# Bob-cheng/DepthModelHardening

Measured on AMD Instinct MI355X. Metric: adv-train images/sec @1024x320, 10-step PGD, bs32, higher is better.
Workload: dtype f32; 1 GPU; Monodepth2 ResNet18 1024x320, 10-step PGD-L_inf attack on 12 scenes, train batch 32/GPU, stereo photometric+SSIM+smoothness loss (md2), Adam; config_index=2, global_batch=32, per_gpu_batch=32, parallelism=dp1, attack_overlap=False, attack_scenes=12, graph_attack=False

## Files before the change

depthmodelhardening_amd/_native.py:

```python
import ctypes as C
import os

import torch

MAX_SCALES = 4
MAX_FRAMES = 4
VARIANT_MD2, VARIANT_DH = 0, 1
NOISE_NONE, NOISE_TENSOR, NOISE_PHILOX = 0, 1, 2
PASTE_COMPOSITE, PASTE_WARP_ONLY = 0, 1
FIN_LOSS, FIN_LOSS_S, FIN_REPROJ_S, FIN_COUNT_S, FIN_SMOOTH_S, FIN_HINT_S, FIN_HINTCOUNT_S, FIN_SIZE = 0, 1, 5, 9, 13, 20, 24, 28

LIB_PATH = os.environ.get("DMH_HIP_LIB") or os.path.join(os.path.dirname(os.path.abspath(__file__)), "lib",
                                                        "libdmh_hip.so")

_fp = C.c_void_p


class PhotoArgs(C.Structure):
    _fields_ = [("target", _fp), ("source", _fp * MAX_FRAMES), ("T", _fp * MAX_FRAMES), ("K", _fp), ("inv_K", _fp),
                ("disp", _fp * MAX_SCALES), ("Hs", C.c_int * MAX_SCALES), ("Ws", C.c_int * MAX_SCALES),
                ("B", C.c_int), ("H", C.c_int), ("W", C.c_int), ("num_frames", C.c_int), ("num_scales", C.c_int),
                ("min_depth", C.c_float), ("max_depth", C.c_float), ("variant", C.c_int), ("automask", C.c_int),
                ("no_ssim", C.c_int), ("noise_mode", C.c_int), ("noise", _fp * MAX_SCALES),
                ("seed", C.c_uint64), ("offset", C.c_uint64), ("depth_hint", _fp), ("depth_hint_mask", _fp)]


class SmoothArgs(C.Structure):
    _fields_ = [("disp", _fp * MAX_SCALES), ("color", _fp * MAX_SCALES), ("Hs", C.c_int * MAX_SCALES),
                ("Ws", C.c_int * MAX_SCALES), ("B", C.c_int), ("num_scales", C.c_int)]


class PasteArgs(C.Structure):
    _fields_ = [("scene", _fp), ("scene_bstride", C.c_int64), ("patch", _fp), ("pmask", _fp), ("coeffs", _fp),
                ("N", C.c_int), ("SH", C.c_int), ("SW", C.c_int), ("PH", C.c_int), ("PW", C.c_int),
                ("OH", C.c_int), ("OW", C.c_int), ("l_pad", C.c_int), ("t_pad", C.c_int), ("mode", C.c_int),
                ("flip", _fp), ("scene_index", _fp)]


class RoiGlueArgs(C.Structure):
    _fields_ = [("y", _fp), ("skip", _fp), ("y_org", _fp), ("skip_org", _fp), ("dst_org", _fp),
                ("B", C.c_int), ("C1", C.c_int), ("C2", C.c_int), ("sh", C.c_int), ("sw", C.c_int), ("kh", C.c_int),
                ("kw", C.c_int), ("hc", C.c_int), ("wc", C.c_int), ("H", C.c_int), ("W", C.c_int), ("up", C.c_int),
                ("elu", C.c_int)]


class WinoWtJob(C.Structure):
    _fields_ = [("w", _fp), ("scale", _fp), ("U", _fp), ("K", C.c_int), ("C", C.c_int), ("backward", C.c_int)]


_PtrArr = _fp * MAX_SCALES

_SIGNATURES = {
    "dmh_version": (C.c_char_p, []),
    "dmh_last_error": (C.c_char_p, []),
    "dmh_debug_channel_copy": (C.c_int, [_fp, _fp, C.c_int64, C.c_int, C.c_int, _fp]),
    "dmh_photo_partials_size": (C.c_int64, [C.c_int, C.c_int, C.c_int, C.c_int]),
    "dmh_photo_stage_size": (C.c_int64, [C.POINTER(PhotoArgs)]),
    "dmh_photo_loss_fwd": (C.c_int, [C.POINTER(PhotoArgs), _fp, _PtrArr, _fp, _fp]),
    "dmh_photo_loss_bwd": (C.c_int, [C.POINTER(PhotoArgs), _fp, _fp, _fp, _fp, _PtrArr, _fp]),
    "dmh_photo_pose_partials_size": (C.c_int64, [C.POINTER(PhotoArgs)]),
    "dmh_photo_loss_bwd_pose": (C.c_int, [C.POINTER(PhotoArgs), _fp, _fp, _fp, _fp, _PtrArr, _fp, _fp]),
    "dmh_unpack_selection": (C.c_int, [_fp, C.c_int64, C.c_int, _fp, _fp]),
    "dmh_upsample_bilinear_adjoint": (C.c_int, [_fp, _fp, C.c_int, C.c_int, C.c_int, C.c_int, C.c_int, C.c_int, _fp]),
    "dmh_warp_view_fwd": (C.c_int, [_fp] * 5 + [C.c_int] * 5 + [C.c_float, C.c_float] + [_fp] * 4),
    "dmh_warp_view_bwd": (C.c_int, [_fp] * 5 + [C.c_int] * 5 + [C.c_float, C.c_float] + [_fp] * 4),
    "dmh_smooth_partials_size": (C.c_int64, [C.POINTER(SmoothArgs)]),
    "dmh_smooth_loss_fwd": (C.c_int, [C.POINTER(SmoothArgs), _fp, _fp]),
    "dmh_smooth_loss_bwd": (C.c_int, [C.POINTER(SmoothArgs), _fp, _fp, C.c_float, _PtrArr, C.c_int, _fp]),
    "dmh_loss_finalize": (C.c_int, [_fp, _fp, C.c_int, C.c_int, C.c_int, C.POINTER(SmoothArgs), C.c_int, C.c_float,
                                    _fp, _fp, _fp]),
    "dmh_eot_paste_fwd": (C.c_int, [C.POINTER(PasteArgs), _fp, _fp, _fp]),
    "dmh_eot_paste_bwd": (C.c_int, [C.POINTER(PasteArgs), _fp, _fp, _fp]),
    "dmh_pgd_linf_step": (C.c_int, [_fp, _fp, _fp, C.c_float, C.c_float, _fp, C.c_int64, _fp]),
    "dmh_apgd_step": (C.c_int, [_fp] * 6 + [C.c_int, C.c_float, C.c_int64, _fp]),
    "dmh_apgd_commit": (C.c_int, [_fp] * 10 + [C.c_int] * 3 + [C.c_double, C.c_int64, _fp]),
    "dmh_l0_fused_step": (C.c_int, [_fp] * 15 + [C.c_int] * 3 + [C.c_float] * 3 + [_fp]),
    "dmh_tube_light_compose": (C.c_int, [_fp] * 4 + [C.c_int] * 3 + [_fp]),
    "dmh_tube_light_commit": (C.c_int, [_fp] * 4 + [C.c_int, _fp]),
    "dmh_gauss_blur_windows": (C.c_int, [_fp] * 5 + [C.c_int] * 9 + [_fp]),
    "dmh_gauss_blur_compose": (C.c_int, [_fp] * 4 + [C.c_int] * 8 + [_fp]),
    "dmh_square_propose": (C.c_int, [_fp] * 6 + [C.c_int] * 4 + [C.c_float, _fp]),
    "dmh_pgd_l2_workspace_size": (C.c_int64, [C.c_int64]),
    "dmh_pgd_l2_step": (C.c_int, [_fp, _fp, _fp, C.c_double, C.c_double, _fp, C.c_int64, _fp, C.c_int64, _fp]),
    "dmh_eigen_select_ws_size": (C.c_int64, [C.c_int]),
    "dmh_eigen_partials_size": (C.c_int64, [C.c_int]),
    "dmh_eigen_gt_stats": (C.c_int, [_fp, C.c_int64, _fp, _fp] + [C.c_int] * 7 + [_fp] * 4),
    "dmh_eigen_pred_depth": (C.c_int, [_fp, _fp, C.c_int, C.c_int, _fp, C.c_int64, _fp, _fp] + [C.c_int] * 7
                             + [C.c_float, C.c_int64, _fp, C.c_int64, _fp, _fp]),
    "dmh_eigen_pred_ratio": (C.c_int, [_fp, C.c_int64, C.c_int64, C.c_int64, _fp, _fp] + [C.c_int] * 6 + [_fp] * 5),
    "dmh_eigen_metrics": (C.c_int, [_fp, C.c_int64, _fp, C.c_int64, C.c_int64, _fp, _fp] + [C.c_int] * 6 + [_fp] * 4),
    "dmh_l0_compose_fwd": (C.c_int, [_fp, _fp, _fp, C.c_int, C.c_int, C.c_float, C.c_int, _fp, _fp, _fp]),
    "dmh_l0_compose_bwd": (C.c_int, [_fp, _fp, _fp, _fp, C.c_int, C.c_int, _fp, _fp, C.c_int, _fp]),
    "dmh_l0_mask_partials_size": (C.c_int64, [C.c_int]),
    "dmh_l0_mask_cost_fwd": (C.c_int, [_fp, _fp, C.c_int, C.c_int, _fp, _fp, _fp]),
    "dmh_l0_mask_cost_bwd": (C.c_int, [_fp, _fp, C.c_int, C.c_int, _fp, _fp, _fp, _fp, C.c_int, _fp]),
    "dmh_sq_mean_partials_size": (C.c_int64, [C.c_int64]),
    "dmh_masked_sq_mean_fwd": (C.c_int, [_fp, _fp, C.c_int64, _fp, _fp, _fp]),
    "dmh_masked_sq_mean_bwd": (C.c_int, [_fp, _fp, C.c_int64, _fp, _fp, _fp]),
    "dmh_gt_depth_mse_fwd": (C.c_int, [_fp, _fp, _fp, C.c_int64, _fp, C.c_int, C.c_int64, C.c_float, C.c_float, _fp, _fp, _fp]),
    "dmh_gt_depth_mse_bwd": (C.c_int, [_fp, _fp, _fp, C.c_int64, _fp, C.c_int, C.c_int64, C.c_float, C.c_float, _fp, _fp, _fp]),
    "dmh_ssim_map": (C.c_int, [_fp, _fp, C.c_int, C.c_int, C.c_int, _fp, _fp]),
    "dmh_ssim_map_bwd": (C.c_int, [_fp, _fp, _fp, C.c_int, C.c_int, C.c_int, _fp, _fp, _fp, _fp]),
    "dmh_avg_pyramid": (C.c_int, [_fp, C.c_int, C.c_int, C.c_int, _fp, _fp, _fp, _fp]),
    "dmh_edge_smooth_partials_size": (C.c_int64, [C.c_int, C.c_int, C.c_int]),
    "dmh_edge_smooth": (C.c_int, [_fp, _fp] + [C.c_int] * 4 + [_fp, _fp, _fp]),
    "dmh_edge_smooth_bwd": (C.c_int, [_fp, _fp] + [C.c_int] * 4 + [_fp, _fp, _fp]),
    "dmh_depth_errors_partials_size": (C.c_int64, [C.c_int64]),
    "dmh_masked_depth_errors": (C.c_int, [_fp, _fp, _fp, C.c_int64] + [C.c_float] * 5 + [_fp, _fp, _fp]),
    "dmh_dec_up_cat_pad_fwd": (C.c_int, [_fp, _fp] + [C.c_int] * 5 + [_fp, _fp]),
    "dmh_dec_up_cat_pad_bwd": (C.c_int, [_fp, _fp] + [C.c_int] * 5 + [_fp, _fp, _fp]),
    "dmh_elu_pad_fwd": (C.c_int, [_fp] + [C.c_int] * 5 + [_fp, _fp]),
    "dmh_elu_pad_bwd": (C.c_int, [_fp, _fp] + [C.c_int] * 5 + [_fp, _fp]),
    "dmh_roi_glue_fwd": (C.c_int, [C.POINTER(RoiGlueArgs), _fp, _fp]),
    "dmh_roi_glue_bwd": (C.c_int, [C.POINTER(RoiGlueArgs), _fp, _fp, _fp, _fp, C.c_int, C.c_int, _fp, C.c_int, C.c_int, _fp]),
    "dmh_roi_crop": (C.c_int, [_fp] * 4 + [C.c_int] * 7 + [_fp, _fp]),
    "dmh_roi_paste": (C.c_int, [_fp, _fp, C.c_int, C.c_int, _fp] + [C.c_int] * 6 + [_fp, _fp]),
    "dmh_stem_conv_norm_fwd_win": (C.c_int, [_fp, _fp, _fp] + [C.c_int] * 5 + [C.c_float, C.c_float, _fp, _fp]),
    "dmh_stem_bn_relu_pool_bwd_win": (C.c_int, [_fp] * 7 + [C.c_int] * 8 + [_fp, _fp]),
    "dmh_conv7x7s2_bwd_data_win": (C.c_int, [_fp] * 4 + [C.c_int] * 9 + [_fp, _fp]),
    "dmh_roi_cost_partials_size": (C.c_int64, [C.c_int, C.c_int, C.c_int]),
    "dmh_roi_cost_fwd": (C.c_int, [_fp, _fp, _fp] + [C.c_int] * 5 + [_fp] * 4),
    "dmh_roi_cost_bwd": (C.c_int, [_fp, _fp, _fp] + [C.c_int] * 5 + [_fp] * 3),
    "dmh_roi_cost_fwd_scaled": (C.c_int, [_fp, _fp, _fp] + [C.c_int] * 5 + [C.c_float] + [_fp] * 4),
    "dmh_roi_cost_bwd_scaled": (C.c_int, [_fp, _fp, _fp] + [C.c_int] * 5 + [C.c_float] + [_fp] * 3),
    "dmh_bn_act_fwd": (C.c_int, [_fp] * 4 + [C.c_int] * 4 + [_fp, _fp]),
    "dmh_bn_act_bwd": (C.c_int, [_fp] * 3 + [C.c_int] * 4 + [_fp, _fp, _fp]),
    "dmh_bn_stats_partials_size": (C.c_int64, [C.c_int, C.c_int, C.c_int]),
    "dmh_bn_train_stats": (C.c_int, [_fp, C.c_int, C.c_int, C.c_int, _fp, _fp, C.c_float, C.c_float] + [_fp] * 8),
    "dmh_bn_train_stats_tracked": (C.c_int, [_fp, C.c_int, C.c_int, C.c_int, _fp, _fp, C.c_float, C.c_float] + [_fp] * 9),
    "dmh_channel_sum_partials_size": (C.c_int64, [C.c_int, C.c_int, C.c_int]),
    "dmh_channel_sum": (C.c_int, [_fp, C.c_int, C.c_int, C.c_int, _fp, _fp, C.c_void_p]),
    "dmh_bn_train_bwd_workspace_size": (C.c_int64, [C.c_int, C.c_int, C.c_int]),
    "dmh_bn_train_bwd": (C.c_int, [_fp] * 6 + [C.c_int, C.c_int, C.c_int] + [_fp] * 5 + [C.c_void_p]),
    "dmh_stem_bn_relu_pool_fwd": (C.c_int, [_fp] * 3 + [C.c_int] * 4 + [_fp] * 4),
    "dmh_stem_bn_relu_pool_bwd": (C.c_int, [_fp] * 5 + [C.c_int] * 4 + [_fp, _fp]),
    "dmh_wino_weight_size": (C.c_int64, [C.c_int, C.c_int]),
    "dmh_wino_weight_transform": (C.c_int, [_fp, C.c_int, C.c_int, C.c_int, _fp, _fp]),
    "dmh_wino_conv3x3": (C.c_int, [_fp] * 3 + [C.c_int] * 6 + [_fp, _fp]),
    "dmh_wino_conv3x3_ws": (C.c_int, [_fp] * 3 + [C.c_int] * 6 + [_fp, _fp, C.c_int64, _fp]),
    "dmh_wino_conv3x3_plan": (C.c_int, [C.c_int] * 7 + [C.c_int64]),
    "dmh_wino_weight_transform_scaled": (C.c_int, [_fp, C.c_int, C.c_int, C.c_int, _fp, _fp, _fp]),
    "dmh_wino_conv3x3_act": (C.c_int, [_fp] * 4 + [C.c_int] * 7 + [_fp, _fp]),
    "dmh_wino_weight_transform_batch": (C.c_int, [C.POINTER(WinoWtJob), C.c_int, _fp]),
    "dmh_wino_conv3x3_act_ws": (C.c_int, [_fp] * 4 + [C.c_int] * 7 + [_fp, _fp, C.c_int64, _fp]),
    "dmh_wino32_weight_size": (C.c_int64, [C.c_int, C.c_int]),
    "dmh_wino32_weight_transform": (C.c_int, [_fp, C.c_int, C.c_int, C.c_int, _fp, _fp]),
    "dmh_wino32_conv3x3": (C.c_int, [_fp] * 3 + [C.c_int] * 6 + [_fp, _fp]),
    "dmh_wino32_conv3x3_ws": (C.c_int, [_fp] * 3 + [C.c_int] * 6 + [_fp, _fp, C.c_int64, _fp]),
    "dmh_wino_wrw_workspace_size": (C.c_int64, [C.c_int] * 6),
    "dmh_wino_wrw": (C.c_int, [_fp, _fp] + [C.c_int] * 6 + [_fp, _fp, _fp]),
    "dmh_conv3x3_small": (C.c_int, [_fp] * 3 + [C.c_int] * 7 + [_fp, _fp]),
    "dmh_conv3x3_head": (C.c_int, [_fp] * 3 + [C.c_int] * 5 + [_fp, _fp]),
    "dmh_conv3x3_head_bwd_data": (C.c_int, [_fp, _fp] + [C.c_int] * 4 + [_fp, _fp]),
    "dmh_down_wrw_workspace_size": (C.c_int64, [C.c_int] * 5),
    "dmh_down_wrw": (C.c_int, [_fp] * 3 + [C.c_int] * 5 + [_fp] * 4),
    "dmh_stem_wrw_workspace_size": (C.c_int64, [C.c_int] * 3),
    "dmh_stem_wrw": (C.c_int, [_fp, _fp] + [C.c_int] * 3 + [C.c_float, C.c_float, _fp, _fp, _fp]),
    "dmh_conv3x3_head_wrw_partials_size": (C.c_int64, [C.c_int] * 5),
    "dmh_conv3x3_head_wrw": (C.c_int, [_fp, _fp] + [C.c_int] * 5 + [_fp] * 4),
    "dmh_conv3x3_small_wrw_partials_size": (C.c_int64, [C.c_int]),
    "dmh_conv3x3_small_wrw": (C.c_int, [_fp, _fp] + [C.c_int] * 5 + [_fp] * 4),
    "dmh_conv7x7s2_bwd_data": (C.c_int, [_fp, _fp] + [C.c_int] * 5 + [_fp, _fp]),
    "dmh_stem_conv_norm_fwd": (C.c_int, [_fp, _fp, C.c_int, C.c_int, C.c_int, C.c_float, C.c_float, _fp, _fp]),
    "dmh_down_conv_fwd": (C.c_int, [_fp] * 3 + [C.c_int] * 5 + [_fp] * 3),
    "dmh_down_conv_fwd_act": (C.c_int, [_fp] * 5 + [C.c_int] * 6 + [_fp] * 3),
    "dmh_down_conv_bwd_data": (C.c_int, [_fp] * 4 + [C.c_int] * 5 + [_fp, _fp]),
    "dmh_down_conv_bwd_data_acc": (C.c_int, [_fp] * 5 + [C.c_int] * 5 + [_fp, _fp]),
    "dmh_down_conv_image_size": (C.c_int64, [C.c_int, C.c_int]),
    "dmh_down_conv_weight_image": (C.c_int, [_fp, _fp, C.c_int, C.c_int, _fp, _fp]),
    "dmh_down_conv_fwd_img": (C.c_int, [_fp, _fp, C.c_int, _fp, _fp] + [C.c_int] * 6 + [_fp] * 3),
    "dmh_down_conv_bwd_data_img": (C.c_int, [_fp] * 4 + [C.c_int] * 5 + [_fp, _fp]),
}

EXPORTS = tuple(sorted(_SIGNATURES))

_lib = None


def lib():
    global _lib
    if _lib is None:
        if not os.path.exists(LIB_PATH) and "DMH_HIP_LIB" not in os.environ:
            try:
                from .build import build
                build(verbose=False)
            except Exception as e:
                raise RuntimeError("libdmh_hip.so is not built (%s) and building it failed (%s): run `python -m "
                                   "depthmodelhardening_amd.build`; there is no CPU/eager fallback for the hot path"
                                   % (LIB_PATH, e))
        if not os.path.exists(LIB_PATH):
            raise RuntimeError("libdmh_hip.so is not built (%s): run `python -m depthmodelhardening_amd.build`; "
                               "there is no CPU/eager fallback for the hot path" % LIB_PATH)
        handle = C.CDLL(LIB_PATH)
        for name, (res, args) in _SIGNATURES.items():
            fn = getattr(handle, name)
            fn.restype = res
            fn.argtypes = args
        _lib = handle
    return _lib


def check(rc):
    if rc != 0:
        raise RuntimeError("libdmh_hip: " + lib().dmh_last_error().decode())


def ptr(t):
    if t is None:
        return None
    if not t.is_cuda:
        raise RuntimeError("libdmh_hip ops need CUDA (ROCm) tensors; got device %s -- there is no CPU path" % t.device)
    if not t.is_contiguous():
        raise RuntimeError("libdmh_hip ops need contiguous tensors")
    if t.dtype not in (torch.float32, torch.int32, torch.uint8):
        raise RuntimeError("libdmh_hip ops compute in fp32; got %s" % t.dtype)
    return C.c_void_p(t.data_ptr())


def ptr_f64(t):
    if not t.is_cuda:
        raise RuntimeError("libdmh_hip ops need CUDA (ROCm) tensors; got device %s -- there is no CPU path" % t.device)
    if not t.is_contiguous() or t.dtype != torch.float64:
        raise RuntimeError("libdmh_hip: expected a contiguous float64 tensor; got %s" % t.dtype)
    return C.c_void_p(t.data_ptr())


def stream():
    return C.c_void_p(torch.cuda.current_stream().cuda_stream)


def ptr_array(tensors, n=MAX_SCALES):
    arr = (_fp * n)()
    for i, t in enumerate(tensors):
        arr[i] = None if t is None else ptr(t)
    return arr
```

depthmodelhardening_amd/csrc/common.hpp:

```cpp
#pragma once
#include <hip/hip_runtime.h>

#include <atomic>
#include <stdint.h>
#include <stdio.h>
#include <string.h>

#include "dmh_hip.h"

namespace dmh {

constexpr int WAVE = 64;

extern thread_local char g_err[512];

inline int fail(int code, const char* fmt, const char* a = "", long long b = 0, long long c = 0) {
    snprintf(g_err, sizeof(g_err), fmt, a, b, c);
    return code;
}

#define DMH_REQUIRE(cond, msg)                                                     \
    do {                                                                            \
        if (!(cond)) return dmh::fail(DMH_EINVAL, "%s: requirement failed: " msg, __func__); \
    } while (0)

inline int check_launch(const char* fn) {
    hipError_t e = hipGetLastError();
    if (e != hipSuccess) {
        snprintf(g_err, sizeof(g_err), "%s: launch failed: %s", fn, hipGetErrorString(e));
        return DMH_ELAUNCH;
    }
    return DMH_OK;
}

__device__ __forceinline__ float wave_sum(float v) {
#pragma unroll
    for (int o = WAVE / 2; o > 0; o >>= 1) v += __shfl_down(v, o, WAVE);
    return v;
}

template <int NT>
__device__ __forceinline__ float block_sum(float v, float* red) {
    v = wave_sum(v);
    const int lane = threadIdx.x & (WAVE - 1), w = threadIdx.x / WAVE;
    __syncthreads();
    if (lane == 0) red[w] = v;
    __syncthreads();
    float t = 0.f;
    if (threadIdx.x == 0) {
#pragma unroll
        for (int i = 0; i < NT / WAVE; ++i) t += red[i];
    }
    return t;
}

__device__ __forceinline__ int reflect_idx(int p, int n) {
    p = p < 0 ? -p : p;
    p = p >= n ? 2 * (n - 1) - p : p;
    return min(max(p, 0), n - 1);
}

__device__ __forceinline__ float fast_rcp(float x) {
    float r = __builtin_amdgcn_rcpf(x);
    return r * (2.0f - x * r);
}

typedef __amdgpu_buffer_rsrc_t rsrc_t;

__device__ __forceinline__ rsrc_t make_rsrc(const void* p, unsigned bytes) {
    const unsigned long long v = (unsigned long long)p;
    const unsigned lo = __builtin_amdgcn_readfirstlane((unsigned)v), hi = __builtin_amdgcn_readfirstlane((unsigned)(v >> 32));
    return __builtin_amdgcn_make_buffer_rsrc((void*)(((unsigned long long)hi << 32) | lo), 0, bytes, 0x00020000);
}
typedef float f32x2 __attribute__((ext_vector_type(2)));
#define DMH_PK_FORM(NAME, MODS)                                                  \
    __device__ __forceinline__ f32x2 NAME(const f32x2 a, const f32x2 b) {        \
        f32x2 r;                                                                 \
        asm("v_pk_add_f32 %0, %1, %2 " MODS : "=v"(r) : "v"(a), "v"(b));         \
        return r;                                                                \
    }
DMH_PK_FORM(pk_add, "")
DMH_PK_FORM(pk_sub, "neg_lo:[0,1] neg_hi:[0,1]")
DMH_PK_FORM(pk_bfly, "op_sel:[0,1] op_sel_hi:[0,1] neg_hi:[0,1]")
DMH_PK_FORM(pk_bfly_neg, "op_sel:[0,1] op_sel_hi:[0,1] neg_lo:[1,1] neg_hi:[1,0]")
DMH_PK_FORM(pk_col01, "op_sel:[0,0] op_sel_hi:[1,0] neg_lo:[0,1]")
DMH_PK_FORM(pk_col23, "op_sel:[1,0] op_sel_hi:[1,1] neg_lo:[1,0] neg_hi:[0,1]")
#define DMH_PK_MOV(NAME, MODS)                                                   \
    __device__ __forceinline__ f32x2 NAME(const f32x2 a, const f32x2 b) {        \
        f32x2 r;                                                                 \
        asm("v_pk_mov_b32 %0, %1, %2 " MODS : "=v"(r) : "v"(a), "v"(b));         \
        return r;                                                                \
    }
DMH_PK_MOV(pk_lo_lo, "op_sel:[0,0]")
DMH_PK_MOV(pk_hi_hi, "op_sel:[1,1]")

__device__ __forceinline__ float ldb(rsrc_t rs, unsigned byte_off, unsigned s_off) {
    return __builtin_bit_cast(float, __builtin_amdgcn_raw_buffer_load_b32(rs, byte_off, s_off, 0));
}
__device__ __forceinline__ float lane_prev(float v) {
    return __builtin_bit_cast(float, __builtin_amdgcn_update_dpp(0, __builtin_bit_cast(int, v), 0x138, 0xf, 0xf, false));
}
__device__ __forceinline__ float lane_next(float v) {
    return __builtin_bit_cast(float, __builtin_amdgcn_update_dpp(0, __builtin_bit_cast(int, v), 0x130, 0xf, 0xf, false));
}

template <int ROUNDS = 7>
struct Philox {
    uint32_t k0, k1;
    __device__ __forceinline__ Philox(uint64_t seed) : k0((uint32_t)seed), k1((uint32_t)(seed >> 32)) {}
    __device__ __forceinline__ uint4 operator()(uint64_t ctr_lo, uint64_t ctr_hi) const {
        uint32_t c0 = (uint32_t)ctr_lo, c1 = (uint32_t)(ctr_lo >> 32), c2 = (uint32_t)ctr_hi,
                 c3 = (uint32_t)(ctr_hi >> 32);
        uint32_t a = k0, b = k1;
#pragma unroll
        for (int r = 0; r < ROUNDS; ++r) {
            const uint32_t hi0 = __umulhi(0xD2511F53u, c0), lo0 = 0xD2511F53u * c0;
            const uint32_t hi1 = __umulhi(0xCD9E8D57u, c2), lo1 = 0xCD9E8D57u * c2;
            const uint32_t n0 = hi1 ^ c1 ^ a, n1 = lo1, n2 = hi0 ^ c3 ^ b, n3 = lo0;
            c0 = n0; c1 = n1; c2 = n2; c3 = n3;
            a += 0x9E3779B9u;
            b += 0xBB67AE85u;
        }
        return make_uint4(c0, c1, c2, c3);
    }
};

__device__ __forceinline__ float normal_from_bits(uint32_t u0, uint32_t u1) {
    const float a = ((float)u0 + 1.0f) * 2.3283064365386963e-10f;
    const float b = (float)u1 * 2.3283064365386963e-10f;
    return sqrtf(-2.0f * __logf(a)) * __cosf(6.283185307179586f * b);
}

__device__ __forceinline__ float2 normal_pair_from_bits(uint32_t u0, uint32_t u1) {
    const float a = ((float)u0 + 1.0f) * 2.3283064365386963e-10f;
    const float b = (float)u1 * 2.3283064365386963e-10f;
    const float rad = sqrtf(-2.0f * __logf(a));
    float sn, cs;
    __sincosf(6.283185307179586f * b, &sn, &cs);
    return make_float2(rad * cs, rad * sn);
}

__host__ __device__ inline int sk_boundary(int per, int rem, int nch, int w) {
    const int b = w * per + (w < rem ? w : rem);
    const int item = b / nch;
    int c = b - item * nch;
    if (c != 0) {
        if (nch >= 6) c = c < 3 ? 3 : (c > nch - 3 ? nch - 3 : c);
        else c = (2 * c < nch) ? 0 : nch;
    }
    return item * nch + c;
}

template <typename Kernel>
inline hipError_t configure_dynamic_lds(Kernel kernel, size_t bytes, std::atomic<uint64_t>& done) {
    int dev = 0;
    hipError_t e = hipGetDevice(&dev);
    if (e != hipSuccess) return e;
    const uint64_t bit = (dev >= 0 && dev < 64) ? (1ull << dev) : 0;
    if (bit && (done.load(std::memory_order_acquire) & bit)) return hipSuccess;
    e = hipFuncSetAttribute(reinterpret_cast<const void*>(kernel), hipFuncAttributeMaxDynamicSharedMemorySize, (int)bytes);
    if (e == hipSuccess && bit) done.fetch_or(bit, std::memory_order_release);
    return e;
}

}
```

depthmodelhardening_amd/csrc/encoder_glue.hip:

```cpp
#include "common.hpp"

#include <cmath>

using namespace dmh;

namespace {

constexpr int NT = 256;

__device__ __forceinline__ float relu_f(float v) { return v > 0.f ? v : 0.f; }

template <bool RELU, bool RES>
__global__ __launch_bounds__(NT) void bn_act_fwd_vec(const float4* __restrict__ x, const float* __restrict__ scale,
                                                     const float* __restrict__ shift, const float4* __restrict__ res,
                                                     unsigned C, unsigned hw4, unsigned total4, float4* __restrict__ out) {
    const unsigned i = blockIdx.x * NT + threadIdx.x;
    if (i >= total4) return;
    const unsigned c = (i / hw4) % C;
    const float s = scale[c], b = shift[c];
    const float4 v = x[i];
    float4 r = make_float4(fmaf(v.x, s, b), fmaf(v.y, s, b), fmaf(v.z, s, b), fmaf(v.w, s, b));
    if (RES) {
        const float4 q = res[i];
        r.x += q.x; r.y += q.y; r.z += q.z; r.w += q.w;
// ... 41 lines not shown
    if (RES) g_res[i] = gv;
    g_x[i] = gv * scale[(i / hw) % C];
}

__global__ __launch_bounds__(NT) void stem_fwd_kernel(const float* __restrict__ x, const float* __restrict__ scale,
                                                      const float* __restrict__ shift, int C, int H, int W,
                                                      float* __restrict__ feat, float* __restrict__ pooled,
                                                      unsigned char* __restrict__ argmax) {
    const int PH = H >> 1, PW = W >> 1;
    const int t = blockIdx.x * NT + threadIdx.x;
    if (t >= PH * PW) return;
    const int plane = blockIdx.y, c = plane % C;
    const int i = t / PW, j = t - i * PW;
    const float s = scale[c], b = shift[c];
    const float* xp = x + (size_t)plane * H * W;
    float* fp = feat + (size_t)plane * H * W;
    float m = -INFINITY;
    int arg = 4;
#pragma unroll
    for (int ky = 0; ky < 3; ++ky) {
        const int yy = 2 * i - 1 + ky;
        if (yy < 0) continue;
        const float* row = xp + (size_t)yy * W + 2 * j;
        const float2 vc = *reinterpret_cast<const float2*>(row);
        const float a1 = relu_f(fmaf(vc.x, s, b)), a2 = relu_f(fmaf(vc.y, s, b));
        if (j > 0) {
            const float a0 = relu_f(fmaf(row[-1], s, b));
            if (a0 > m) { m = a0; arg = ky * 3; }
        }
        if (a1 > m) { m = a1; arg = ky * 3 + 1; }
        if (a2 > m) { m = a2; arg = ky * 3 + 2; }
        if (ky >= 1) *reinterpret_cast<float2*>(fp + (size_t)yy * W + 2 * j) = make_float2(a1, a2);
    }
    const size_t o = (size_t)plane * PH * PW + t;
    pooled[o] = m;
    argmax[o] = (unsigned char)arg;
}

__global__ __launch_bounds__(NT) void stem_bwd_kernel(const float* __restrict__ feat, const unsigned char* __restrict__ argmax,
                                                      const float* __restrict__ g_feat, const float* __restrict__ g_pool,
                                                      const float* __restrict__ scale, int C, int H, int W,
                                                      float* __restrict__ g_x) {
    const int PH = H >> 1, PW = W >> 1;
    const int t = blockIdx.x * NT + threadIdx.x;
    if (t >= PH * PW) return;
    const int plane = blockIdx.y, c = plane % C;
    const int i = t / PW, j = t - i * PW;
    const size_t base = (size_t)plane * H * W, pbase = (size_t)plane * PH * PW;
    float acc[2][2] = {{0.f, 0.f}, {0.f, 0.f}};
    if (g_pool) {
#pragma unroll
        for (int di = 0; di < 2; ++di) {
            const int oi = i + di;
            if (oi >= PH) continue;
#pragma unroll
            for (int dj = 0; dj < 2; ++dj) {
                const int oj = j + dj;
                if (oj >= PW) continue;
                const int a = argmax[pbase + (size_t)oi * PW + oj];
                const int ky = a / 3, kx = a - ky * 3;
                const int ry = 2 * di - 1 + ky, rx = 2 * dj - 1 + kx;
                if (ry >= 0 && ry < 2 && rx >= 0 && rx < 2) {
                    const float gp = g_pool[pbase + (size_t)oi * PW + oj];
                    if (ry == 0 && rx == 0) acc[0][0] += gp;
                    if (ry == 0 && rx == 1) acc[0][1] += gp;
                    if (ry == 1 && rx == 0) acc[1][0] += gp;
                    if (ry == 1 && rx == 1) acc[1][1] += gp;
                }
            }
        }
    }
    const float s = scale[c];
#pragma unroll
    for (int r = 0; r < 2; ++r) {
        const size_t o = base + (size_t)(2 * i + r) * W + 2 * j;
        const float2 f = *reinterpret_cast<const float2*>(feat + o);
        float g0 = acc[r][0], g1 = acc[r][1];
        if (g_feat) {
            const float2 gf = *reinterpret_cast<const float2*>(g_feat + o);
            g0 += gf.x;
            g1 += gf.y;
        }
        *reinterpret_cast<float2*>(g_x + o) = make_float2(f.x > 0.f ? g0 * s : 0.f, f.y > 0.f ? g1 * s : 0.f);
    }
}

__global__ __launch_bounds__(NT) void stem_bwd4_kernel(const float* __restrict__ feat, const unsigned char* __restrict__ argmax,
                                                       const float* __restrict__ g_feat, const float* __restrict__ g_pool,
                                                       const float* __restrict__ scale, int C, int H, int W,
                                                       float* __restrict__ g_x) {
    const int PH = H >> 1, PW = W >> 1, PW2 = PW >> 1;
    const int t = blockIdx.x * NT + threadIdx.x;
    if (t >= PH * PW2) return;
    const int plane = blockIdx.y, c = plane % C;
    const int i = t / PW2, j = (t - i * PW2) * 2;
    const size_t base = (size_t)plane * H * W, pbase = (size_t)plane * PH * PW;
    float acc[2][4] = {{0.f, 0.f, 0.f, 0.f}, {0.f, 0.f, 0.f, 0.f}};
    if (g_pool) {
#pragma unroll
        for (int di = 0; di < 2; ++di) {
            const int oi = i + di;
            if (oi >= PH) continue;
#pragma unroll
            for (int dj = 0; dj < 3; ++dj) {
                const int oj = j + dj;
                if (oj >= PW) continue;
                const int a = argmax[pbase + (size_t)oi * PW + oj];
                const int ky = a / 3, kx = a - ky * 3;
                const int ry = 2 * di - 1 + ky, rx = 2 * dj - 1 + kx;
                if (ry >= 0 && ry < 2 && rx >= 0 && rx < 4) {
                    const float gp = g_pool[pbase + (size_t)oi * PW + oj];
#pragma unroll
                    for (int r = 0; r < 2; ++r)
#pragma unroll
                        for (int q = 0; q < 4; ++q)
                            if (ry == r && rx == q) acc[r][q] += gp;
                }
            }
        }
    }
    const float s = scale[c];
#pragma unroll
    for (int r = 0; r < 2; ++r) {
        const size_t o = base + (size_t)(2 * i + r) * W + 2 * j;
        const float4 f = *reinterpret_cast<const float4*>(feat + o);
        float g0 = acc[r][0], g1 = acc[r][1], g2 = acc[r][2], g3 = acc[r][3];
        if (g_feat) {
            const float4 gf = *reinterpret_cast<const float4*>(g_feat + o);
            g0 += gf.x;
            g1 += gf.y;
            g2 += gf.z;
            g3 += gf.w;
        }
        *reinterpret_cast<float4*>(g_x + o) = make_float4(f.x > 0.f ? g0 * s : 0.f, f.y > 0.f ? g1 * s : 0.f,
                                                          f.z > 0.f ? g2 * s : 0.f, f.w > 0.f ? g3 * s : 0.f);
    }
}

__device__ __forceinline__ int slabs_of(int HW, int s, int S) {
    const int nslab = (HW + 4 * NT - 1) / (4 * NT);
    return s < nslab ? (nslab - 1 - s) / S + 1 : 0;
}

struct Wf {
    float n, mean, m2;
};
__device__ __forceinline__ Wf wf_merge(Wf a, Wf b) {
    if (b.n == 0.f) return a;
    if (a.n == 0.f) return b;
    const float n = a.n + b.n, d = b.mean - a.mean, f = b.n / n;
    return Wf{n, a.mean + d * f, a.m2 + b.m2 + d * d * a.n * f};
}

__global__ __launch_bounds__(NT) void bn_stats_partial_kernel(const float* __restrict__ x, int B, int C, int HW, int S,
                                                              float* __restrict__ part) {
    const int c = blockIdx.y, s = blockIdx.x;
    const float k = x[(size_t)c * HW];
    float nq[4] = {0.f, 0.f, 0.f, 0.f}, s1q[4] = {0.f, 0.f, 0.f, 0.f}, s2q[4] = {0.f, 0.f, 0.f, 0.f};
    for (int b = 0; b < B; ++b) {
        const float* xp = x + ((size_t)b * C + c) * HW;
        if ((HW & 3) == 0) continue;
        for (int r0 = s * 4 * NT; r0 < HW; r0 += S * 4 * NT) {
            float v[4];
#pragma unroll
            for (int q = 0; q < 4; ++q) {
                const int r = r0 + q * NT + threadIdx.x;
                v[q] = r < HW ? xp[r] : k;
                nq[q] += r < HW ? 1.f : 0.f;
            }
#pragma unroll
            for (int q = 0; q < 4; ++q) {
                const float d = v[q] - k;
                s1q[q] += d;
                s2q[q] = fmaf(d, d, s2q[q]);
            }
        }
    }
    if ((HW & 3) == 0) {
        const int nk = slabs_of(HW, s, S), total = B * nk;
        for (int i0 = 0; i0 < total; i0 += 4) {
            float4 v4[4];
            bool ok[4];
#pragma unroll
            for (int u = 0; u < 4; ++u) {
                const int i = min(i0 + u, total - 1), b = i / nk, r = (s + (i - b * nk) * S) * 4 * NT + 4 * (int)threadIdx.x;
                ok[u] = i0 + u < total && r < HW;
                v4[u] = ok[u] ? *reinterpret_cast<const float4*>(x + ((size_t)b * C + c) * HW + r) : make_float4(k, k, k, k);
            }
#pragma unroll
            for (int u = 0; u < 4; ++u) {
                const float v[4] = {v4[u].x, v4[u].y, v4[u].z, v4[u].w};
#pragma unroll
                for (int q = 0; q < 4; ++q) {
                    const float d = v[q] - k;
                    nq[q] += ok[u] ? 1.f : 0.f;
                    s1q[q] += d;
                    s2q[q] = fmaf(d, d, s2q[q]);
                }
            }
        }
    }
    const float n = (nq[0] + nq[1]) + (nq[2] + nq[3]), s1 = (s1q[0] + s1q[1]) + (s1q[2] + s1q[3]),
                s2 = (s2q[0] + s2q[1]) + (s2q[2] + s2q[3]);
    Wf w{n, n > 0.f ? k + s1 / n : 0.f, n > 0.f ? s2 - s1 * s1 / n : 0.f};
#pragma unroll
    for (int o = WAVE / 2; o > 0; o >>= 1) {
        Wf other{__shfl_down(w.n, o, WAVE), __shfl_down(w.mean, o, WAVE), __shfl_down(w.m2, o, WAVE)};
        w = wf_merge(w, other);
    }
    __shared__ Wf red[NT / WAVE];
    if ((threadIdx.x & (WAVE - 1)) == 0) red[threadIdx.x / WAVE] = w;
    __syncthreads();
    if (threadIdx.x == 0) {
        Wf t = red[0];
#pragma unroll
        for (int i = 1; i < NT / WAVE; ++i) t = wf_merge(t, red[i]);
        float* p = part + ((size_t)c * S + s) * 3;
        p[0] = t.n; p[1] = t.mean; p[2] = t.m2;
    }
}

__global__ __launch_bounds__(NT) void bn_stats_finalize_kernel(const float* __restrict__ part, int C, int S,
                                                               const float* __restrict__ weight,
                                                               const float* __restrict__ bias, float momentum, float eps,
                                                               float* __restrict__ running_mean,
                                                               float* __restrict__ running_var, float* __restrict__ scale,
                                                               float* __restrict__ shift, float* __restrict__ save_mean,
                                                               float* __restrict__ save_invstd,
                                                               long long* __restrict__ num_batches_tracked) {
    const int c = blockIdx.x * NT + threadIdx.x;
    if (c >= C) return;
    if (c == 0 && num_batches_tracked) num_batches_tracked[0] += 1;
    Wf t{0.f, 0.f, 0.f};
    for (int s = 0; s < S; ++s) {
        const float* p = part + ((size_t)c * S + s) * 3;
        t = wf_merge(t, Wf{p[0], p[1], p[2]});
    }
    const float var = t.m2 / t.n, invstd = rsqrtf(var + eps);
    const float sc = (weight ? weight[c] : 1.f) * invstd;
    scale[c] = sc;
    shift[c] = (bias ? bias[c] : 0.f) - t.mean * sc;
    save_mean[c] = t.mean;
    save_invstd[c] = invstd;
    if (running_mean) running_mean[c] = (1.f - momentum) * running_mean[c] + momentum * t.mean;
    if (running_var) running_var[c] = (1.f - momentum) * running_var[c] + momentum * (t.m2 / fmaxf(t.n - 1.f, 1.f));
}

inline unsigned blocks_for(int64_t n) { return (unsigned)((n + NT - 1) / NT); }

template <bool RELU, bool VEC>
__global__ __launch_bounds__(NT) void bn_bwd_partial_kernel(const float* __restrict__ x, const float* __restrict__ g,
                                                            const float* __restrict__ out, const float* __restrict__ mean,
                                                            int B, int C, int HW, int S, float* __restrict__ part) {
    const int c = blockIdx.y, s = blockIdx.x;
    const float m = mean[c];
    float a1[4] = {0.f, 0.f, 0.f, 0.f}, a2[4] = {0.f, 0.f, 0.f, 0.f};
    for (int b = 0; b < B; ++b) {
        const size_t base = ((size_t)b * C + c) * HW;
        if (VEC) {
            break;
        } else {
            for (int r0 = s * 4 * NT; r0 < HW; r0 += S * 4 * NT) {
#pragma unroll
                for (int q = 0; q < 4; ++q) {
                    const int r = r0 + q * NT + (int)threadIdx.x;
                    if (r < HW) {
                        float gv = g[base + r];
                        if (RELU) gv = out[base + r] > 0.f ? gv : 0.f;
                        a1[q] += gv;
                        a2[q] = fmaf(gv, x[base + r] - m, a2[q]);
                    }
                }
            }
        }
    }
    if (VEC) {
        const int nk = slabs_of(HW, s, S), total = B * nk;
        for (int i0 = 0; i0 < total; i0 += 2) {
            float4 xv[2], gv[2], ov[2];
#pragma unroll
            for (int u = 0; u < 2; ++u) {
                const int i = min(i0 + u, total - 1), b = i / nk, r = (s + (i - b * nk) * S) * 4 * NT + 4 * (int)threadIdx.x;
                const bool ok = i0 + u < total && r < HW;
                const size_t o = ((size_t)b * C + c) * HW + r;
                xv[u] = ok ? *reinterpret_cast<const float4*>(x + o) : make_float4(m, m, m, m);
                gv[u] = ok ? *reinterpret_cast<const float4*>(g + o) : make_float4(0.f, 0.f, 0.f, 0.f);
                if (RELU) ov[u] = ok ? *reinterpret_cast<const float4*>(out + o) : make_float4(0.f, 0.f, 0.f, 0.f);
            }
#pragma unroll
            for (int u = 0; u < 2; ++u) {
                float4 gq = gv[u];
                if (RELU)
                    gq = make_float4(ov[u].x > 0.f ? gq.x : 0.f, ov[u].y > 0.f ? gq.y : 0.f, ov[u].z > 0.f ? gq.z : 0.f,
                                     ov[u].w > 0.f ? gq.w : 0.f);
                a1[0] += gq.x; a1[1] += gq.y; a1[2] += gq.z; a1[3] += gq.w;
                a2[0] = fmaf(gq.x, xv[u].x - m, a2[0]); a2[1] = fmaf(gq.y, xv[u].y - m, a2[1]);
                a2[2] = fmaf(gq.z, xv[u].z - m, a2[2]); a2[3] = fmaf(gq.w, xv[u].w - m, a2[3]);
            }
        }
    }
    float s1 = (a1[0] + a1[1]) + (a1[2] + a1[3]), s2 = (a2[0] + a2[1]) + (a2[2] + a2[3]);
#pragma unroll
    for (int o = WAVE / 2; o > 0; o >>= 1) {
        s1 += __shfl_down(s1, o, WAVE);
        s2 += __shfl_down(s2, o, WAVE);
    }
    __shared__ float red[NT / WAVE][2];
    if ((threadIdx.x & (WAVE - 1)) == 0) {
        red[threadIdx.x / WAVE][0] = s1;
        red[threadIdx.x / WAVE][1] = s2;
    }
    __syncthreads();
    if (threadIdx.x == 0) {
        float t1 = red[0][0], t2 = red[0][1];
#pragma unroll
        for (int i = 1; i < NT / WAVE; ++i) {
            t1 += red[i][0];
            t2 += red[i][1];
        }
        part[((size_t)c * S + s) * 2 + 0] = t1;
        part[((size_t)c * S + s) * 2 + 1] = t2;
    }
}

__global__ __launch_bounds__(NT) void bn_bwd_finalize_kernel(const float* __restrict__ part, int C, int S, double inv_n,
                                                             const float* __restrict__ weight, const float* __restrict__ mean,
                                                             const float* __restrict__ invstd, float* __restrict__ coef,
                                                             float* __restrict__ g_weight, float* __restrict__ g_bias) {
    const int c = blockIdx.x * NT + threadIdx.x;
    if (c >= C) return;
    double s1 = 0.0, s2 = 0.0;
    for (int s = 0; s < S; ++s) {
        s1 += (double)part[((size_t)c * S + s) * 2 + 0];
        s2 += (double)part[((size_t)c * S + s) * 2 + 1];
    }
    const double is = (double)invstd[c], w = weight ? (double)weight[c] : 1.0;
    if (g_bias) g_bias[c] = (float)s1;
    if (g_weight) g_weight[c] = (float)(s2 * is);
    float4 k;
    k.x = (float)(w * is);
    k.y = (float)(s1 * inv_n);
    k.z = (float)(s2 * is * is * inv_n);
    k.w = mean[c];
    reinterpret_cast<float4*>(coef)[c] = k;
}

template <bool RELU, bool RES>
__global__ __launch_bounds__(NT) void bn_bwd_apply_vec(const float4* __restrict__ x, const float4* __restrict__ g,
                                                       const float4* __restrict__ out, const float4* __restrict__ coef,
                                                       unsigned C, unsigned hw4, unsigned total4, float4* __restrict__ g_x,
                                                       float4* __restrict__ g_res) {
    const unsigned i = blockIdx.x * NT + threadIdx.x;
    if (i >= total4) return;
    const float4 k = coef[(i / hw4) % C];
    const float4 xv = x[i];
    float4 gv = g[i];
    if (RELU) {
        const float4 o = out[i];
        gv = make_float4(o.x > 0.f ? gv.x : 0.f, o.y > 0.f ? gv.y : 0.f, o.z > 0.f ? gv.z : 0.f, o.w > 0.f ? gv.w : 0.f);
    }
    if (RES) g_res[i] = gv;
    g_x[i] = make_float4(k.x * ((gv.x - k.y) - (xv.x - k.w) * k.z), k.x * ((gv.y - k.y) - (xv.y - k.w) * k.z),
                         k.x * ((gv.z - k.y) - (xv.z - k.w) * k.z), k.x * ((gv.w - k.y) - (xv.w - k.w) * k.z));
}

template <bool RELU, bool RES>
__global__ __launch_bounds__(NT) void bn_bwd_apply_scalar(const float* __restrict__ x, const float* __restrict__ g,
                                                          const float* __restrict__ out, const float4* __restrict__ coef,
                                                          unsigned C, unsigned hw, unsigned total, float* __restrict__ g_x,
                                                          float* __restrict__ g_res) {
    const unsigned i = blockIdx.x * NT + threadIdx.x;
    if (i >= total) return;
    const float4 k = coef[(i / hw) % C];
    float gv = g[i];
    if (RELU) gv = out[i] > 0.f ? gv : 0.f;
    if (RES) g_res[i] = gv;
    g_x[i] = k.x * ((gv - k.y) - (x[i] - k.w) * k.z);
}

template <bool RELU, bool RES>
void launch_bn_bwd_apply(const float* x, const float* g, const float* out, const float* coef, int C, int HW, int64_t total,
                         float* g_x, float* g_res, hipStream_t st) {
    if ((HW & 3) == 0)
        hipLaunchKernelGGL((bn_bwd_apply_vec<RELU, RES>), dim3(blocks_for(total / 4)), dim3(NT), 0, st,
                           reinterpret_cast<const float4*>(x), reinterpret_cast<const float4*>(g),
                           reinterpret_cast<const float4*>(out), reinterpret_cast<const float4*>(coef), (unsigned)C,
                           (unsigned)(HW / 4), (unsigned)(total / 4), reinterpret_cast<float4*>(g_x),
                           reinterpret_cast<float4*>(g_res));
    else
        hipLaunchKernelGGL((bn_bwd_apply_scalar<RELU, RES>), dim3(blocks_for(total)), dim3(NT), 0, st, x, g, out,
                           reinterpret_cast<const float4*>(coef), (unsigned)C, (unsigned)HW, (unsigned)total, g_x, g_res);
}

__global__ __launch_bounds__(NT) void channel_sum_partial_kernel(const float* __restrict__ g, int B, int C, int HW, int S,
                                                                 float* __restrict__ part) {
    const int c = blockIdx.y, s = blockIdx.x;
    float a[4] = {0.f, 0.f, 0.f, 0.f};
    if ((HW & 3) == 0) {
        const int nk = slabs_of(HW, s, S), total = B * nk;
        for (int i0 = 0; i0 < total; i0 += 4) {
            float4 v[4];
#pragma unroll
            for (int u = 0; u < 4; ++u) {
                const int i = min(i0 + u, total - 1), b = i / nk, r = (s + (i - b * nk) * S) * 4 * NT + 4 * (int)threadIdx.x;
                v[u] = (i0 + u < total && r < HW) ? *reinterpret_cast<const float4*>(g + ((size_t)b * C + c) * HW + r)
                                                  : make_float4(0.f, 0.f, 0.f, 0.f);
            }
#pragma unroll
            for (int u = 0; u < 4; ++u) { a[0] += v[u].x; a[1] += v[u].y; a[2] += v[u].z; a[3] += v[u].w; }
        }
    } else {
        for (int b = 0; b < B; ++b) {
            const float* gp = g + ((size_t)b * C + c) * HW;
            for (int r = s * NT + (int)threadIdx.x; r < HW; r += S * NT) a[0] += gp[r];
        }
    }
    float t = (a[0] + a[1]) + (a[2] + a[3]);
#pragma unroll
    for (int o = WAVE / 2; o > 0; o >>= 1) t += __shfl_down(t, o, WAVE);
    __shared__ float red[NT / WAVE];
    if ((threadIdx.x & (WAVE - 1)) == 0) red[threadIdx.x / WAVE] = t;
    __syncthreads();
    if (threadIdx.x == 0) {
        float u = red[0];
#pragma unroll
        for (int i = 1; i < NT / WAVE; ++i) u += red[i];
        part[(size_t)c * S + s] = u;
    }
}

__global__ __launch_bounds__(NT) void channel_sum_finalize_kernel(const float* __restrict__ part, int C, int S,
                                                                  float* __restrict__ out) {
    const int c = blockIdx.x * NT + threadIdx.x;
    if (c >= C) return;
    double t = 0.0;
    for (int s = 0; s < S; ++s) t += (double)part[(size_t)c * S + s];
    out[c] = (float)t;
}

template <bool RELU, bool RES>
void launch_fwd(const float* x, const float* scale, const float* shift, const float* res, int C, int HW, int64_t total,
                float* out, hipStream_t st) {
    if ((HW & 3) == 0)
        hipLaunchKernelGGL((bn_act_fwd_vec<RELU, RES>), dim3(blocks_for(total / 4)), dim3(NT), 0, st,
                           reinterpret_cast<const float4*>(x), scale, shift, reinterpret_cast<const float4*>(res),
                           (unsigned)C, (unsigned)(HW / 4), (unsigned)(total / 4), reinterpret_cast<float4*>(out));
    else
        hipLaunchKernelGGL((bn_act_fwd_scalar<RELU, RES>), dim3(blocks_for(total)), dim3(NT), 0, st, x, scale, shift, res,
                           (unsigned)C, (unsigned)HW, (unsigned)total, out);
}

template <bool RELU, bool RES>
void launch_bwd(const float* out, const float* g, const float* scale, int C, int HW, int64_t total, float* g_x,
                float* g_res, hipStream_t st) {
    if ((HW & 3) == 0)
        hipLaunchKernelGGL((bn_act_bwd_vec<RELU, RES>), dim3(blocks_for(total / 4)), dim3(NT), 0, st,
                           reinterpret_cast<const float4*>(out), reinterpret_cast<const float4*>(g), scale, (unsigned)C,
                           (unsigned)(HW / 4), (unsigned)(total / 4), reinterpret_cast<float4*>(g_x),
                           reinterpret_cast<float4*>(g_res));
    else
        hipLaunchKernelGGL((bn_act_bwd_scalar<RELU, RES>), dim3(blocks_for(total)), dim3(NT), 0, st, out, g, scale,
                           (unsigned)C, (unsigned)HW, (unsigned)total, g_x, g_res);
}

}

extern "C" {

int dmh_bn_act_fwd(const float* x, const float* scale, const float* shift, const float* residual, int B, int C, int HW,
                   int relu, float* out, void* stream) {
    DMH_REQUIRE(x && scale && shift && out, "null pointer");
    DMH_REQUIRE(B > 0 && C > 0 && HW > 0, "bad sizes");
    const int64_t total = (int64_t)B * C * HW;
    DMH_REQUIRE(total < ((int64_t)1 << 31), "tensor too large");
    hipStream_t st = (hipStream_t)stream;
    if (relu) {
        if (residual) launch_fwd<true, true>(x, scale, shift, residual, C, HW, total, out, st);
        else launch_fwd<true, false>(x, scale, shift, nullptr, C, HW, total, out, st);
    } else {
        if (residual) launch_fwd<false, true>(x, scale, shift, residual, C, HW, total, out, st);
        else launch_fwd<false, false>(x, scale, shift, nullptr, C, HW, total, out, st);
    }
    return check_launch("dmh_bn_act_fwd");
}

int dmh_bn_act_bwd(const float* out, const float* g_out, const float* scale, int B, int C, int HW, int relu, float* g_x,
                   float* g_residual, void* stream) {
    DMH_REQUIRE(g_out && scale && g_x && (out || !relu), "null pointer");
    DMH_REQUIRE(B > 0 && C > 0 && HW > 0, "bad sizes");
    const int64_t total = (int64_t)B * C * HW;
    DMH_REQUIRE(total < ((int64_t)1 << 31), "tensor too large");
    hipStream_t st = (hipStream_t)stream;
    if (relu) {
        if (g_residual) launch_bwd<true, true>(out, g_out, scale, C, HW, total, g_x, g_residual, st);
        else launch_bwd<true, false>(out, g_out, scale, C, HW, total, g_x, nullptr, st);
    } else {
        if (g_residual) launch_bwd<false, true>(out, g_out, scale, C, HW, total, g_x, g_residual, st);
        else launch_bwd<false, false>(out, g_out, scale, C, HW, total, g_x, nullptr, st);
    }
    return check_launch("dmh_bn_act_bwd");
}

int64_t dmh_bn_stats_partials_size(int B, int C, int HW) {
    if (B <= 0 || C <= 0 || HW <= 0) return -1;
    int64_t S = ((int64_t)HW + 4 * NT - 1) / (4 * NT);
    if (S > 64) S = 64;
    return (int64_t)C * S * 3;
}

int dmh_bn_train_stats(const float* x, int B, int C, int HW, const float* weight, const float* bias, float momentum,
                       float eps, float* running_mean, float* running_var, float* partials, float* scale, float* shift,
                       float* save_mean, float* save_invstd, void* stream) {
    return dmh_bn_train_stats_tracked(x, B, C, HW, weight, bias, momentum, eps, running_mean, running_var, nullptr, partials,
                                      scale, shift, save_mean, save_invstd, stream);
}

int dmh_bn_train_stats_tracked(const float* x, int B, int C, int HW, const float* weight, const float* bias, float momentum,
                               float eps, float* running_mean, float* running_var, long long* num_batches_tracked,
                               float* partials, float* scale, float* shift, float* save_mean, float* save_invstd,
                               void* stream) {
    DMH_REQUIRE(x && partials && scale && shift && save_mean && save_invstd, "null pointer");
    DMH_REQUIRE((reinterpret_cast<uintptr_t>(num_batches_tracked) & 7) == 0, "num_batches_tracked must be an aligned int64");
    DMH_REQUIRE(B > 0 && C > 0 && HW > 0 && C <= 65535, "bad sizes");
    int64_t S = ((int64_t)HW + 4 * NT - 1) / (4 * NT);
    if (S > 64) S = 64;
    hipStream_t st = (hipStream_t)stream;
    hipLaunchKernelGGL(bn_stats_partial_kernel, dim3((unsigned)S, C), dim3(NT), 0, st, x, B, C, HW, (int)S, partials);
    hipLaunchKernelGGL(bn_stats_finalize_kernel, dim3(blocks_for(C)), dim3(NT), 0, st, partials, C, (int)S, weight, bias,
                       momentum, eps, running_mean, running_var, scale, shift, save_mean, save_invstd, num_batches_tracked);
    return check_launch("dmh_bn_train_stats");
}

int64_t dmh_channel_sum_partials_size(int B, int C, int HW) {
    const int64_t S = dmh_bn_stats_partials_size(B, C, HW);
    return S < 0 ? -1 : S / 3;
}

int dmh_channel_sum(const float* g, int B, int C, int HW, float* partials, float* out, void* stream) {
    DMH_REQUIRE(g && partials && out, "null pointer");
    DMH_REQUIRE(B > 0 && C > 0 && HW > 0 && C <= 65535, "bad sizes");
    int64_t S = ((int64_t)HW + 4 * NT - 1) / (4 * NT);
    if (S > 64) S = 64;
    hipStream_t st = (hipStream_t)stream;
    hipLaunchKernelGGL(channel_sum_partial_kernel, dim3((unsigned)S, C), dim3(NT), 0, st, g, B, C, HW, (int)S, partials);
    hipLaunchKernelGGL(channel_sum_finalize_kernel, dim3(blocks_for(C)), dim3(NT), 0, st, partials, C, (int)S, out);
    return check_launch("dmh_channel_sum");
}

int64_t dmh_bn_train_bwd_workspace_size(int B, int C, int HW) {
    const int64_t S = dmh_bn_stats_partials_size(B, C, HW);
    if (S < 0) return -1;
    return S / 3 * 2 + (int64_t)C * 4;
}

int dmh_bn_train_bwd(const float* x, const float* g_out, const float* out, const float* weight, const float* save_mean,
                     const float* save_invstd, int B, int C, int HW, float* workspace, float* g_x, float* g_weight,
                     float* g_bias, float* g_pre, void* stream) {
    DMH_REQUIRE(x && g_out && save_mean && save_invstd && workspace && g_x, "null pointer");
    DMH_REQUIRE(B > 0 && C > 0 && HW > 0 && C <= 65535, "bad sizes");
    const int64_t total = (int64_t)B * C * HW;
    DMH_REQUIRE(total < ((int64_t)1 << 31), "tensor too large");
    DMH_REQUIRE((reinterpret_cast<uintptr_t>(workspace) & 15) == 0, "workspace must be 16-byte aligned");
    int64_t S = ((int64_t)HW + 4 * NT - 1) / (4 * NT);
    if (S > 64) S = 64;
    hipStream_t st = (hipStream_t)stream;
    float* coef = workspace;
    float* part = workspace + (size_t)C * 4;
    const dim3 pg((unsigned)S, C);
    const bool vec = (HW & 3) == 0;
    if (out) {
        if (vec) hipLaunchKernelGGL((bn_bwd_partial_kernel<true, true>), pg, dim3(NT), 0, st, x, g_out, out, save_mean, B, C, HW, (int)S, part);
        else hipLaunchKernelGGL((bn_bwd_partial_kernel<true, false>), pg, dim3(NT), 0, st, x, g_out, out, save_mean, B, C, HW, (int)S, part);
    } else {
        if (vec) hipLaunchKernelGGL((bn_bwd_partial_kernel<false, true>), pg, dim3(NT), 0, st, x, g_out, out, save_mean, B, C, HW, (int)S, part);
        else hipLaunchKernelGGL((bn_bwd_partial_kernel<false, false>), pg, dim3(NT), 0, st, x, g_out, out, save_mean, B, C, HW, (int)S, part);
    }
    hipLaunchKernelGGL(bn_bwd_finalize_kernel, dim3(blocks_for(C)), dim3(NT), 0, st, part, C, (int)S,
                       1.0 / ((double)B * (double)HW), weight, save_mean, save_invstd, coef, g_weight, g_bias);
    if (out) {
        if (g_pre) launch_bn_bwd_apply<true, true>(x, g_out, out, coef, C, HW, total, g_x, g_pre, st);
        else launch_bn_bwd_apply<true, false>(x, g_out, out, coef, C, HW, total, g_x, nullptr, st);
    } else {
        if (g_pre) launch_bn_bwd_apply<false, true>(x, g_out, out, coef, C, HW, total, g_x, g_pre, st);
        else launch_bn_bwd_apply<false, false>(x, g_out, out, coef, C, HW, total, g_x, nullptr, st);
    }
    return check_launch("dmh_bn_train_bwd");
}

int dmh_stem_bn_relu_pool_fwd(const float* x, const float* scale, const float* shift, int B, int C, int H, int W,
                              float* feat, float* pooled, unsigned char* argmax, void* stream) {
    DMH_REQUIRE(x && scale && shift && feat && pooled && argmax, "null pointer");
    DMH_REQUIRE(B > 0 && C > 0 && H >= 2 && W >= 2 && (H & 1) == 0 && (W & 1) == 0, "H and W must be even and >= 2");
    DMH_REQUIRE((int64_t)B * C <= 65535 && (int64_t)H * W < (1 << 30), "tensor too large");
    hipLaunchKernelGGL(stem_fwd_kernel, dim3(blocks_for((int64_t)(H / 2) * (W / 2)), B * C), dim3(NT), 0,
                       (hipStream_t)stream, x, scale, shift, C, H, W, feat, pooled, argmax);
    return check_launch("dmh_stem_bn_relu_pool_fwd");
}

int dmh_stem_bn_relu_pool_bwd(const float* feat, const unsigned char* argmax, const float* g_feat, const float* g_pooled,
                              const float* scale, int B, int C, int H, int W, float* g_x, void* stream) {
    DMH_REQUIRE(feat && argmax && scale && g_x, "null pointer");
    DMH_REQUIRE(B > 0 && C > 0 && H >= 2 && W >= 2 && (H & 1) == 0 && (W & 1) == 0, "H and W must be even and >= 2");
    DMH_REQUIRE((int64_t)B * C <= 65535 && (int64_t)H * W < (1 << 30), "tensor too large");
    if ((W & 3) == 0)
        hipLaunchKernelGGL(stem_bwd4_kernel, dim3(blocks_for((int64_t)(H / 2) * (W / 4)), B * C), dim3(NT), 0,
                           (hipStream_t)stream, feat, argmax, g_feat, g_pooled, scale, C, H, W, g_x);
    else
        hipLaunchKernelGGL(stem_bwd_kernel, dim3(blocks_for((int64_t)(H / 2) * (W / 2)), B * C), dim3(NT), 0,
                           (hipStream_t)stream, feat, argmax, g_feat, g_pooled, scale, C, H, W, g_x);
    return check_launch("dmh_stem_bn_relu_pool_bwd");
}

}
```

depthmodelhardening_amd/csrc/roi_glue.hip:

```cpp
#include <stdlib.h>

#include "common.hpp"

using namespace dmh;

namespace {

constexpr int NT = 256;

__device__ __forceinline__ float elu_f(float x) { return x > 0.f ? x : expf(x) - 1.f; }
__device__ __forceinline__ float elu_grad(float x) { return x > 0.f ? 1.f : expf(x); }

__device__ __forceinline__ void split_rc(int t, int w2, unsigned magic, int& row, int& col2) {
    if (w2 == 1) {
        row = t;
        col2 = 0;
        return;
    }
    int r = (int)__umulhi((unsigned)t, magic);
    if (r * w2 > t) --r;
    row = r;
    col2 = t - r * w2;
}

// ... 124 lines not shown
        }
        const float* gp = g_out + (size_t)(b * C + a.C1 + c) * PH * PW;
        const int Ys = ky0 + yy, Xs = kx0 + xx;
        g_skip[((size_t)q * a.kh + yy) * a.kw + xx] = (Ys > 1 && Ys < a.H - 2 && Xs > 1 && Xs < a.W - 2)
                                                          ? gather_interior(gp, Ys, Xs, oy, ox, PH, PW)
                                                          : gather_pad(gp, Ys, Xs, a.H, a.W, oy, ox, PH, PW);
    }
}

__device__ __forceinline__ float glue_bwd_y_elem(const dmh_roi_glue_args& a, const float* __restrict__ gp, int Ys, int Xs, int oy,
                                                 int ox, int PH, int PW) {
    if (a.up) {
        const int Y0 = 2 * Ys, X0 = 2 * Xs;
        if (Y0 > 1 && Y0 + 1 < a.H - 2 && X0 > 1 && X0 + 1 < a.W - 2) {
            const int r = Y0 + 1 - oy, q = X0 + 1 - ox;
            if (r >= 0 && r + 1 < PH && q >= 0 && q + 1 < PW) {
                const float* p0 = gp + r * PW + q;
                return p0[0] + p0[1] + p0[PW] + p0[PW + 1];
            }
            if (r + 1 < 0 || r >= PH || q + 1 < 0 || q >= PW) return 0.f;
            return gather_interior(gp, Y0, X0, oy, ox, PH, PW) + gather_interior(gp, Y0, X0 + 1, oy, ox, PH, PW) +
                   gather_interior(gp, Y0 + 1, X0, oy, ox, PH, PW) + gather_interior(gp, Y0 + 1, X0 + 1, oy, ox, PH, PW);
        }
        return gather_pad(gp, Y0, X0, a.H, a.W, oy, ox, PH, PW) + gather_pad(gp, Y0, X0 + 1, a.H, a.W, oy, ox, PH, PW) +
               gather_pad(gp, Y0 + 1, X0, a.H, a.W, oy, ox, PH, PW) + gather_pad(gp, Y0 + 1, X0 + 1, a.H, a.W, oy, ox, PH, PW);
    }
    if (Ys > 1 && Ys < a.H - 2 && Xs > 1 && Xs < a.W - 2) return gather_interior(gp, Ys, Xs, oy, ox, PH, PW);
    return gather_pad(gp, Ys, Xs, a.H, a.W, oy, ox, PH, PW);
}

struct Region2 {
    Region rg;
    unsigned ymagic, kmagic;
    int yblocks, kblocks;
};
template <int CPT>
__global__ __launch_bounds__(NT) void roi_glue_bwd2_kernel(const dmh_roi_glue_args a, const Region2 r2,
                                                           const float* __restrict__ g_out, float* __restrict__ g_y,
                                                           float* __restrict__ g_skip) {
    const Region& rg = r2.rg;
    const int PH = a.hc + 2, PW = a.wc + 2, C = a.C1 + a.C2;
    const int ytotal = r2.yblocks * a.B * (a.C1 / CPT);
    const bool ypart = (int)blockIdx.x < ytotal;
    const int bid = ypart ? (int)blockIdx.x : (int)blockIdx.x - ytotal;
    const int per = ypart ? r2.yblocks : r2.kblocks;
    const int pl = bid / per;
    const int t = (bid - pl * per) * NT + (int)threadIdx.x;
    const size_t gplane = (size_t)PH * PW;
    if (ypart) {
        const int groups = a.C1 / CPT;
        const int b = pl / groups, c0 = (pl - b * groups) * CPT;
        const int w2 = rg.yw >> 1;
        if (t >= rg.yh * w2) return;
        const int oy = a.dst_org[2 * b], ox = a.dst_org[2 * b + 1];
        const int sy0 = a.y_org ? a.y_org[2 * b] : 0, sx0 = a.y_org ? a.y_org[2 * b + 1] : 0;
        int yy, xx;
        split_rc(t, w2, r2.ymagic, yy, xx);
        xx *= 2;
        if (rg.y_org) {
            yy += rg.y_org[2 * b];
            xx += rg.y_org[2 * b + 1];
        }
        const int Ys = sy0 + yy, Xs = sx0 + xx;
        const float* gp = g_out + (size_t)(b * C + c0) * gplane;
        const size_t splane = (size_t)a.sh * a.sw;
        size_t o = ((size_t)(b * a.C1 + c0) * a.sh + yy) * a.sw + xx;
        int fast = 0, off = 0;
        if (a.up) {
            const int Y0 = 2 * Ys, X0 = 2 * Xs, r = Y0 + 1 - oy, q = X0 + 1 - ox;
            if (Y0 > 1 && Y0 + 1 < a.H - 2 && X0 > 1 && X0 + 3 < a.W - 2 && r >= 0 && r + 1 < PH && q >= 0 && q + 3 < PW) {
                fast = 1;
                off = r * PW + q;
            }
        } else {
            const int r = Ys + 1 - oy, q = Xs + 1 - ox;
            if (Ys > 1 && Ys < a.H - 2 && Xs > 1 && Xs + 1 < a.W - 2 && r >= 0 && r < PH && q >= 0 && q + 1 < PW) {
                fast = 2;
                off = r * PW + q;
            }
        }
        if (fast == 1) {
#pragma unroll
            for (int j = 0; j < CPT; ++j, gp += gplane, o += splane) {
                const float* p0 = gp + off;
                float v0 = p0[0] + p0[1] + p0[PW] + p0[PW + 1];
                float v1 = p0[2] + p0[3] + p0[PW + 2] + p0[PW + 3];
                if (a.elu) {
                    const float2 yv = *reinterpret_cast<const float2*>(a.y + o);
                    v0 = v0 != 0.f ? v0 * elu_grad(yv.x) : v0;
                    v1 = v1 != 0.f ? v1 * elu_grad(yv.y) : v1;
                }
                *reinterpret_cast<float2*>(g_y + o) = make_float2(v0, v1);
            }
        } else if (fast == 2) {
#pragma unroll
            for (int j = 0; j < CPT; ++j, gp += gplane, o += splane) {
                float v0 = gp[off], v1 = gp[off + 1];
                if (a.elu) {
                    const float2 yv = *reinterpret_cast<const float2*>(a.y + o);
                    v0 = v0 != 0.f ? v0 * elu_grad(yv.x) : v0;
                    v1 = v1 != 0.f ? v1 * elu_grad(yv.y) : v1;
                }
                *reinterpret_cast<float2*>(g_y + o) = make_float2(v0, v1);
            }
        } else {
#pragma unroll 1
            for (int j = 0; j < CPT; ++j, gp += gplane, o += splane) {
                float v0 = glue_bwd_y_elem(a, gp, Ys, Xs, oy, ox, PH, PW);
                float v1 = glue_bwd_y_elem(a, gp, Ys, Xs + 1, oy, ox, PH, PW);
                if (a.elu) {
                    const float2 yv = *reinterpret_cast<const float2*>(a.y + o);
                    v0 = v0 != 0.f ? v0 * elu_grad(yv.x) : v0;
                    v1 = v1 != 0.f ? v1 * elu_grad(yv.y) : v1;
                }
                *reinterpret_cast<float2*>(g_y + o) = make_float2(v0, v1);
            }
        }
    } else {
        const int groups = a.C2 / CPT;
        const int b = pl / groups, c0 = (pl - b * groups) * CPT;
        const int w2 = rg.kw >> 1;
        if (t >= rg.kh * w2) return;
        const int oy = a.dst_org[2 * b], ox = a.dst_org[2 * b + 1];
        const int ky0 = a.skip_org ? a.skip_org[2 * b] : 0, kx0 = a.skip_org ? a.skip_org[2 * b + 1] : 0;
        int yy, xx;
        split_rc(t, w2, r2.kmagic, yy, xx);
        xx *= 2;
        if (rg.skip_org) {
            yy += rg.skip_org[2 * b];
            xx += rg.skip_org[2 * b + 1];
        }
        const float* gp = g_out + (size_t)(b * C + a.C1 + c0) * gplane;
        const int Ys = ky0 + yy, Xs = kx0 + xx;
        const int r = Ys + 1 - oy, qq = Xs + 1 - ox;
        const bool fast = Ys > 1 && Ys < a.H - 2 && Xs > 1 && Xs + 1 < a.W - 2 && r >= 0 && r < PH && qq >= 0 && qq + 1 < PW;
        const bool in0 = Ys > 1 && Ys < a.H - 2 && Xs > 1 && Xs < a.W - 2, in1 = Ys > 1 && Ys < a.H - 2 && Xs + 1 > 1 && Xs + 1 < a.W - 2;
        const size_t kplane = (size_t)a.kh * a.kw;
        float* gs = g_skip + ((size_t)(b * a.C2 + c0) * a.kh + yy) * a.kw + xx;
        if (fast) {
#pragma unroll
            for (int j = 0; j < CPT; ++j, gp += gplane, gs += kplane)
                *reinterpret_cast<float2*>(gs) = make_float2(gp[r * PW + qq], gp[r * PW + qq + 1]);
        } else {
#pragma unroll 1
            for (int j = 0; j < CPT; ++j, gp += gplane, gs += kplane) {
                const float v0 = in0 ? gather_interior(gp, Ys, Xs, oy, ox, PH, PW) : gather_pad(gp, Ys, Xs, a.H, a.W, oy, ox, PH, PW);
                const float v1 = in1 ? gather_interior(gp, Ys, Xs + 1, oy, ox, PH, PW) : gather_pad(gp, Ys, Xs + 1, a.H, a.W, oy, ox, PH, PW);
                *reinterpret_cast<float2*>(gs) = make_float2(v0, v1);
            }
        }
    }
}

__global__ __launch_bounds__(NT) void roi_cost_fwd_kernel(const float* __restrict__ d_pre, const float* __restrict__ mask,
                                                          const int* __restrict__ org, int hd, int wd, int H, int W,
                                                          float* __restrict__ sig, float* __restrict__ partials) {
    __shared__ float s_red[NT / WAVE];
    const int b = blockIdx.y, n = hd * wd;
    const int oy = org[2 * b], ox = org[2 * b + 1];
    float acc = 0.f;
    for (int t = blockIdx.x * NT + threadIdx.x; t < n; t += gridDim.x * NT) {
        const int i = t / wd, j = t - i * wd;
        const float s = 1.f / (1.f + expf(-d_pre[(size_t)b * n + t]));
        sig[(size_t)b * n + t] = s;
        const float v = s * mask[((size_t)b * H + oy + i) * W + ox + j];
        acc += v * v;
    }
    const float r = block_sum<NT>(acc, s_red);
    if (threadIdx.x == 0) partials[blockIdx.y * gridDim.x + blockIdx.x] = r;
}

__global__ __launch_bounds__(NT) void roi_cost_finalize_kernel(const float* __restrict__ partials, int nblk, double n,
                                                               float* __restrict__ cost) {
    __shared__ double s_red[NT];
    double acc = 0.0;
    for (int i = threadIdx.x; i < nblk; i += NT) acc += (double)partials[i];
    s_red[threadIdx.x] = acc;
    __syncthreads();
    for (int o = NT / 2; o > 0; o >>= 1) {
        if ((int)threadIdx.x < o) s_red[threadIdx.x] += s_red[threadIdx.x + o];
        __syncthreads();
    }
    if (threadIdx.x == 0) cost[0] = (float)(s_red[0] / n);
}

__global__ __launch_bounds__(NT) void roi_cost_bwd_kernel(const float* __restrict__ sig, const float* __restrict__ mask,
                                                          const int* __restrict__ org, int hd, int wd, int H, int W,
                                                          const float* __restrict__ gscale, float inv_n,
                                                          float* __restrict__ g_pre) {
    const int b = blockIdx.y, n = hd * wd;
    const int t = blockIdx.x * NT + threadIdx.x;
    if (t >= n) return;
    const int oy = org[2 * b], ox = org[2 * b + 1];
    const int i = t / wd, j = t - i * wd;
    const float s = sig[(size_t)b * n + t], m = mask[((size_t)b * H + oy + i) * W + ox + j];
    g_pre[(size_t)b * n + t] = gscale[0] * 2.f * inv_n * s * m * m * s * (1.f - s);
}

inline unsigned blocks_for(int64_t n) { return (unsigned)((n + NT - 1) / NT); }
inline int cost_blocks(int n) {
    const int b = (n + NT * 4 - 1) / (NT * 4);
    return b < 1 ? 1 : (b > 64 ? 64 : b);
}

int check_glue(const dmh_roi_glue_args* a) {
    DMH_REQUIRE(a && a->y && a->dst_org && (a->skip || a->C2 == 0), "null pointer");
    DMH_REQUIRE(a->B > 0 && a->C1 > 0 && a->C2 >= 0 && a->sh >= 1 && a->sw >= 1 && (a->C2 == 0 || (a->kh >= 1 && a->kw >= 1)),
                "bad sizes");
    DMH_REQUIRE(a->hc >= 2 && a->wc >= 2 && (a->wc & 1) == 0 && a->hc <= a->H && a->wc <= a->W && a->H >= 4 && a->W >= 4,
                "window must be at least 2 x 2, of even width, inside a frame of at least 4 x 4");
    DMH_REQUIRE((int64_t)a->B * (a->C1 + a->C2) <= 65535, "too many planes");
    DMH_REQUIRE((int64_t)a->sh * a->sw < (1 << 30) && (int64_t)a->kh * a->kw < (1 << 30), "source plane too large");
    return DMH_OK;
}

}

extern "C" {

int dmh_roi_glue_fwd(const dmh_roi_glue_args* a, float* out, void* stream) {
    if (int rc = check_glue(a)) return rc;
    DMH_REQUIRE(out, "null pointer");
    const unsigned magic = (unsigned)(((uint64_t)1 << 32) / (unsigned)((a->wc + 2) >> 1)) + 1u;
    const int cpt = (a->C1 % 8 == 0 && a->C2 % 8 == 0) ? 8 : ((a->C1 % 4 == 0 && a->C2 % 4 == 0) ? 4 : 1);
    const dim3 grid(blocks_for((int64_t)(a->hc + 2) * (a->wc + 2) / 2), (unsigned)(a->B * ((a->C1 + a->C2) / cpt)));
    if (cpt == 8) hipLaunchKernelGGL(roi_glue_fwd_kernel<8>, grid, dim3(NT), 0, (hipStream_t)stream, *a, magic, out);
    else if (cpt == 4) hipLaunchKernelGGL(roi_glue_fwd_kernel<4>, grid, dim3(NT), 0, (hipStream_t)stream, *a, magic, out);
    else hipLaunchKernelGGL(roi_glue_fwd_kernel<1>, grid, dim3(NT), 0, (hipStream_t)stream, *a, magic, out);
    return check_launch("dmh_roi_glue_fwd");
}

int dmh_roi_glue_bwd(const dmh_roi_glue_args* a, const float* g_out, float* g_y, float* g_skip, const int* y_reg_org,
                     int y_reg_h, int y_reg_w, const int* skip_reg_org, int skip_reg_h, int skip_reg_w, void* stream) {
    if (int rc = check_glue(a)) return rc;
    DMH_REQUIRE(g_out && g_y, "null pointer");
    DMH_REQUIRE(!y_reg_org || (!a->y_org && y_reg_h >= 1 && y_reg_w >= 1 && y_reg_h <= a->sh && y_reg_w <= a->sw),
                "a y region needs a whole-frame y and must fit its plane");
    DMH_REQUIRE(!skip_reg_org || (!a->skip_org && skip_reg_h >= 1 && skip_reg_w >= 1 && skip_reg_h <= a->kh && skip_reg_w <= a->kw),
                "a skip region needs a whole-frame skip and must fit its plane");
    Region rg;
    rg.y_org = y_reg_org;
    rg.skip_org = skip_reg_org;
    rg.yh = y_reg_org ? y_reg_h : a->sh;
    rg.yw = y_reg_org ? y_reg_w : a->sw;
    rg.kh = skip_reg_org ? skip_reg_h : a->kh;
    rg.kw = skip_reg_org ? skip_reg_w : a->kw;
    const bool skip = g_skip && a->C2 > 0;
    const int planes = a->B * a->C1 + (skip ? a->B * a->C2 : 0);
    const int64_t ny = (int64_t)rg.yh * rg.yw, nk = skip ? (int64_t)rg.kh * rg.kw : 0;
    static const bool wide_ok = !(getenv("DMH_ROI_GLUE2") && atoi(getenv("DMH_ROI_GLUE2")) == 0);
    bool wide = wide_ok && !(rg.yw & 1) && !(a->sw & 1) && !(((uintptr_t)g_y | (uintptr_t)a->y) & 7) &&
                (!skip || (!(rg.kw & 1) && !(a->kw & 1) && !((uintptr_t)g_skip & 7)));
    if (wide) {
        Region2 r2;
        r2.rg = rg;
        const unsigned yw2 = (unsigned)(rg.yw >> 1), kw2 = skip ? (unsigned)(rg.kw >> 1) : 1u;
        r2.ymagic = (unsigned)(((uint64_t)1 << 32) / yw2) + 1u;
        r2.kmagic = (unsigned)(((uint64_t)1 << 32) / kw2) + 1u;
        r2.yblocks = (int)blocks_for(ny / 2);
        r2.kblocks = skip ? (int)blocks_for(nk / 2) : 1;
        const int c2 = skip ? a->C2 : 0;
        static const int cpt_env = getenv("DMH_ROI_GLUE_CPT") ? atoi(getenv("DMH_ROI_GLUE_CPT")) : 1;
        const int cpt = (cpt_env == 8 && a->C1 % 8 == 0 && c2 % 8 == 0) ? 8 : ((cpt_env >= 4 && a->C1 % 4 == 0 && c2 % 4 == 0) ? 4 : 1);
        const int64_t total = (int64_t)r2.yblocks * a->B * (a->C1 / cpt) + (skip ? (int64_t)r2.kblocks * a->B * (c2 / cpt) : 0);
        DMH_REQUIRE(total < ((int64_t)1 << 31), "too many blocks");
        const dim3 grid((unsigned)total);
        if (cpt == 8) hipLaunchKernelGGL(roi_glue_bwd2_kernel<8>, grid, dim3(NT), 0, (hipStream_t)stream, *a, r2, g_out, g_y, g_skip);
        else if (cpt == 4) hipLaunchKernelGGL(roi_glue_bwd2_kernel<4>, grid, dim3(NT), 0, (hipStream_t)stream, *a, r2, g_out, g_y, g_skip);
        else hipLaunchKernelGGL(roi_glue_bwd2_kernel<1>, grid, dim3(NT), 0, (hipStream_t)stream, *a, r2, g_out, g_y, g_skip);
        return check_launch("dmh_roi_glue_bwd");
    }
    hipLaunchKernelGGL(roi_glue_bwd_kernel, dim3(blocks_for(ny > nk ? ny : nk), planes), dim3(NT), 0, (hipStream_t)stream, *a,
                       rg, g_out, g_y, g_skip);
    return check_launch("dmh_roi_glue_bwd");
}

int64_t dmh_roi_cost_partials_size(int B, int hd, int wd) { return (int64_t)B * cost_blocks(hd * wd); }

int dmh_roi_cost_fwd(const float* d_pre, const float* mask, const int* org, int B, int hd, int wd, int H, int W, float* sig,
                     float* partials, float* cost, void* stream) {
    return dmh_roi_cost_fwd_scaled(d_pre, mask, org, B, hd, wd, H, W, 1.f, sig, partials, cost, stream);
}

int dmh_roi_cost_fwd_scaled(const float* d_pre, const float* mask, const int* org, int B, int hd, int wd, int H, int W,
                            float scale, float* sig, float* partials, float* cost, void* stream) {
    DMH_REQUIRE(d_pre && mask && org && sig && partials && cost, "null pointer");
    DMH_REQUIRE(scale == 1.f || scale == -1.f, "scale must be +1 or -1 (a sign: the result stays bit-identical to -cost)");
    DMH_REQUIRE(B > 0 && B <= 65535 && hd >= 1 && wd >= 1 && hd <= H && wd <= W && (int64_t)hd * wd < (1 << 30), "bad sizes");
    const int nb = cost_blocks(hd * wd);
    hipLaunchKernelGGL(roi_cost_fwd_kernel, dim3(nb, B), dim3(NT), 0, (hipStream_t)stream, d_pre, mask, org, hd, wd, H, W, sig,
                       partials);
    hipLaunchKernelGGL(roi_cost_finalize_kernel, dim3(1), dim3(NT), 0, (hipStream_t)stream, partials, nb * B,
                       (double)scale * (double)B * (double)H * (double)W, cost);
    return check_launch("dmh_roi_cost_fwd");
}

int dmh_roi_cost_bwd(const float* sig, const float* mask, const int* org, int B, int hd, int wd, int H, int W,
                     const float* gscale, float* g_pre, void* stream) {
    return dmh_roi_cost_bwd_scaled(sig, mask, org, B, hd, wd, H, W, 1.f, gscale, g_pre, stream);
}

int dmh_roi_cost_bwd_scaled(const float* sig, const float* mask, const int* org, int B, int hd, int wd, int H, int W,
                            float scale, const float* gscale, float* g_pre, void* stream) {
    DMH_REQUIRE(sig && mask && org && gscale && g_pre, "null pointer");
    DMH_REQUIRE(scale == 1.f || scale == -1.f, "scale must be +1 or -1");
    DMH_REQUIRE(B > 0 && B <= 65535 && hd >= 1 && wd >= 1 && hd <= H && wd <= W && (int64_t)hd * wd < (1 << 30), "bad sizes");
    hipLaunchKernelGGL(roi_cost_bwd_kernel, dim3(blocks_for((int64_t)hd * wd), B), dim3(NT), 0, (hipStream_t)stream, sig, mask,
                       org, hd, wd, H, W, gscale, (float)((double)scale / ((double)B * (double)H * (double)W)), g_pre);
    return check_launch("dmh_roi_cost_bwd");
}

}
```

depthmodelhardening_amd/ops.py:

```python
import contextlib
import ctypes as C
import os
from collections import namedtuple

import numpy as np
import torch

from . import _native as N

LossOut = namedtuple("LossOut", ["fin", "sel", "to_opt"])

_profile = None
_profile_only = None


def enable_profile(on=True, only=None):
    global _profile, _profile_only
    _profile = {} if on else None
    _profile_only = tuple(only) if (on and only) else None


def profile_ms():
    if not _profile:
        return {}
# ... 851 lines not shown

def l0_fused_step(obj, pos, neg, m_pos, v_pos, m_neg, v_neg, g_adv, adv, count, rec, cursor, tab, adv_cost, mask_cost, steps,
                  mask_wt, thresh, l0_clip=1.0 / 255.0):
    steps = int(steps)
    if obj.dim() != 4 or obj.shape[0] != 1:
        raise RuntimeError("l0_fused_step: obj must be [1,C,H,W]")
    n = obj.numel()
    for t in (obj, pos, neg, m_pos, v_pos, m_neg, v_neg, g_adv, adv):
        if t.numel() != n or t.dtype != torch.float32:
            raise RuntimeError("l0_fused_step: the patch-sized tensors must be fp32 and of one size")
    if steps < 1 or steps >= 1 << 24:
        raise RuntimeError("l0_fused_step: steps must lie in [1, 2^24)")
    if count.dtype != torch.int32 or count.numel() < 2 * steps + 1:
        raise RuntimeError("l0_fused_step: count must be int32[2 * steps + 1]")
    if rec.dtype != torch.float32 or rec.numel() < 2 * steps * L0_REC:
        raise RuntimeError("l0_fused_step: rec must hold 2 * steps records of %d floats" % L0_REC)
    if tab.dtype != torch.float32 or tab.numel() < 4 * steps:
        raise RuntimeError("l0_fused_step: tab must hold 2 * steps pairs of floats")
    if cursor.dtype != torch.int32 or cursor.numel() < 2:
        raise RuntimeError("l0_fused_step: cursor must be int32[2]")
    for name, t in (("adv_cost", adv_cost), ("mask_cost", mask_cost)):
        if t is not None and (t.numel() != 1 or t.dtype != torch.float32):
            raise RuntimeError("l0_fused_step: %s must be one fp32 value" % name)
    N.check(N.lib().dmh_l0_fused_step(N.ptr(obj), N.ptr(pos), N.ptr(neg), N.ptr(m_pos), N.ptr(v_pos), N.ptr(m_neg), N.ptr(v_neg),
                                      N.ptr(g_adv), N.ptr(adv), N.ptr(count), N.ptr(rec), N.ptr(cursor), N.ptr(tab),
                                      N.ptr(adv_cost), N.ptr(mask_cost), steps, obj.shape[1], obj.shape[2] * obj.shape[3],
                                      float(mask_wt), float(thresh), float(l0_clip), N.stream()))
    return adv


class _UpCatPad(torch.autograd.Function):
    @staticmethod
    def forward(ctx, y, skip):
        lib = N.lib()
        B, C1, h, w = y.shape
        C2 = 0 if skip is None else skip.shape[1]
        if skip is not None and tuple(skip.shape) != (B, C2, 2 * h, 2 * w):
            raise RuntimeError("up_cat_pad: skip must be [B,C2,2h,2w], got %s for y %s" % (tuple(skip.shape), tuple(y.shape)))
        out = torch.empty((B, C1 + C2, 2 * h + 2, 2 * w + 2), device=y.device, dtype=torch.float32)
        nb = 4 * (y.numel() + (0 if skip is None else skip.numel()) + out.numel())
        N.check(_timed("up_cat_pad_fwd", lambda: lib.dmh_dec_up_cat_pad_fwd(N.ptr(y), N.ptr(skip), B, C1, C2, h, w,
                                                                           N.ptr(out), N.stream()), nb))
        ctx.save_for_backward(y)
        ctx.c2 = C2
        ctx.skip_grad = skip is not None and skip.requires_grad
        return out

    @staticmethod
    def backward(ctx, g_out):
        (y,) = ctx.saved_tensors
        lib = N.lib()
        B, C1, h, w = y.shape
        g_y = torch.empty_like(y)
        g_skip = torch.empty((B, ctx.c2, 2 * h, 2 * w), device=y.device, dtype=torch.float32) if ctx.skip_grad else None
        g_out = _c(g_out)
        nb = 4 * (2 * y.numel() + g_out.numel() + (0 if g_skip is None else g_skip.numel()))
        N.check(_timed("up_cat_pad_bwd", lambda: lib.dmh_dec_up_cat_pad_bwd(N.ptr(y), N.ptr(g_out), B, C1, ctx.c2, h, w,
                                                                           N.ptr(g_y), N.ptr(g_skip), N.stream()), nb))
        return g_y, g_skip


def up_cat_pad(y, skip=None):
    return _UpCatPad.apply(_c(y), None if skip is None else _c(skip))


class _EluPad(torch.autograd.Function):
    @staticmethod
    def forward(ctx, z, apply_elu):
        lib = N.lib()
        B, Cc, H, W = z.shape
        out = torch.empty((B, Cc, H + 2, W + 2), device=z.device, dtype=torch.float32)
        N.check(_timed("elu_pad_fwd", lambda: lib.dmh_elu_pad_fwd(N.ptr(z), B, Cc, H, W, int(apply_elu), N.ptr(out),
                                                                 N.stream()), 4 * (z.numel() + out.numel())))
        ctx.save_for_backward(z)
        ctx.apply_elu = int(apply_elu)
        return out

    @staticmethod
    def backward(ctx, g_out):
        (z,) = ctx.saved_tensors
        lib = N.lib()
        B, Cc, H, W = z.shape
        g_z = torch.empty_like(z)
        g_out = _c(g_out)
        N.check(_timed("elu_pad_bwd", lambda: lib.dmh_elu_pad_bwd(N.ptr(z), N.ptr(g_out), B, Cc, H, W, ctx.apply_elu,
                                                                 N.ptr(g_z), N.stream()), 4 * (2 * z.numel() + g_out.numel())))
        return g_z, None


def elu_pad(z, apply_elu=True):
    return _EluPad.apply(_c(z), bool(apply_elu))


class _BnAct(torch.autograd.Function):
    @staticmethod
    def forward(ctx, x, scale, shift, residual, relu):
        lib = N.lib()
        B, Cc = x.shape[0], x.shape[1]
        HW = x.numel() // (B * Cc)
        if scale.numel() != Cc or shift.numel() != Cc:
            raise RuntimeError("bn_act: scale/shift must have %d entries" % Cc)
        if residual is not None and residual.shape != x.shape:
            raise RuntimeError("bn_act: residual %s does not match x %s" % (tuple(residual.shape), tuple(x.shape)))
        out = torch.empty_like(x)
        nb = 4 * (x.numel() * (2 if residual is None else 3))
        N.check(_timed("bn_act_fwd", lambda: lib.dmh_bn_act_fwd(N.ptr(x), N.ptr(scale), N.ptr(shift), N.ptr(residual), B,
                                                               Cc, HW, int(relu), N.ptr(out), N.stream()), nb))
        ctx.save_for_backward(out if relu else None, scale)
        ctx.relu = int(relu)
        ctx.res_grad = residual is not None and residual.requires_grad
        ctx.x_grad = x.requires_grad
        return out

    @staticmethod
    def backward(ctx, g_out):
        out, scale = ctx.saved_tensors
        lib = N.lib()
        g_out = _c(g_out)
        B, Cc = g_out.shape[0], g_out.shape[1]
        HW = g_out.numel() // (B * Cc)
        g_x = torch.empty_like(g_out)
        g_res = torch.empty_like(g_out) if ctx.res_grad else None
        nb = 4 * g_out.numel() * (2 + (1 if ctx.relu else 0) + (1 if ctx.res_grad else 0))
        N.check(_timed("bn_act_bwd", lambda: lib.dmh_bn_act_bwd(N.ptr(out), N.ptr(g_out), N.ptr(scale), B, Cc, HW, ctx.relu,
                                                               N.ptr(g_x), N.ptr(g_res), N.stream()), nb))
        return g_x, None, None, g_res, None


def _reject_affine_grad(name, scale, shift):
    if torch.is_grad_enabled() and not _wino_frozen and (scale.requires_grad or shift.requires_grad):
        raise RuntimeError("%s: scale/shift require grad, but this op treats them as constants (eval-mode BatchNorm "
                           "inside an attack); use the nn.BatchNorm2d module path, ops.frozen_weights() or detach()" % name)


def bn_act(x, scale, shift, residual=None, relu=True):
    _reject_affine_grad("bn_act", scale, shift)
    return _BnAct.apply(_c(x), _c(scale.detach()), _c(shift.detach()), None if residual is None else _c(residual),
                        bool(relu))


def _bn_train_stats(x, bn):
    lib = N.lib()
    B, Cc = x.shape[0], x.shape[1]
    HW = x.numel() // (B * Cc)
    dev = x.device
    part = torch.empty(lib.dmh_bn_stats_partials_size(B, Cc, HW), device=dev, dtype=torch.float32)
    scale, shift, mean, invstd = (torch.empty(Cc, device=dev, dtype=torch.float32) for _ in range(4))
    if bn.momentum is None:
        raise RuntimeError("bn_act_train: cumulative-average BatchNorm (momentum=None) is not supported")
    track = bn.track_running_stats and bn.running_mean is not None
    nbt = bn.num_batches_tracked if (track and bn.num_batches_tracked is not None) else None
    if nbt is not None and not (nbt.is_cuda and nbt.dtype == torch.int64 and nbt.numel() == 1):
        raise RuntimeError("bn_act_train: num_batches_tracked must be a CUDA int64 scalar")
    N.check(_timed("bn_train_stats", lambda: lib.dmh_bn_train_stats_tracked(
        N.ptr(x), B, Cc, HW, N.ptr(None if bn.weight is None else _c(bn.weight.detach())),
        N.ptr(None if bn.bias is None else _c(bn.bias.detach())), float(bn.momentum), float(bn.eps),
        N.ptr(bn.running_mean if track else None), N.ptr(bn.running_var if track else None),
        None if nbt is None else C.c_void_p(nbt.data_ptr()), N.ptr(part), N.ptr(scale),
        N.ptr(shift), N.ptr(mean), N.ptr(invstd), N.stream()), 4 * x.numel()))
    return scale, shift, mean, invstd


def _bn_backward(g_pre, x, weight, bn, mean, invstd, eps, mask):
    if all(mask) and weight is not None and hasattr(torch.ops.aten, "miopen_batch_norm_backward"):
        return torch.ops.aten.miopen_batch_norm_backward(x, g_pre, weight, bn.running_mean, bn.running_var, mean, invstd, eps)
    return torch.ops.aten.native_batch_norm_backward(g_pre, x, weight, bn.running_mean, bn.running_var, mean, invstd, True,
                                                     eps, mask)


def channel_sum(g):
    lib = N.lib()
    B, Cc = g.shape[0], g.shape[1]
    HW = g.numel() // (B * Cc)
    part = torch.empty(lib.dmh_channel_sum_partials_size(B, Cc, HW), device=g.device, dtype=torch.float32)
    out = torch.empty(Cc, device=g.device, dtype=torch.float32)
    N.check(_timed("channel_sum", lambda: lib.dmh_channel_sum(N.ptr(g), B, Cc, HW, N.ptr(part), N.ptr(out), N.stream()),
                   4 * g.numel()))
    return out


BN_BWD_ENABLED = os.environ.get("DMH_BN_BWD", "1") != "0"


def _bn_backward_fused(g, x, out, weight, mean, invstd, want_pre):
    lib = N.lib()
    B, Cc = g.shape[0], g.shape[1]
    HW = g.numel() // (B * Cc)
    ws = torch.empty(lib.dmh_bn_train_bwd_workspace_size(B, Cc, HW), device=g.device, dtype=torch.float32)
    gx = torch.empty_like(g)
    gw = torch.empty(Cc, device=g.device, dtype=torch.float32)
    gb = torch.empty(Cc, device=g.device, dtype=torch.float32)
    g_pre = torch.empty_like(g) if want_pre else None
    nb = 4 * g.numel() * ((6 if out is not None else 4) + 1 + (1 if want_pre else 0))
    N.check(_timed("bn_train_bwd", lambda: lib.dmh_bn_train_bwd(
        N.ptr(x), N.ptr(g), N.ptr(out), N.ptr(weight), N.ptr(mean), N.ptr(invstd), B, Cc, HW, N.ptr(ws), N.ptr(gx), N.ptr(gw),
        N.ptr(gb), N.ptr(g_pre), N.stream()), nb))
    return gx, gw, gb, g_pre


class _BnActTrain(torch.autograd.Function):

    @staticmethod
    def forward(ctx, x, weight, bias, residual, relu, bn):
        lib = N.lib()
        scale, shift, mean, invstd = _bn_train_stats(x, bn)
        B, Cc = x.shape[0], x.shape[1]
        HW = x.numel() // (B * Cc)
        out = torch.empty_like(x)
        nb = 4 * (x.numel() * (2 if residual is None else 3))
        N.check(_timed("bn_act_fwd", lambda: lib.dmh_bn_act_fwd(N.ptr(x), N.ptr(scale), N.ptr(shift), N.ptr(residual), B, Cc,
                                                               HW, int(relu), N.ptr(out), N.stream()), nb))
        ctx.save_for_backward(x, weight, mean, invstd, out if relu else None)
        ctx.relu, ctx.eps, ctx.bn = bool(relu), float(bn.eps), bn
        ctx.res_grad = residual is not None and residual.requires_grad
        return out

    @staticmethod
    def backward(ctx, g):
        x, weight, mean, invstd, out = ctx.saved_tensors
        lib = N.lib()
        g = _c(g)
        B, Cc = g.shape[0], g.shape[1]
        if BN_BWD_ENABLED and weight is not None and g.numel() < (1 << 31) and Cc <= 65535:
            gx, gw, gb, g_pre = _bn_backward_fused(g, x, out if ctx.relu else None, weight, mean, invstd,
                                                   ctx.res_grad and ctx.relu)
            if ctx.res_grad and not ctx.relu:
                g_pre = g
            return gx, gw, gb, (g_pre if ctx.res_grad else None), None, None
        if ctx.relu:
            ones = frozen_memo(("ones", Cc, g.device), lambda: torch.ones(Cc, device=g.device, dtype=torch.float32))
            g_pre = torch.empty_like(g)
            N.check(_timed("bn_act_bwd", lambda: lib.dmh_bn_act_bwd(N.ptr(out), N.ptr(g), N.ptr(ones), B, Cc,
                                                                   g.numel() // (B * Cc), 1, N.ptr(g_pre), None, N.stream()),
                           12 * g.numel()))
        else:
            g_pre = g
        gx, gw, gb = _bn_backward(g_pre, x, weight, ctx.bn, mean, invstd, ctx.eps,
                                  [ctx.needs_input_grad[0], weight is not None and ctx.needs_input_grad[1],
                                   weight is not None and ctx.needs_input_grad[2]])
        return gx, gw, gb, (g_pre if ctx.res_grad else None), None, None


def bn_act_train(bn, x, residual=None, relu=True):
    return _BnActTrain.apply(_c(x), bn.weight, bn.bias, None if residual is None else _c(residual), bool(relu), bn)


class _StemBnReluPool(torch.autograd.Function):
    @staticmethod
    def forward(ctx, x, scale, shift):
        lib = N.lib()
        B, Cc, H, W = x.shape
        feat = torch.empty_like(x)
        pooled = torch.empty((B, Cc, H // 2, W // 2), device=x.device, dtype=torch.float32)
        arg = torch.empty((B, Cc, H // 2, W // 2), device=x.device, dtype=torch.uint8)
        nb = 4 * (2 * x.numel() + pooled.numel()) + arg.numel()
        N.check(_timed("stem_fwd", lambda: lib.dmh_stem_bn_relu_pool_fwd(N.ptr(x), N.ptr(scale), N.ptr(shift), B, Cc, H, W,
                                                                        N.ptr(feat), N.ptr(pooled), N.ptr(arg),
                                                                        N.stream()), nb))
        ctx.save_for_backward(feat, arg, scale)
        ctx.mark_non_differentiable(arg)
        ctx.set_materialize_grads(False)
        return feat, pooled, arg

    @staticmethod
    def backward(ctx, g_feat, g_pooled, _g_arg):
        feat, arg, scale = ctx.saved_tensors
        if g_feat is None and g_pooled is None:
            return None, None, None
        lib = N.lib()
        B, Cc, H, W = feat.shape
        g_feat = None if g_feat is None else _c(g_feat)
        g_pooled = None if g_pooled is None else _c(g_pooled)
        g_x = torch.empty_like(feat)
        nb = 4 * (2 * feat.numel() + (0 if g_feat is None else feat.numel()) +
                  (0 if g_pooled is None else g_pooled.numel())) + arg.numel()
        N.check(_timed("stem_bwd", lambda: lib.dmh_stem_bn_relu_pool_bwd(N.ptr(feat), N.ptr(arg), N.ptr(g_feat),
                                                                        N.ptr(g_pooled), N.ptr(scale), B, Cc, H, W,
                                                                        N.ptr(g_x), N.stream()), nb))
        return g_x, None, None


class _StemTrain(torch.autograd.Function):

    @staticmethod
    def forward(ctx, x, weight, bias, bn):
        lib = N.lib()
        scale, shift, mean, invstd = _bn_train_stats(x, bn)
        B, Cc, H, W = x.shape
        feat = torch.empty_like(x)
        pooled = torch.empty((B, Cc, H // 2, W // 2), device=x.device, dtype=torch.float32)
        arg = torch.empty((B, Cc, H // 2, W // 2), device=x.device, dtype=torch.uint8)
        nb = 4 * (2 * x.numel() + pooled.numel()) + arg.numel()
        N.check(_timed("stem_fwd", lambda: lib.dmh_stem_bn_relu_pool_fwd(N.ptr(x), N.ptr(scale), N.ptr(shift), B, Cc, H, W,
                                                                        N.ptr(feat), N.ptr(pooled), N.ptr(arg),
                                                                        N.stream()), nb))
        ctx.save_for_backward(x, weight, mean, invstd, feat, arg)
        ctx.eps, ctx.bn = float(bn.eps), bn
        ctx.mark_non_differentiable(arg)
        ctx.set_materialize_grads(False)
        return feat, pooled, arg

    @staticmethod
    def backward(ctx, g_feat, g_pooled, _g_arg):
        x, weight, mean, invstd, feat, arg = ctx.saved_tensors
        if g_feat is None and g_pooled is None:
            return None, None, None, None
        lib = N.lib()
        B, Cc, H, W = feat.shape
        g_feat = None if g_feat is None else _c(g_feat)
        g_pooled = None if g_pooled is None else _c(g_pooled)
        ones = frozen_memo(("ones", Cc, feat.device), lambda: torch.ones(Cc, device=feat.device, dtype=torch.float32))
        g_pre = torch.empty_like(feat)
        N.check(_timed("stem_bwd", lambda: lib.dmh_stem_bn_relu_pool_bwd(N.ptr(feat), N.ptr(arg), N.ptr(g_feat),
                                                                        N.ptr(g_pooled), N.ptr(ones), B, Cc, H, W,
                                                                        N.ptr(g_pre), N.stream()), 12 * feat.numel()))
        if BN_BWD_ENABLED and weight is not None and g_pre.numel() < (1 << 31) and Cc <= 65535:
            gx, gw, gb, _ = _bn_backward_fused(g_pre, x, None, weight, mean, invstd, False)
            return gx, gw, gb, None
        gx, gw, gb = _bn_backward(g_pre, x, weight, ctx.bn, mean, invstd, ctx.eps,
                                  [ctx.needs_input_grad[0], weight is not None and ctx.needs_input_grad[1],
                                   weight is not None and ctx.needs_input_grad[2]])
        return gx, gw, gb, None


def stem_bn_relu_pool_train(bn, x):
    feat, pooled, _ = _StemTrain.apply(_c(x), bn.weight, bn.bias, bn)
    return feat, pooled


def stem_bn_relu_pool(x, scale, shift):
    _reject_affine_grad("stem_bn_relu_pool", scale, shift)
    feat, pooled, _ = _StemBnReluPool.apply(_c(x), _c(scale.detach()), _c(shift.detach()))
    return feat, pooled


WINO_ENABLED = os.environ.get("DMH_WINO", "1") != "0"
WRW_ENABLED = os.environ.get("DMH_WRW", "1") != "0"
_wino_frozen = 0
_wino_cache = {}


@contextlib.contextmanager
def frozen_weights():
    global _wino_frozen
    _wino_frozen += 1
    try:
        yield
    finally:
        _wino_frozen -= 1
# ... 17 lines not shown
    lib = N.lib()
    K, Cc = weight.shape[0], weight.shape[1]
    key = (weight.data_ptr(), weight._version, bool(backward), None if scale is None else scale.data_ptr())
    if _wino_frozen and key in _wino_cache:
        return _wino_cache[key]
    if scale is None and not _wino_frozen:
        ready = _wino_ready.get((key[0], key[2]))
        if ready is not None and ready[0] == key[1] and ready[1].device == weight.device:
            return ready[1]
    n_out, n_in = (Cc, K) if backward else (K, Cc)
    U = torch.empty(lib.dmh_wino_weight_size(n_out, n_in), device=weight.device, dtype=torch.float32)
    N.check(lib.dmh_wino_weight_transform_scaled(N.ptr(_c(weight.detach())), K, Cc, int(backward), N.ptr(scale), N.ptr(U),
                                                 N.stream()))
    if _wino_frozen:
        _wino_cache[key] = U
    return U


WINO_PREFETCH = os.environ.get("DMH_WINO_PREFETCH", "1") != "0"
_wino_ready = {}


def wino_prefetch(jobs, fresh=False):
    if not (WINO_ENABLED and WINO_PREFETCH):
        return 0
    lib = N.lib()
    todo, keep = [], []
    if fresh and not _wino_frozen:
        _wino_ready.clear()
    for weight, backward, scale in jobs:
        if not (weight.is_cuda and weight.dtype == torch.float32 and weight.dim() == 4 and tuple(weight.shape[2:]) == (3, 3)):
            continue
        K, Cc = weight.shape[0], weight.shape[1]
        n_out, n_in = (Cc, K) if backward else (K, Cc)
        if n_in % 8 or n_in < 24 or n_out < 64:
            continue
        if scale is not None and not _wino_frozen:
            continue
        sc = None if scale is None else _c(scale.detach())
        key = (weight.data_ptr(), weight._version, bool(backward), None if sc is None else sc.data_ptr())
        if _wino_frozen and key in _wino_cache:
            continue
        U = torch.empty(lib.dmh_wino_weight_size(n_out, n_in), device=weight.device, dtype=torch.float32)
        w = _c(weight.detach())
        keep.append((w, sc))
        todo.append((N.ptr(w), N.ptr(sc), N.ptr(U), K, Cc, int(bool(backward))))
        if _wino_frozen:
            _wino_cache[key] = U
        else:
            _wino_ready[(key[0], key[2])] = (key[1], U, weight)
    if todo:
        arr = (N.WinoWtJob * len(todo))()
        for j, (w, sc, U, K, Cc, bw) in enumerate(todo):
            arr[j].w, arr[j].scale, arr[j].U, arr[j].K, arr[j].C, arr[j].backward = w, sc, U, K, Cc, bw
        N.check(lib.dmh_wino_weight_transform_batch(arr, len(todo), N.stream()))
    return len(todo)


WINO_SK = os.environ.get("DMH_WINO_SK", "1") != "0"
_WINO_MIN_ITEMS = int(os.environ.get("DMH_WINO_MIN_ITEMS", "64"))
_WINO_MIN_FILL = float(os.environ.get("DMH_WINO_MIN_FILL", "0.5"))


def _wino_ok(B, n_in, n_out, Ho, Wo, allow_split=True, allow_sk=False):
    if not WINO_ENABLED or n_in % 8 or n_in < 24 or n_out < 64 or Ho % 2 or Wo % 2 or Ho < 2 or Wo < 2:
        return False
    if B * n_in * (Ho + 2) * (Wo + 2) >= (1 << 30):
        return False
    if n_in < 64 and n_out % 64:
        return False
    ht, wt = Ho // 2, Wo // 2
    narrow = wt % 32 != 0 and (wt <= 16 or (-wt) % 16 < (-wt) % 32)
    if narrow:
        flat = 5 * ht <= 4 * (-(-ht // 4) * 4)
        rows = -(-(B * ht) // 4) * 4 if flat else B * -(-ht // 4) * 4
        cols = -(-wt // 16) * 16
    else:
        rows, cols = B * -(-ht // 2) * 2, -(-wt // 32) * 32
    if B * ht * wt < _WINO_MIN_FILL * rows * cols:
        return False
    regions = (rows // (4 if narrow else 2)) * (cols // (16 if narrow else 32))
    regions *= -(-n_out // 64)
    nch = n_in // 8
    split = 2 if (allow_split and regions < 192 and nch % 2 == 0 and nch >= 6) else 1
    if WINO_SK and (allow_split or allow_sk) and regions * nch >= 8 * _WINO_MIN_ITEMS:
        try:
            ws_floats = _sk_ws_floats(torch.cuda.current_device()) if torch.cuda.is_available() else 2 * 256 * _SK_SLOT_FLOATS
        except Exception:
            ws_floats = 2 * 256 * _SK_SLOT_FLOATS
        plan = N.lib().dmh_wino_conv3x3_plan(B, n_in, n_out, Ho, Wo, 1, 0 if allow_split else 1, ws_floats)
        if plan >= 0 and (plan & 1):
            return True
    return regions * split >= (_WINO_MIN_ITEMS if WINO_SK else max(_WINO_MIN_ITEMS, 200))


def _wrw_ok(x, g, K, Cc):
    if not WINO_ENABLED or not WRW_ENABLED or g.shape[2] % 2 or g.shape[3] % 2:
        return False
    if K % 64 == 0 and Cc % 64 == 0:
        kch, cch = 64, 64
    elif K % 32 == 0 and Cc % 96 == 0:
        kch, cch = 32, 96
    elif K % 32 == 0 and Cc % 64 == 0:
        kch, cch = 32, 64
    else:
        return False
    pad = (g.shape[2] + 2 - x.shape[2]) // 2
    if pad not in (0, 1) or (pad == 1 and x.shape[3] % 16):
        return False
    if x.numel() * 4 > 0xFFFFFF00 or g.numel() >= (1 << 30):
        return False
    chunks = g.shape[0] * (g.shape[2] // 2) * -(-(g.shape[3] // 2) // 8)
    return chunks * (K // kch) * (Cc // cch) >= 1024


def _wino32_ok(B, n_in, n_out, Ho, Wo):
    if (not WINO_ENABLED or n_in % 8 or n_in < 32 or n_out % 32 or n_out % 64 == 0 or n_out > 96 or Ho % 2 or Wo % 2
            or B * n_in * (Ho + 2) * (Wo + 2) >= (1 << 30)):
        return False
    ht, wt = Ho // 2, Wo // 2
    rows, cols = -(-ht // 4) * 4, -(-wt // 32) * 32
    if ht * wt < 0.8 * rows * cols:
        return False
    return B * (rows // 4) * (cols // 32) * (n_out // 32) >= 400


def _wino32_filter(weight, backward):
    lib = N.lib()
    K, Cc = weight.shape[0], weight.shape[1]
    key = (weight.data_ptr(), weight._version, bool(backward), "k17")
    if _wino_frozen and key in _wino_cache:
        return _wino_cache[key]
    n_out, n_in = (Cc, K) if backward else (K, Cc)
    U = torch.empty(lib.dmh_wino32_weight_size(n_out, n_in), device=weight.device, dtype=torch.float32)
    N.check(lib.dmh_wino32_weight_transform(N.ptr(_c(weight.detach())), K, Cc, int(backward), N.ptr(U), N.stream()))
    if _wino_frozen:
        _wino_cache[key] = U
    return U


def _wino32_conv(x, U, bias, K, pad):
    lib = N.lib()
    B, Cc, H, W = x.shape
    y = torch.empty((B, K, H + 2 * pad - 2, W + 2 * pad - 2), device=x.device, dtype=torch.float32)
    nb = 4 * (x.numel() + y.numel()) + 4 * U.numel()
    ws = _sk_workspace(x.device) if WINO_SK else None
    N.check(_timed("wino32_conv3x3", lambda: lib.dmh_wino32_conv3x3_ws(
        N.ptr(x), N.ptr(U), N.ptr(bias), B, Cc, K, H, W, pad, N.ptr(y), N.ptr(ws), 0 if ws is None else ws.numel(), N.stream()),
        nb, 18 * Cc * y.numel()))
    return y


_sk_ws = {}
_SK_SLOT_FLOATS = 16384


def _sk_ws_floats(device):
    return 2 * torch.cuda.get_device_properties(device).multi_processor_count * _SK_SLOT_FLOATS


def _sk_workspace(device):
    key = (device.index if device.index is not None else torch.cuda.current_device(), torch.cuda.current_stream(device).cuda_stream)
    ws = _sk_ws.get(key)
    if ws is None:
        ws = _sk_ws[key] = torch.empty(_sk_ws_floats(device), device=device, dtype=torch.float32)
    return ws


def _k10_act(lib, x, U, bias, res, relu, B, Cc, K, H, W, pad, y, stream):
    if not WINO_SK:
        return lib.dmh_wino_conv3x3_act(x, U, bias, res, relu, B, Cc, K, H, W, pad, y, stream)
    ws = _sk_workspace(torch.device("cuda", torch.cuda.current_device()))
    return lib.dmh_wino_conv3x3_act_ws(x, U, bias, res, relu, B, Cc, K, H, W, pad, y, N.ptr(ws), ws.numel(), stream)


def _wino_conv(x, U, bias, K, pad):
    lib = N.lib()
    B, Cc, H, W = x.shape
    y = torch.empty((B, K, H + 2 * pad - 2, W + 2 * pad - 2), device=x.device, dtype=torch.float32)
    nb = 4 * (x.numel() + y.numel()) + 4 * U.numel()
    ws = _sk_workspace(x.device) if WINO_SK else None
    N.check(_timed("wino_conv3x3", lambda: lib.dmh_wino_conv3x3_ws(
        N.ptr(x), N.ptr(U), N.ptr(bias), B, Cc, K, H, W, pad, N.ptr(y), N.ptr(ws), 0 if ws is None else ws.numel(), N.stream()),
        nb, 18 * Cc * y.numel()))
    return y


def _small_ok(n_in, n_out):
    return WINO_ENABLED and ((n_in in (1, 2, 3, 4, 16) and n_out <= 32) or (n_in == 32 and n_out <= 16))


def _small_conv(x, weight, bias, pad, backward):
    lib = N.lib()
    if x.numel() >= (1 << 30):
        if backward:
            return torch.nn.functional.conv_transpose2d(x, weight, None, 1, 2 - pad)
        return torch.conv2d(x, weight, bias, 1, pad)
    B, _, H, W = x.shape
    Kw, Cw = weight.shape[0], weight.shape[1]
    n_out = Cw if backward else Kw
    y = torch.empty((B, n_out, H + 2 * pad - 2, W + 2 * pad - 2), device=x.device, dtype=torch.float32)
    nb = 4 * (x.numel() + y.numel())
    N.check(_timed("conv3x3_small", lambda: lib.dmh_conv3x3_small(N.ptr(x), N.ptr(_c(weight.detach())), N.ptr(bias), B, Kw,
                                                                 Cw, H, W, pad, int(backward), N.ptr(y), N.stream()), nb,
                   18 * x.shape[1] * y.numel()))
    return y


class _Conv3x3(torch.autograd.Function):
    @staticmethod
    def forward(ctx, x, weight, bias, pad):
        B, Cc, H, W = x.shape
        K = weight.shape[0]
        ctx.pad = pad
        ctx.has_bias = bias is not None
        ctx.params_const = _wino_frozen > 0
        ctx.save_for_backward(x, weight)
        if _wino_ok(B, Cc, K, H + 2 * pad - 2, W + 2 * pad - 2):
            return _wino_conv(x, _wino_filter(weight, False), None if bias is None else _c(bias.detach()), K, pad)
        if _wino32_ok(B, Cc, K, H + 2 * pad - 2, W + 2 * pad - 2):
            return _wino32_conv(x, _wino32_filter(weight, False), None if bias is None else _c(bias.detach()), K, pad)
        if WINO_ENABLED and K == 1 and ((pad == 0 and Cc % 4 == 0) or (
                Cc % 16 == 0 and Cc >= 32 and B * -(-(H + 2 * pad - 2) // 8) * -(-(W + 2 * pad - 2) // 64) >= 512)):
            lib = N.lib()
            y = torch.empty((B, 1, H + 2 * pad - 2, W + 2 * pad - 2), device=x.device, dtype=torch.float32)
            N.check(_timed("conv3x3_head", lambda: lib.dmh_conv3x3_head(
                N.ptr(x), N.ptr(_c(weight.detach())), N.ptr(None if bias is None else _c(bias.detach())), B, Cc, H, W, pad,
                N.ptr(y), N.stream()), 4 * (x.numel() + y.numel())))
            return y
        if _small_ok(Cc, K):
            return _small_conv(x, weight, None if bias is None else _c(bias.detach()), pad, False)
        return torch.conv2d(x, weight, bias, 1, pad)

    @staticmethod
    def backward(ctx, g):
        x, weight = ctx.saved_tensors
        B, Cc, H, W = x.shape
        K = weight.shape[0]
        pad = ctx.pad
        g = _c(g)
        need_x = ctx.needs_input_grad[0]
        need_w = ctx.needs_input_grad[1] and not ctx.params_const
        need_b = ctx.has_bias and ctx.needs_input_grad[2] and not ctx.params_const
        g_x = g_w = g_b = None
        if need_x and _wino_ok(B, K, Cc, H, W):
            g_x = _wino_conv(g, _wino_filter(weight, True), None, Cc, 2 - pad)
            need_x = False
        elif need_x and _wino32_ok(B, K, Cc, H, W):
            g_x = _wino32_conv(g, _wino32_filter(weight, True), None, Cc, 2 - pad)
            need_x = False
        elif need_x and K == 1 and pad == 0 and Cc % 4 == 0 and Cc <= 64 and H >= 3 and W >= 3 and WINO_ENABLED:
            lib = N.lib()
            g_x = torch.empty_like(x)
            N.check(_timed("conv3x3_head_bwd", lambda: lib.dmh_conv3x3_head_bwd_data(
                N.ptr(g), N.ptr(_c(weight.detach())), B, Cc, H, W, N.ptr(g_x), N.stream()), 4 * (g_x.numel() + g.numel())))
            need_x = False
        elif need_x and _small_ok(K, Cc):
            g_x = _small_conv(g, weight, None, 2 - pad, True)
            need_x = False
        if need_w and K == 1 and WINO_ENABLED and Cc * H * W < (1 << 29):
            lib = N.lib()
            part = torch.empty(lib.dmh_conv3x3_head_wrw_partials_size(B, Cc, H, W, pad), device=g.device, dtype=torch.float32)
            g_w = torch.empty_like(weight)
            g_b = torch.empty(1, device=g.device, dtype=torch.float32) if need_b else None
            N.check(_timed("conv3x3_head_wrw", lambda: lib.dmh_conv3x3_head_wrw(
                N.ptr(x), N.ptr(g), B, Cc, H, W, pad, N.ptr(part), N.ptr(g_w), N.ptr(g_b), N.stream()),
                4 * (x.numel() + g.numel())))
            need_w = need_b = False
        if need_w and K == 16 and Cc in (16, 32) and WINO_ENABLED and Cc * H * W < (1 << 28):
            lib = N.lib()
            part = torch.empty(lib.dmh_conv3x3_small_wrw_partials_size(Cc), device=g.device, dtype=torch.float32)
            g_w = torch.empty_like(weight)
            g_b = torch.empty(16, device=g.device, dtype=torch.float32) if need_b else None
            N.check(_timed("conv3x3_small_wrw", lambda: lib.dmh_conv3x3_small_wrw(
                N.ptr(x), N.ptr(g), B, Cc, H, W, pad, N.ptr(part), N.ptr(g_w), N.ptr(g_b), N.stream()),
                4 * (x.numel() + g.numel()), 2 * 9 * 16 * Cc * g.numel() // 16))
            need_w = need_b = False
        if need_w and _wrw_ok(x, g, K, Cc):
            lib = N.lib()
            ws = torch.empty(lib.dmh_wino_wrw_workspace_size(B, Cc, K, H, W, pad), device=g.device, dtype=torch.float32)
            g_w = torch.empty_like(weight)
            N.check(_timed("wino_wrw", lambda: lib.dmh_wino_wrw(N.ptr(x), N.ptr(g), B, Cc, K, H, W, pad, N.ptr(ws), N.ptr(g_w),
                                                                N.stream()), 4 * (x.numel() + g.numel()), 18 * Cc * g.numel()))
            if need_b:
                g_b = channel_sum(g) if K <= 65535 else g.sum((0, 2, 3))
            need_w = need_b = False
        if need_x or need_w or need_b:
            r = torch.ops.aten.convolution_backward(g, x, weight, [K] if ctx.has_bias else None, [1, 1], [pad, pad], [1, 1],
                                                    False, [0, 0], 1, [need_x, need_w, need_b])
            g_x = r[0] if need_x else g_x
            g_w = r[1] if need_w else g_w
            g_b = r[2] if need_b else g_b
        return g_x, g_w, g_b, None


class _ConvBnAct(torch.autograd.Function):

    @staticmethod
    def forward(ctx, x, weight, scale, shift, residual, relu, pad):
        K = weight.shape[0]
        lib = N.lib()
        B, Cc, H, W = x.shape
        y = torch.empty((B, K, H + 2 * pad - 2, W + 2 * pad - 2), device=x.device, dtype=torch.float32)
        U = _wino_filter(weight, False, scale)
        nb = 4 * (x.numel() + y.numel() * (1 if residual is None else 2)) + 4 * U.numel()
        N.check(_timed("wino_conv3x3", lambda: _k10_act(lib, N.ptr(x), N.ptr(U), N.ptr(shift), N.ptr(residual),
                                                                       int(relu), B, Cc, K, H, W, pad, N.ptr(y),
                                                                       N.stream()), nb, 18 * Cc * y.numel()))
        ctx.save_for_backward(x, weight, scale, y if relu else None)
        ctx.pad, ctx.relu = pad, bool(relu)
        ctx.res_grad = residual is not None and residual.requires_grad
        ctx.params_const = _wino_frozen > 0
        return y

    @staticmethod
    def backward(ctx, g):
        x, weight, scale, y = ctx.saved_tensors
        lib = N.lib()
        B, Cc, H, W = x.shape
# ... 342 lines not shown
                           lambda: _c((wd * sd.view(-1, 1, 1, 1)).reshape(Co, Cin).t()))
        g_x = torch.empty((B, Cin, H, W), device=g.device, dtype=torch.float32)
        N.check(_timed("down_conv_bwd", lambda: _k15_bwd(lib, g1, g2, w3ts, wdts, g_skip, B, Cin, Co, H, W, g_x, N.stream()),
                       4 * (g_x.numel() * (1 if g_skip is None else 2) + 2 * g.numel()), 20 * Cin * g.numel()))
        return (g_x,) + (None,) * 10


DOWN_NODE_ENABLED = os.environ.get("DMH_DOWN_NODE", "1") != "0"


def down_block_eval_ok(x, w3, wd, w2):
    if not (_wino_frozen > 0 and DOWN_NODE_ENABLED and down_convs_ok(x, w3, wd)):
        return False
    Co = w3.shape[0]
    return tuple(w2.shape) == (Co, Co, 3, 3) and _wino_ok(x.shape[0], Co, Co, x.shape[2] // 2, x.shape[3] // 2, allow_split=False,
                                                         allow_sk=True)


def down_block_eval(x, w3, scale1, shift1, wd, scale_d, shift_d, w2, scale2, shift2, return_skip=False):
    if not down_block_eval_ok(x, w3, wd, w2):
        raise RuntimeError("down_block_eval: needs ops.frozen_weights() and shapes K15 / K10 take (ops.down_block_eval_ok)")
    for sc, sh in ((scale1, shift1), (scale_d, shift_d), (scale2, shift2)):
        _reject_affine_grad("down_block_eval", sc, sh)
    d = lambda t: _c(t.detach())
    x = _c(x)
    args = (x, w3.detach(), d(scale1), d(shift1), wd.detach(), d(scale_d), d(shift_d), w2.detach(), d(scale2), d(shift2))
    if not x.requires_grad:
        with torch.no_grad():
            y, _ = _DownBlockEval.apply(*args, False)
        return (y, x) if return_skip else y
    y, skip = _DownBlockEval.apply(*args, bool(return_skip))
    return (y, skip) if return_skip else y


ROI_ENABLED = os.environ.get("DMH_ROI", "1") != "0"


def _conv_any(x, weight, bias, pad, backward=False):
    B, n_in, H, W = x.shape
    n_out = weight.shape[1] if backward else weight.shape[0]
    Ho, Wo = H + 2 * pad - 2, W + 2 * pad - 2
    if WINO_ENABLED and x.numel() < (1 << 30):
        if not backward and n_out == 1 and pad == 0 and n_in % 4 == 0:
            y = torch.empty((B, 1, Ho, Wo), device=x.device, dtype=torch.float32)
            N.check(_timed("conv3x3_head", lambda: N.lib().dmh_conv3x3_head(
                N.ptr(x), N.ptr(_c(weight.detach())), N.ptr(bias), B, n_in, H, W, 0, N.ptr(y), N.stream()),
                4 * (x.numel() + y.numel())))
            return y
        if backward and n_in == 1 and pad == 2 and n_out % 4 == 0 and n_out <= 64 and Ho >= 3 and Wo >= 3:
            y = torch.empty((B, n_out, Ho, Wo), device=x.device, dtype=torch.float32)
            N.check(_timed("conv3x3_head_bwd", lambda: N.lib().dmh_conv3x3_head_bwd_data(
                N.ptr(x), N.ptr(_c(weight.detach())), B, n_out, Ho, Wo, N.ptr(y), N.stream()), 4 * (x.numel() + y.numel())))
            return y
        if _small_ok(n_in, n_out):
            return _small_conv(x, weight, bias, pad, backward)
        if n_in % 8 == 0 and n_in >= 24 and Ho % 2 == 0 and Wo % 2 == 0 and Ho >= 2 and Wo >= 2:
            if n_out % 32 == 0 and n_out % 64 and n_out <= 96:
                return _wino32_conv(x, _wino32_filter(weight, backward), bias, n_out, pad)
            if n_out >= 64:
                return _wino_conv(x, _wino_filter(weight, backward), bias, n_out, pad)
    if backward:
        return torch.nn.functional.conv_transpose2d(x, weight, None, 1, 2 - pad)
    return torch.conv2d(x, weight, bias, 1, pad)


def _roi_glue_args(y, y_org, skip, skip_org, dst_org, size, frame, up, elu):
    a = N.RoiGlueArgs()
    a.y, a.skip = N.ptr(y), N.ptr(skip)
    a.y_org, a.skip_org, a.dst_org = N.ptr(y_org), N.ptr(skip_org), N.ptr(dst_org)
    a.B, a.C1, a.C2 = y.shape[0], y.shape[1], (0 if skip is None else skip.shape[1])
    a.sh, a.sw = y.shape[2], y.shape[3]
    a.kh, a.kw = (0, 0) if skip is None else (skip.shape[2], skip.shape[3])
    a.hc, a.wc = size
    a.H, a.W = frame
    a.up, a.elu = int(up), int(elu)
    return a


def _roi_glue_fwd(a, device):
    out = torch.empty((a.B, a.C1 + a.C2, a.hc + 2, a.wc + 2), device=device, dtype=torch.float32)
    N.check(_timed("roi_glue_fwd", lambda: N.lib().dmh_roi_glue_fwd(C.byref(a), N.ptr(out), N.stream()), 8 * out.numel()))
    return out


def _roi_glue_bwd(a, g_out, device, want_skip, y_region=None, skip_region=None, skip_prezero=True):
    if y_region is not None and a.sh * a.sw < 3 * y_region[1][0] * y_region[1][1]:
        y_region = None
    if skip_region is not None and skip_prezero and a.kh * a.kw < 3 * skip_region[1][0] * skip_region[1][1]:
        skip_region = None
    new = torch.zeros if y_region is not None else torch.empty
    g_y = new((a.B, a.C1, a.sh, a.sw), device=device, dtype=torch.float32)
    g_skip = None
    if want_skip:
        new = torch.zeros if (skip_region is not None and skip_prezero) else torch.empty
        g_skip = new((a.B, a.C2, a.kh, a.kw), device=device, dtype=torch.float32)
    yo, (yh, yw) = y_region if y_region is not None else (None, (0, 0))
    ko, (kh, kw) = skip_region if (skip_region is not None and want_skip) else (None, (0, 0))
    nb = 4 * (g_out.numel() + 2 * a.B * a.C1 * (yh * yw if yo is not None else a.sh * a.sw) +
              (0 if g_skip is None else a.B * a.C2 * (kh * kw if ko is not None else a.kh * a.kw)))
    N.check(_timed("roi_glue_bwd", lambda: N.lib().dmh_roi_glue_bwd(C.byref(a), N.ptr(g_out), N.ptr(g_y), N.ptr(g_skip),
                                                                   N.ptr(yo), yh, yw, N.ptr(ko), kh, kw, N.stream()), nb))
    return g_y, g_skip


from .roi import STAGES as _ROI_STAGES, TABLE as _ROI_NAMES

ROI_DEPTH = int(os.environ.get("DMH_ROI_DEPTH", "4"))
_ROI_CHANNELS = {"d": (1, 16), "z01": (16, 16), "y00": (16, 32), "z11": (32, 96), "y10": (32, 64), "z21": (64, 128),
                 "y20": (64, 128), "z31": (128, 256), "y30": (128, 256), "z41": (256, 512)}


def _roi_chain(depth):
    names = [st[0] for st in _ROI_STAGES]
    return list(reversed(_ROI_STAGES[:names.index("z%d1" % depth) + 1]))


class _RoiTail(torch.autograd.Function):

    @staticmethod
    def _glue(chain, k, src, feats, org, sz, H0, W0, f0_compact):
        name, lvl, up, skip = chain[k]
        src_org = None if k == 0 else org[chain[k - 1][0]]
        skip_org = org["hz"] if (skip == 0 and f0_compact) else None
        return _roi_glue_args(src, src_org, None if skip is None else feats[skip], skip_org, org[name], sz[name],
                              (H0 >> lvl, W0 >> lvl), up, 1)

    @staticmethod
    def forward(ctx, plan, depth, x_top, *rest):
        lib = N.lib()
        dev = x_top.device
        depth, sign = (depth if isinstance(depth, tuple) else (depth, 1.0))
        feats, mask, tab = rest[:depth], rest[depth], rest[depth + 1]
        wb = rest[depth + 2:]
        chain = _roi_chain(depth)
        B = x_top.shape[0]
        H0, W0 = x_top.shape[2] << (depth + 1), x_top.shape[3] << (depth + 1)
        f0c = bool(plan.f0_compact)
        if (any(tuple(f.shape[2:]) != ((H0 >> (k + 1), W0 >> (k + 1)) if (k or not f0c) else plan.size["hz"])
                for k, f in enumerate(feats))
                or tuple(mask.shape) != (B, 1, H0, W0) or plan.B != B or (plan.H, plan.W) != (H0, W0)):
            raise RuntimeError("roi tail: feature / mask / plan shapes do not match")
        org = {n: tab[k] for k, n in enumerate(_ROI_NAMES)}
        sz = plan.size
        outs, src = [], x_top
        for k in range(len(chain)):
            a = _RoiTail._glue(chain, k, src, feats, org, sz, H0, W0, f0c)
            src = _conv_any(_roi_glue_fwd(a, dev), wb[2 * k], wb[2 * k + 1], 0)
            outs.append(src)
        d_pre = outs.pop()
        hd, wd_ = sz["d"]
        sig = torch.empty_like(d_pre)
        part = torch.empty(lib.dmh_roi_cost_partials_size(B, hd, wd_), device=dev, dtype=torch.float32)
        cost = torch.empty((), device=dev, dtype=torch.float32)
        N.check(lib.dmh_roi_cost_fwd_scaled(N.ptr(d_pre), N.ptr(mask), N.ptr(org["d"]), B, hd, wd_, H0, W0, sign, N.ptr(sig),
                                            N.ptr(part), N.ptr(cost), N.stream()))
        ctx.save_for_backward(x_top, mask, tab, sig, *feats, *outs, *wb[0::2])
        ctx.plan, ctx.depth, ctx.f0c, ctx.sign = plan, depth, f0c, sign
        return cost

    @staticmethod
    def backward(ctx, g):
        plan, depth = ctx.plan, ctx.depth
        sv = ctx.saved_tensors
        x_top, mask, tab, sig = sv[:4]
        chain = _roi_chain(depth)
        n = len(chain)
        feats, outs, ws = sv[4:4 + depth], sv[4 + depth:4 + depth + n - 1], sv[4 + depth + n - 1:]
        lib = N.lib()
        dev = x_top.device
        B = x_top.shape[0]
        H0, W0 = plan.H, plan.W
        org = {nm: tab[k] for k, nm in enumerate(_ROI_NAMES)}
        sz = plan.size
        hd, wd_ = sz["d"]
        g_cur = torch.empty_like(sig)
        N.check(lib.dmh_roi_cost_bwd_scaled(N.ptr(sig), N.ptr(mask), N.ptr(org["d"]), B, hd, wd_, H0, W0, ctx.sign,
                                            N.ptr(_c(g.to(torch.float32))), N.ptr(g_cur), N.stream()))
        g_feats = [None] * depth
        for k in range(n - 1, -1, -1):
            name, lvl, up, skip = chain[k]
            src = x_top if k == 0 else outs[k - 1]
            a = _RoiTail._glue(chain, k, src, feats, org, sz, H0, W0, ctx.f0c)
            want_skip = skip is not None and ctx.needs_input_grad[3 + skip]
            y_reg = ("r_y%d0" % lvl) if k == 0 else None
            s_reg = None if (skip is None or (skip == 0 and ctx.f0c)) else "r_f%d" % skip
            g_cur, g_skip = _roi_glue_bwd(a, _conv_any(g_cur, ws[k], None, 2, True), dev, want_skip,
                                          y_region=None if y_reg is None else (org[y_reg], sz[y_reg]),
                                          skip_region=None if s_reg is None else (org[s_reg], sz[s_reg]),
                                          skip_prezero=not (skip == 0 and plan.head_windowed))
            if skip is not None:
                g_feats[skip] = g_skip
        return (None, None, g_cur) + tuple(g_feats) + (None,) * (2 + 2 * n)


def roi_tail_ok(x_top, feats, convs, depth):
    if depth not in (2, 3, 4) or len(feats) != depth:
        return False
    chain = _roi_chain(depth)
    shapes = [tuple(c.weight.shape) for c in convs]
    return (ROI_ENABLED and _wino_frozen > 0 and x_top.is_cuda and all(t.dtype == torch.float32 for t in (x_top,) + tuple(feats))
            and shapes == [_ROI_CHANNELS[st[0]] + (3, 3) for st in chain]
            and x_top.shape[1] == _ROI_CHANNELS["z%d1" % depth][0]
            and all(f.shape[1] == _ROI_CHANNELS["z%d1" % (k + 1)][1] - _ROI_CHANNELS["z%d1" % (k + 1)][0] for k, f in enumerate(feats))
            and x_top.shape[2] >= 2 and x_top.shape[3] >= 2)


def roi_tail_cost(x_top, feats, mask, plan, tab, convs, negate=False):
    depth = plan.depth
    feats = tuple(feats)
    if not roi_tail_ok(x_top, feats, convs, depth):
        raise RuntimeError("roi_tail_cost: needs ops.frozen_weights(), fp32 CUDA tensors and the Monodepth2 decoder tail")
    if tab.dtype != torch.int32 or tuple(tab.shape) != (len(_ROI_NAMES), x_top.shape[0], 2):
        raise RuntimeError("roi_tail_cost: origin table must be int32 [%d, B, 2] (roi.TABLE)" % len(_ROI_NAMES))
    wb = []
    for c in convs:
        wb += [c.weight.detach(), None if c.bias is None else _c(c.bias.detach())]
    return _RoiTail.apply(plan, (depth, -1.0) if negate else depth, _c(x_top), *[_c(f) for f in feats], _c(mask), _c(tab), *wb)


def _roi_crop(src, gate, g, org, size):
    ref = src if src is not None else gate
    B, Cc, H, W = ref.shape
    out = torch.empty((B, Cc) + tuple(size), device=ref.device, dtype=torch.float32)
    N.check(_timed("roi_crop", lambda: N.lib().dmh_roi_crop(N.ptr(src), N.ptr(gate), N.ptr(g), N.ptr(org), B, Cc, H, W, size[0],
                                                           size[1], 0, N.ptr(out), N.stream()),
                   4 * out.numel() * (2 + (gate is not None))))
    return out


class _EncHeadEval(torch.autograd.Function):

    @staticmethod
    def forward(ctx, x, plan, tab, w_stem, s0, b0, w1a, s1a, b1a, w2a, s2a, b2a, w1b, s1b, b1b, w2b, s2b, b2b):
        lib = N.lib()
        B, _, H, W = x.shape
        dev = x.device
        st = N.stream()
        z = torch.empty((B, 64, H // 2, W // 2), device=dev, dtype=torch.float32)
        N.check(_timed("stem_conv_fwd", lambda: lib.dmh_stem_conv_norm_fwd(N.ptr(x), N.ptr(_c(w_stem)), B, H, W, 0.45, 0.225,
                                                                          N.ptr(z), st), 4 * (x.numel() + z.numel()),
                       2 * 147 * z.numel()))
        f0 = torch.empty_like(z)
        pooled = torch.empty((B, 64, H // 4, W // 4), device=dev, dtype=torch.float32)
        arg = torch.empty((B, 64, H // 4, W // 4), device=dev, dtype=torch.uint8)
        N.check(_timed("stem_fwd", lambda: lib.dmh_stem_bn_relu_pool_fwd(N.ptr(z), N.ptr(s0), N.ptr(b0), B, 64, H // 2, W // 2,
                                                                        N.ptr(f0), N.ptr(pooled), N.ptr(arg), st),
                       4 * (2 * z.numel() + pooled.numel()) + arg.numel()))
        del z

        def conv_act(inp, w, s, b, res):
            y = torch.empty_like(inp)
            N.check(_timed("wino_conv3x3", lambda: lib.dmh_wino_conv3x3_act(
                N.ptr(inp), N.ptr(_wino_filter(w, False, s)), N.ptr(b), N.ptr(res), 1, B, 64, 64, H // 4, W // 4, 1, N.ptr(y), st),
                4 * (2 + (res is not None)) * inp.numel(), 18 * 64 * inp.numel()))
            return y

        o1a = conv_act(pooled, w1a, s1a, b1a, None)
        ya = conv_act(o1a, w2a, s2a, b2a, pooled)
        o1b = conv_act(ya, w1b, s1b, b1b, None)
        f1 = conv_act(o1b, w2b, s2b, b2b, ya)
        ctx.save_for_backward(f0, arg, s0, o1a, ya, o1b, f1, tab, w_stem, w1a, s1a, w2a, s2a, w1b, s1b, w2b, s2b)
        ctx.plan, ctx.img = plan, (H, W)
        ctx.set_materialize_grads(False)
        return f0, f1

    @staticmethod
    def backward(ctx, g_f0, g_f1):
        f0, arg, s0, o1a, ya, o1b, f1, tab, w_stem, w1a, s1a, w2a, s2a, w1b, s1b, w2b, s2b = ctx.saved_tensors
        plan, (H, W) = ctx.plan, ctx.img
        lib = N.lib()
        dev = f0.device
        B = f0.shape[0]
        st = N.stream()
        org = {n: tab[k] for k, n in enumerate(_ROI_NAMES)}
        sz = plan.size
        hq, wq = sz["l1"]
        if g_f1 is None:
            g_pool = torch.zeros((B, 64, hq, wq), device=dev, dtype=torch.float32)
        else:
            def conv_bwd(g, w, s, res, flag):
                y = torch.empty_like(g)
                N.check(_timed("wino_conv3x3", lambda: lib.dmh_wino_conv3x3_act(
                    N.ptr(g), N.ptr(_wino_filter(w, True, s)), None, N.ptr(res), flag, B, 64, 64, hq, wq, 1, N.ptr(y), st),
                    4 * 3 * g.numel(), 18 * 64 * g.numel()))
                return y

            g2b = _roi_crop(_c(g_f1), f1, None, org["l1"], (hq, wq))
            g1b = conv_bwd(g2b, w2b, s2b, _roi_crop(o1b, None, None, org["l1"], (hq, wq)), 2)
            g_ya = conv_bwd(g1b, w1b, s1b, g2b, 0)
            g2a = _roi_crop(None, ya, g_ya, org["l1"], (hq, wq))
            g1a = conv_bwd(g2a, w2a, s2a, _roi_crop(o1a, None, None, org["l1"], (hq, wq)), 2)
            g_pool = conv_bwd(g1a, w1a, s1a, g2a, 0)
        hs, ws = sz["gz"]
        g_z = torch.empty((B, 64, hs, ws), device=dev, dtype=torch.float32)
        N.check(_timed("stem_bwd_win", lambda: lib.dmh_stem_bn_relu_pool_bwd_win(
            N.ptr(f0), N.ptr(arg), N.ptr(None if g_f0 is None else _c(g_f0)), N.ptr(g_pool), N.ptr(s0), N.ptr(org["gz"]),
            N.ptr(org["l1"]), B, 64, H // 2, W // 2, hs, ws, hq, wq, N.ptr(g_z), st), 4 * 4 * g_z.numel()))
        w_s = frozen_memo(("stem_w_over_std", w_stem.data_ptr(), w_stem._version, 0.225),
                          lambda: _c(w_stem.detach() * (1.0 / 0.225)))
        g_x = torch.zeros((B, 3, H, W), device=dev, dtype=torch.float32)
        hd, wd = sz["d"]
        N.check(_timed("stem_conv_bwd_win", lambda: lib.dmh_conv7x7s2_bwd_data_win(
            N.ptr(g_z), N.ptr(w_s), N.ptr(org["d"]), N.ptr(org["gz"]), B, 64, 3, H, W, hd, wd, hs, ws, N.ptr(g_x), st),
            4 * (g_z.numel() + B * 3 * hd * wd), 2 * 147 * 64 * B * (hd // 2) * (wd // 2)))
        return (g_x,) + (None,) * 17


def encoder_head_ok(x, conv1_weight, blocks):
# ... 448 lines not shown
```

include/dmh_hip.h:

```cpp
#ifndef DMH_HIP_H
#define DMH_HIP_H

#include <stdint.h>

#ifdef __cplusplus
extern "C" {
#endif

#define DMH_OK 0
#define DMH_EINVAL 1
#define DMH_ELAUNCH 2

#define DMH_MAX_SCALES 4
#define DMH_MAX_FRAMES 4

#define DMH_VARIANT_MD2 0
#define DMH_VARIANT_DH 1

#define DMH_NOISE_NONE 0
#define DMH_NOISE_TENSOR 1
#define DMH_NOISE_PHILOX 2

#define DMH_FIN_LOSS 0
#define DMH_FIN_LOSS_S 1
// ... 66 lines not shown
int64_t dmh_smooth_partials_size(const dmh_smooth_args* a);
int dmh_smooth_loss_fwd(const dmh_smooth_args* a, float* partials, void* stream);
int dmh_smooth_loss_bwd(const dmh_smooth_args* a, const float* gvec, const float* sstats,
                        float smooth_wt, float* const g_disp[DMH_MAX_SCALES], int accumulate, void* stream);

int dmh_loss_finalize(const float* photo_partials, const float* smooth_partials, int B, int H, int W,
                      const dmh_smooth_args* sm, int variant, float smooth_wt, float* fin, float* sstats,
                      void* stream);

#define DMH_PASTE_COMPOSITE 0
#define DMH_PASTE_WARP_ONLY 1

typedef struct dmh_paste_args {
    const float* scene;
    int64_t scene_bstride;
    const float* patch;
    const float* pmask;
    const float* coeffs;
    int N, SH, SW, PH, PW, OH, OW;
    int l_pad, t_pad;
    int mode;
    const int32_t* flip;
    const int32_t* scene_index;
} dmh_paste_args;

int dmh_eot_paste_fwd(const dmh_paste_args* a, float* adv, float* mask_out, void* stream);
int dmh_eot_paste_bwd(const dmh_paste_args* a, const float* g_adv, float* g_patch, void* stream);

int dmh_pgd_linf_step(const float* x, const float* x0, const float* g, float alpha, float eps, float* out,
                      int64_t n, void* stream);

#define DMH_APGD_REC 16
int dmh_apgd_step(float* x_adv, float* x_old, const float* x0, const float* grad, const float* ctl, int32_t* cursor,
                  int steps, float eps, int64_t n, void* stream);
int dmh_apgd_commit(float* x_adv, const float* g_new, float* grad, float* x_best, float* grad_best, float* x_ret,
                    const float* loss, float* ctl, float* hist, int32_t* cursor, int steps, int size_decr, int steps_min,
                    double rho, int64_t n, void* stream);

#define DMH_L0_REC 8
int dmh_l0_fused_step(const float* obj, float* pos, float* neg, float* m_pos, float* v_pos, float* m_neg, float* v_neg,
                      const float* g_adv, float* adv, int32_t* count, float* rec, int32_t* cursor, const float* tab,
                      const float* adv_cost, const float* mask_cost, int steps, int C, int HW, float mask_wt, float thresh,
                      float l0_clip, void* stream);

#define DMH_LIGHT_REC 10
int dmh_tube_light_compose(const double* table, const int32_t* index, const uint8_t* base, float* out, int n_queries, int H,
                           int W, void* stream);
int dmh_tube_light_commit(const float* cost_in, float* cost, float* best, int32_t* state, int n_queries, void* stream);

int dmh_gauss_blur_windows(const float* obj, const double* weights, const int32_t* radii, float* tmp, float* windows, int steps,
                           int wstride, int C, int H, int W, int r0, int r1, int c0, int c1, void* stream);
int dmh_gauss_blur_compose(const float* windows, const int32_t* index, const float* obj, float* out, int steps, int C, int H,
                           int W, int r0, int r1, int c0, int c1, void* stream);

int dmh_square_propose(const float* x0, float* x_best, float* x_new, const int32_t* table, const float* stripes,
                       const int32_t* state, int n_queries, int C, int H, int W, float eps, void* stream);

int64_t dmh_pgd_l2_workspace_size(int64_t n);
int dmh_pgd_l2_step(const float* x, const float* x0, const float* g, double alpha, double eps, float* out, int64_t n,
                    void* workspace, int64_t workspace_bytes, void* stream);

#define DMH_EIGEN_REC 8
#define DMH_EIGEN_CHUNK 8192
#define DMH_EIGEN_MAX_BATCH 64
int64_t dmh_eigen_select_ws_size(int n);
int64_t dmh_eigen_partials_size(int grid);
int dmh_eigen_gt_stats(const float* gt, int64_t gt_len, const int32_t* table, const int32_t* blk_img, int n_images, int n_blocks,
                       int first, int n, int b0, int grid, int eigen, uint32_t* ws, float* med, int32_t* count, void* stream);
int dmh_eigen_pred_depth(const float* pred, const float* flip, int h, int w, const float* gt, int64_t gt_len, const int32_t* table,
                         const int32_t* blk_img, int n_images, int n_blocks, int first, int n, int b0, int grid, int eigen,
                         float factor, int64_t px0, float* depth, int64_t depth_len, uint32_t* ws, void* stream);
int dmh_eigen_pred_ratio(const float* depth, int64_t depth_len, int64_t px0, int64_t gt_len, const int32_t* table,
                         const int32_t* blk_img, int n_images, int n_blocks, int first, int n, int b0, int grid, uint32_t* ws,
                         const float* med_gt, float* med_pred, float* ratio, void* stream);
int dmh_eigen_metrics(const float* gt, int64_t gt_len, const float* depth, int64_t depth_len, int64_t px0, const int32_t* table,
                      const int32_t* blk_img, int n_images, int n_blocks, int first, int n, int b0, int grid, const float* ratio,
                      float* partials, float* errors, void* stream);

int dmh_l0_compose_fwd(const float* obj, const float* pos, const float* neg, int C, int HW, float l0_clip,
                       int finalize, float* adv, int32_t* l0_count, void* stream);
int dmh_l0_compose_bwd(const float* obj, const float* pos, const float* neg, const float* g_adv, int C, int HW,
                       float* g_pos, float* g_neg, int accumulate, void* stream);
int64_t dmh_l0_mask_partials_size(int HW);
int dmh_l0_mask_cost_fwd(const float* pos, const float* neg, int C, int HW, float* partials, float* cost,
                         void* stream);
int dmh_l0_mask_cost_bwd(const float* pos, const float* neg, int C, int HW, const float* gscale,
                         const float* weight, float* g_pos, float* g_neg, int accumulate, void* stream);

int64_t dmh_sq_mean_partials_size(int64_t n);
int dmh_masked_sq_mean_fwd(const float* disp, const float* mask, int64_t n, float* partials, float* cost,
                           void* stream);
int dmh_masked_sq_mean_bwd(const float* disp, const float* mask, int64_t n, const float* gscale, float* g_disp,
                           void* stream);

int dmh_gt_depth_mse_fwd(const float* disp, const float* disp_gt, const float* objmask, int64_t mask_bstride,
                         const float* objdepth, int B, int64_t HW, float min_depth, float max_depth, float* partials,
                         float* cost, void* stream);
int dmh_gt_depth_mse_bwd(const float* disp, const float* disp_gt, const float* objmask, int64_t mask_bstride,
                         const float* objdepth, int B, int64_t HW, float min_depth, float max_depth, const float* gscale,
                         float* g_disp, void* stream);

int64_t dmh_down_wrw_workspace_size(int B, int C, int K, int H, int W);
int dmh_down_wrw(const float* x, const float* g3, const float* gd, int B, int C, int K, int H, int W, float* workspace, float* dw3,
                 float* dwd, void* stream);
int64_t dmh_stem_wrw_workspace_size(int B, int H, int W);
int dmh_stem_wrw(const float* x, const float* g, int B, int H, int W, float mean, float std, float* workspace, float* dw,
                 void* stream);

int dmh_ssim_map(const float* x, const float* y, int planes, int H, int W, float* out, void* stream);
int dmh_ssim_map_bwd(const float* x, const float* y, const float* g_out, int planes, int H, int W, float* workspace, float* g_x,
                     float* g_y, void* stream);
int dmh_avg_pyramid(const float* x, int planes, int H, int W, float* out1, float* out2, float* out3, void* stream);
int64_t dmh_edge_smooth_partials_size(int B, int H, int W);
int dmh_edge_smooth(const float* disp, const float* img, int B, int C, int H, int W, float* partials, float* out, void* stream);
int dmh_edge_smooth_bwd(const float* disp, const float* img, int B, int C, int H, int W, const float* gscale, float* g_disp,
                        void* stream);

int64_t dmh_depth_errors_partials_size(int64_t n);
int dmh_masked_depth_errors(const float* disp_gt, const float* disp_pred, const float* mask, int64_t n,
                            float min_depth, float max_depth, float scale, float clamp_lo, float clamp_hi,
                            float* partials, float* out8, void* stream);

int dmh_dec_up_cat_pad_fwd(const float* y, const float* skip, int B, int C1, int C2, int h, int w, float* out,
                           void* stream);
int dmh_dec_up_cat_pad_bwd(const float* y, const float* g_out, int B, int C1, int C2, int h, int w, float* g_y,
                           float* g_skip, void* stream);
int dmh_elu_pad_fwd(const float* z, int B, int C, int H, int W, int apply_elu, float* out, void* stream);
int dmh_elu_pad_bwd(const float* z, const float* g_out, int B, int C, int H, int W, int apply_elu, float* g_z,
                    void* stream);

typedef struct dmh_roi_glue_args {
    const float* y;
    const float* skip;
    const int* y_org;
    const int* skip_org;
    const int* dst_org;
    int B, C1, C2;
    int sh, sw;
    int kh, kw;
    int hc, wc;
    int H, W;
    int up, elu;
} dmh_roi_glue_args;
int dmh_roi_glue_fwd(const dmh_roi_glue_args* a, float* out, void* stream);
int dmh_roi_glue_bwd(const dmh_roi_glue_args* a, const float* g_out, float* g_y, float* g_skip, const int* y_reg_org,
                     int y_reg_h, int y_reg_w, const int* skip_reg_org, int skip_reg_h, int skip_reg_w, void* stream);
int64_t dmh_roi_cost_partials_size(int B, int hd, int wd);
int dmh_roi_cost_fwd(const float* d_pre, const float* mask, const int* org, int B, int hd, int wd, int H, int W, float* sig,
                     float* partials, float* cost, void* stream);
int dmh_roi_cost_bwd(const float* sig, const float* mask, const int* org, int B, int hd, int wd, int H, int W,
                     const float* gscale, float* g_pre, void* stream);
int dmh_roi_cost_fwd_scaled(const float* d_pre, const float* mask, const int* org, int B, int hd, int wd, int H, int W,
                            float scale, float* sig, float* partials, float* cost, void* stream);
int dmh_roi_cost_bwd_scaled(const float* sig, const float* mask, const int* org, int B, int hd, int wd, int H, int W,
                            float scale, const float* gscale, float* g_pre, void* stream);

int dmh_roi_crop(const float* src, const float* gate, const float* g, const int* org, int B, int C, int H, int W, int hc,
                 int wc, int gate_compact, float* out, void* stream);
int dmh_roi_paste(const float* src, const int* src_org, int sh, int sw, const int* win_org, int B, int C, int H, int W, int h,
                  int w, float* dst, void* stream);
int dmh_stem_bn_relu_pool_bwd_win(const float* feat, const unsigned char* argmax, const float* g_feat, const float* g_pool,
                                  const float* scale, const int* org, const int* pool_org, int B, int C, int H, int W, int hs,
                                  int ws, int hq, int wq, float* g_z, void* stream);

int dmh_bn_act_fwd(const float* x, const float* scale, const float* shift, const float* residual, int B, int C, int HW,
                   int relu, float* out, void* stream);
int dmh_bn_act_bwd(const float* out, const float* g_out, const float* scale, int B, int C, int HW, int relu, float* g_x,
                   float* g_residual, void* stream);
int64_t dmh_bn_stats_partials_size(int B, int C, int HW);
int dmh_bn_train_stats(const float* x, int B, int C, int HW, const float* weight, const float* bias, float momentum,
                       float eps, float* running_mean, float* running_var, float* partials, float* scale, float* shift,
                       float* save_mean, float* save_invstd, void* stream);
int dmh_bn_train_stats_tracked(const float* x, int B, int C, int HW, const float* weight, const float* bias, float momentum,
                               float eps, float* running_mean, float* running_var, long long* num_batches_tracked,
                               float* partials, float* scale, float* shift, float* save_mean, float* save_invstd,
                               void* stream);
int64_t dmh_channel_sum_partials_size(int B, int C, int HW);
int dmh_channel_sum(const float* g, int B, int C, int HW, float* partials, float* out, void* stream);
int64_t dmh_bn_train_bwd_workspace_size(int B, int C, int HW);
int dmh_bn_train_bwd(const float* x, const float* g_out, const float* out, const float* weight, const float* save_mean,
                     const float* save_invstd, int B, int C, int HW, float* workspace, float* g_x, float* g_weight,
                     float* g_bias, float* g_pre, void* stream);
int dmh_stem_bn_relu_pool_fwd(const float* x, const float* scale, const float* shift, int B, int C, int H, int W,
                              float* feat, float* pooled, unsigned char* argmax, void* stream);
int dmh_stem_bn_relu_pool_bwd(const float* feat, const unsigned char* argmax, const float* g_feat, const float* g_pooled,
                              const float* scale, int B, int C, int H, int W, float* g_x, void* stream);

int64_t dmh_wino_weight_size(int n_out, int n_in);
int dmh_wino_weight_transform(const float* w, int K, int C, int backward, float* U, void* stream);
int dmh_wino_conv3x3(const float* x, const float* U, const float* bias, int B, int C, int K, int H, int W, int pad,
                     float* y, void* stream);
int dmh_wino_conv3x3_ws(const float* x, const float* U, const float* bias, int B, int C, int K, int H, int W, int pad,
                        float* y, float* workspace, int64_t workspace_floats, void* stream);
int dmh_wino_conv3x3_plan(int B, int C, int K, int H, int W, int pad, int epilogue, int64_t workspace_floats);
int dmh_wino_weight_transform_scaled(const float* w, int K, int C, int backward, const float* scale, float* U,
                                     void* stream);
int dmh_wino_conv3x3_act(const float* x, const float* U, const float* bias, const float* residual, int relu, int B, int C,
                         int K, int H, int W, int pad, float* y, void* stream);
typedef struct dmh_wino_wt_job {
    const float* w;
    const float* scale;
    float* U;
    int K, C, backward;
} dmh_wino_wt_job;
int dmh_wino_weight_transform_batch(const dmh_wino_wt_job* jobs, int n, void* stream);
int dmh_wino_conv3x3_act_ws(const float* x, const float* U, const float* bias, const float* residual, int relu, int B, int C,
                            int K, int H, int W, int pad, float* y, float* workspace, int64_t workspace_floats, void* stream);

int64_t dmh_wino32_weight_size(int n_out, int n_in);
int dmh_wino32_weight_transform(const float* w, int K, int C, int backward, float* U, void* stream);
int dmh_wino32_conv3x3(const float* x, const float* U, const float* bias, int B, int C, int K, int H, int W, int pad,
                       float* y, void* stream);
int dmh_wino32_conv3x3_ws(const float* x, const float* U, const float* bias, int B, int C, int K, int H, int W, int pad,
                          float* y, float* workspace, int64_t workspace_floats, void* stream);

int64_t dmh_wino_wrw_workspace_size(int B, int C, int K, int H, int W, int pad);
int dmh_wino_wrw(const float* x, const float* dy, int B, int C, int K, int H, int W, int pad, float* workspace, float* dw,
                 void* stream);

int dmh_conv3x3_small(const float* x, const float* w, const float* bias, int B, int Kw, int Cw, int H, int W, int pad,
                      int backward, float* y, void* stream);

int dmh_conv7x7s2_bwd_data(const float* g_y, const float* w, int B, int K, int Cin, int H, int W, float* g_x,
                           void* stream);
int dmh_conv7x7s2_bwd_data_win(const float* g_y, const float* w, const int* img_org, const int* gy_org, int B, int K, int Cin,
                               int H, int W, int hwin, int wwin, int sh, int sw, float* g_x, void* stream);

int dmh_conv3x3_head(const float* x, const float* w, const float* bias, int B, int C, int H, int W, int pad, float* y,
                     void* stream);
int dmh_conv3x3_head_bwd_data(const float* g, const float* w, int B, int C, int H, int W, float* g_x, void* stream);
int64_t dmh_conv3x3_head_wrw_partials_size(int B, int C, int H, int W, int pad);
int dmh_conv3x3_head_wrw(const float* x, const float* g, int B, int C, int H, int W, int pad, float* partials, float* g_w,
                         float* g_b, void* stream);

int64_t dmh_conv3x3_small_wrw_partials_size(int C);
int dmh_conv3x3_small_wrw(const float* x, const float* g, int B, int C, int H, int W, int pad, float* partials, float* g_w,
                          float* g_b, void* stream);

int dmh_stem_conv_norm_fwd(const float* x, const float* w, int B, int H, int W, float mean, float std, float* y,
                           void* stream);
int dmh_stem_conv_norm_fwd_win(const float* x, const float* w, const int* org, int B, int H, int W, int hw, int ww, float mean,
                               float std, float* y, void* stream);

int dmh_down_conv_fwd(const float* x, const float* w3, const float* wd, int B, int Cin, int Cout, int H, int W,
                      float* y3, float* yd, void* stream);
int dmh_down_conv_fwd_act(const float* x, const float* w3, const float* wd, const float* shift3, const float* shiftd,
                          int relu3, int B, int Cin, int Cout, int H, int W, float* y3, float* yd, void* stream);
int dmh_down_conv_bwd_data(const float* g3, const float* gd, const float* w3t, const float* wdt, int B, int Cin, int Cout,
                           int H, int W, float* g_x, void* stream);
int dmh_down_conv_bwd_data_acc(const float* g3, const float* gd, const float* w3t, const float* wdt, const float* g_add, int B,
                               int Cin, int Cout, int H, int W, float* g_x, void* stream);

int64_t dmh_down_conv_image_size(int rows, int inner);
int dmh_down_conv_weight_image(const float* w3, const float* wd, int rows, int inner, float* image, void* stream);
int dmh_down_conv_fwd_img(const float* x, const float* image, int has_down, const float* shift3, const float* shiftd, int relu3,
                          int B, int Cin, int Cout, int H, int W, float* y3, float* yd, void* stream);
int dmh_down_conv_bwd_data_img(const float* g3, const float* gd, const float* image, const float* g_add, int B, int Cin, int Cout,
                               int H, int W, float* g_x, void* stream);

#ifdef __cplusplus
}
#endif
#endif
```

Before: 408.4 images/s.

## Fuse two-pass reductions via per-channel atomic tickets, dropping finalize kernels

Adds ticket counters so the last block finishing each channel's partial reduction merges the partials and writes the final BN statistics, BN-backward coefficients, channel sums or ROI cost in place. This removes the separate finalize kernel launch after each BN stats, BN backward, channel sum and ROI cost forward. The cost is atomics, fences and a serial merge done by a single wave per channel, plus ticket buffers cached per stream that must be reset correctly. Channel counts above 512 fall back to the old two-kernel path.

Result: no change. 407.8 images/s (-0.2%).

```diff
diff --git a/depthmodelhardening_amd/_native.py b/depthmodelhardening_amd/_native.py
--- a/depthmodelhardening_amd/_native.py
+++ b/depthmodelhardening_amd/_native.py
@@ -122,16 +122,21 @@
     "dmh_roi_cost_fwd": (C.c_int, [_fp, _fp, _fp] + [C.c_int] * 5 + [_fp] * 4),
     "dmh_roi_cost_bwd": (C.c_int, [_fp, _fp, _fp] + [C.c_int] * 5 + [_fp] * 3),
     "dmh_roi_cost_fwd_scaled": (C.c_int, [_fp, _fp, _fp] + [C.c_int] * 5 + [C.c_float] + [_fp] * 4),
+    "dmh_roi_cost_fwd_scaled_tk": (C.c_int, [_fp, _fp, _fp] + [C.c_int] * 5 + [C.c_float] + [_fp] * 4 + [C.c_int, _fp]),
     "dmh_roi_cost_bwd_scaled": (C.c_int, [_fp, _fp, _fp] + [C.c_int] * 5 + [C.c_float] + [_fp] * 3),
     "dmh_bn_act_fwd": (C.c_int, [_fp] * 4 + [C.c_int] * 4 + [_fp, _fp]),
     "dmh_bn_act_bwd": (C.c_int, [_fp] * 3 + [C.c_int] * 4 + [_fp, _fp, _fp]),
     "dmh_bn_stats_partials_size": (C.c_int64, [C.c_int, C.c_int, C.c_int]),
     "dmh_bn_train_stats": (C.c_int, [_fp, C.c_int, C.c_int, C.c_int, _fp, _fp, C.c_float, C.c_float] + [_fp] * 8),
     "dmh_bn_train_stats_tracked": (C.c_int, [_fp, C.c_int, C.c_int, C.c_int, _fp, _fp, C.c_float, C.c_float] + [_fp] * 9),
+    "dmh_bn_train_stats_tracked_tk": (C.c_int, [_fp, C.c_int, C.c_int, C.c_int, _fp, _fp, C.c_float, C.c_float] + [_fp] * 9
+                                      + [C.c_int, _fp]),
     "dmh_channel_sum_partials_size": (C.c_int64, [C.c_int, C.c_int, C.c_int]),
     "dmh_channel_sum": (C.c_int, [_fp, C.c_int, C.c_int, C.c_int, _fp, _fp, C.c_void_p]),
+    "dmh_channel_sum_tk": (C.c_int, [_fp, C.c_int, C.c_int, C.c_int, _fp, _fp, _fp, C.c_int, C.c_void_p]),
     "dmh_bn_train_bwd_workspace_size": (C.c_int64, [C.c_int, C.c_int, C.c_int]),
     "dmh_bn_train_bwd": (C.c_int, [_fp] * 6 + [C.c_int, C.c_int, C.c_int] + [_fp] * 5 + [C.c_void_p]),
+    "dmh_bn_train_bwd_tk": (C.c_int, [_fp] * 6 + [C.c_int, C.c_int, C.c_int] + [_fp] * 6 + [C.c_int, C.c_void_p]),
     "dmh_stem_bn_relu_pool_fwd": (C.c_int, [_fp] * 3 + [C.c_int] * 4 + [_fp] * 4),
     "dmh_stem_bn_relu_pool_bwd": (C.c_int, [_fp] * 5 + [C.c_int] * 4 + [_fp, _fp]),
     "dmh_wino_weight_size": (C.c_int64, [C.c_int, C.c_int]),
diff --git a/depthmodelhardening_amd/csrc/common.hpp b/depthmodelhardening_amd/csrc/common.hpp
--- a/depthmodelhardening_amd/csrc/common.hpp
+++ b/depthmodelhardening_amd/csrc/common.hpp
@@ -151,6 +151,38 @@
     return item * nch + c;
 }
 
+__device__ __forceinline__ void ticket_store(float* p, float v) { __hip_atomic_store(p, v, __ATOMIC_RELAXED, __HIP_MEMORY_SCOPE_AGENT); }
+__device__ __forceinline__ float ticket_load(const float* p) { return __hip_atomic_load(p, __ATOMIC_RELAXED, __HIP_MEMORY_SCOPE_AGENT); }
+__device__ __forceinline__ bool ticket_draw(int* counter, int expected) {
+    return __hip_atomic_fetch_add(counter, 1, __ATOMIC_RELAXED, __HIP_MEMORY_SCOPE_AGENT) == expected - 1;
+}
+__device__ __forceinline__ void ticket_reset(int* counter) {
+    __hip_atomic_store(counter, 0, __ATOMIC_RELAXED, __HIP_MEMORY_SCOPE_AGENT);
+}
+__device__ __forceinline__ bool ticket_last_wave(int* counter, int expected) {
+    asm volatile("s_waitcnt vmcnt(0)" ::: "memory");
+    if (expected == 1) return true;
+    int last = 0;
+    if ((threadIdx.x & (WAVE - 1)) == 0) last = ticket_draw(counter, expected) ? 1 : 0;
+    last = __builtin_amdgcn_readfirstlane(last);
+    if (last) __builtin_amdgcn_fence(__ATOMIC_ACQUIRE, "agent");
+    return last != 0;
+}
+__device__ __forceinline__ bool ticket_last_block(int* counter, int expected, int* word) {
+    asm volatile("s_waitcnt vmcnt(0)" ::: "memory");
+    __syncthreads();
+    if (threadIdx.x == 0) {
+        const int last = ticket_draw(counter, expected) ? 1 : 0;
+        if (last) {
+            __builtin_amdgcn_fence(__ATOMIC_ACQUIRE, "agent");
+            asm volatile("s_waitcnt vmcnt(0)" ::: "memory");
+        }
+        *word = last;
+    }
+    __syncthreads();
+    return *word != 0;
+}
+
 template <typename Kernel>
 inline hipError_t configure_dynamic_lds(Kernel kernel, size_t bytes, std::atomic<uint64_t>& done) {
     int dev = 0;
diff --git a/depthmodelhardening_amd/csrc/encoder_glue.hip b/depthmodelhardening_amd/csrc/encoder_glue.hip
--- a/depthmodelhardening_amd/csrc/encoder_glue.hip
+++ b/depthmodelhardening_amd/csrc/encoder_glue.hip
@@ -217,8 +217,38 @@
     return Wf{n, a.mean + d * f, a.m2 + b.m2 + d * d * a.n * f};
 }
 
+struct BnStatsFin {
+    const float* weight;
+    const float* bias;
+    float momentum, eps;
+    float* running_mean;
+    float* running_var;
+    float* scale;
+    float* shift;
+    float* save_mean;
+    float* save_invstd;
+    long long* num_batches_tracked;
+};
+template <typename Get>
+__device__ __forceinline__ Wf bn_stats_merge(int S, Get get) {
+    Wf t{0.f, 0.f, 0.f};
+    for (int s = 0; s < S; ++s) t = wf_merge(t, get(s));
+    return t;
+}
+__device__ __forceinline__ void bn_stats_finish(const Wf t, int c, const BnStatsFin& f) {
+    if (c == 0 && f.num_batches_tracked) f.num_batches_tracked[0] += 1;
+    const float var = t.m2 / t.n, invstd = rsqrtf(var + f.eps);
+    const float sc = (f.weight ? f.weight[c] : 1.f) * invstd;
+    f.scale[c] = sc;
+    f.shift[c] = (f.bias ? f.bias[c] : 0.f) - t.mean * sc;
+    f.save_mean[c] = t.mean;
+    f.save_invstd[c] = invstd;
+    if (f.running_mean) f.running_mean[c] = (1.f - f.momentum) * f.running_mean[c] + f.momentum * t.mean;
+    if (f.running_var) f.running_var[c] = (1.f - f.momentum) * f.running_var[c] + f.momentum * (t.m2 / fmaxf(t.n - 1.f, 1.f));
+}
+
 __global__ __launch_bounds__(NT) void bn_stats_partial_kernel(const float* __restrict__ x, int B, int C, int HW, int S,
-                                                              float* __restrict__ part) {
+                                                              float* part, int* tick, const BnStatsFin fin) {
     const int c = blockIdx.y, s = blockIdx.x;
     const float k = x[(size_t)c * HW];
     float nq[4] = {0.f, 0.f, 0.f, 0.f}, s1q[4] = {0.f, 0.f, 0.f, 0.f}, s2q[4] = {0.f, 0.f, 0.f, 0.f};
@@ -281,7 +311,17 @@
 #pragma unroll
         for (int i = 1; i < NT / WAVE; ++i) t = wf_merge(t, red[i]);
         float* p = part + ((size_t)c * S + s) * 3;
-        p[0] = t.n; p[1] = t.mean; p[2] = t.m2;
+        ticket_store(p, t.n); ticket_store(p + 1, t.mean); ticket_store(p + 2, t.m2);
+    }
+    if (tick && threadIdx.x < WAVE && ticket_last_wave(tick + c, S)) {
+        const int l = min((int)threadIdx.x, S - 1);
+        const float* p = part + ((size_t)c * S + l) * 3;
+        const Wf mine{ticket_load(p), ticket_load(p + 1), ticket_load(p + 2)};
+        const Wf t = bn_stats_merge(S, [&](int s) { return Wf{__shfl(mine.n, s, WAVE), __shfl(mine.mean, s, WAVE), __shfl(mine.m2, s, WAVE)}; });
+        if (threadIdx.x == 0) {
+            bn_stats_finish(t, c, fin);
+            ticket_reset(tick + c);
+        }
     }
 }
 
@@ -295,28 +335,49 @@
                                                                long long* __restrict__ num_batches_tracked) {
     const int c = blockIdx.x * NT + threadIdx.x;
     if (c >= C) return;
-    if (c == 0 && num_batches_tracked) num_batches_tracked[0] += 1;
-    Wf t{0.f, 0.f, 0.f};
+    const Wf t = bn_stats_merge(S, [&](int s) {
+        const float* p = part + ((size_t)c * S + s) * 3;
+        return Wf{ticket_load(p), ticket_load(p + 1), ticket_load(p + 2)};
+    });
+    bn_stats_finish(t, c, BnStatsFin{weight, bias, momentum, eps, running_mean, running_var, scale, shift, save_mean, save_invstd,
+                                     num_batches_tracked});
+}
+
+inline unsigned blocks_for(int64_t n) { return (unsigned)((n + NT - 1) / NT); }
+
+struct BnBwdFin {
+    double inv_n;
+    const float* weight;
+    const float* invstd;
+    float* coef;
+    float* g_weight;
+    float* g_bias;
+};
+template <typename Get>
+__device__ __forceinline__ void bn_bwd_finish(int c, int S, const float* mean, const BnBwdFin& f, bool write, Get get) {
+    double s1 = 0.0, s2 = 0.0;
     for (int s = 0; s < S; ++s) {
-        const float* p = part + ((size_t)c * S + s) * 3;
-        t = wf_merge(t, Wf{p[0], p[1], p[2]});
-    }
-    const float var = t.m2 / t.n, invstd = rsqrtf(var + eps);
-    const float sc = (weight ? weight[c] : 1.f) * invstd;
-    scale[c] = sc;
-    shift[c] = (bias ? bias[c] : 0.f) - t.mean * sc;
-    save_mean[c] = t.mean;
-    save_invstd[c] = invstd;
-    if (running_mean) running_mean[c] = (1.f - momentum) * running_mean[c] + momentum * t.mean;
-    if (running_var) running_var[c] = (1.f - momentum) * running_var[c] + momentum * (t.m2 / fmaxf(t.n - 1.f, 1.f));
-}
-
-inline unsigned blocks_for(int64_t n) { return (unsigned)((n + NT - 1) / NT); }
+        const float2 p = get(s);
+        s1 += (double)p.x;
+        s2 += (double)p.y;
+    }
+    if (!write) return;
+    const double is = (double)f.invstd[c], w = f.weight ? (double)f.weight[c] : 1.0;
+    if (f.g_bias) f.g_bias[c] = (float)s1;
+    if (f.g_weight) f.g_weight[c] = (float)(s2 * is);
+    float4 k;
+    k.x = (float)(w * is);
+    k.y = (float)(s1 * f.inv_n);
+    k.z = (float)(s2 * is * is * f.inv_n);
+    k.w = mean[c];
+    reinterpret_cast<float4*>(f.coef)[c] = k;
+}
 
 template <bool RELU, bool VEC>
 __global__ __launch_bounds__(NT) void bn_bwd_partial_kernel(const float* __restrict__ x, const float* __restrict__ g,
                                                             const float* __restrict__ out, const float* __restrict__ mean,
-                                                            int B, int C, int HW, int S, float* __restrict__ part) {
+                                                            int B, int C, int HW, int S, float* part, int* tick,
+                                                            const BnBwdFin fin) {
     const int c = blockIdx.y, s = blockIdx.x;
     const float m = mean[c];
     float a1[4] = {0.f, 0.f, 0.f, 0.f}, a2[4] = {0.f, 0.f, 0.f, 0.f};
@@ -383,8 +444,15 @@
             t1 += red[i][0];
             t2 += red[i][1];
         }
-        part[((size_t)c * S + s) * 2 + 0] = t1;
-        part[((size_t)c * S + s) * 2 + 1] = t2;
+        ticket_store(part + ((size_t)c * S + s) * 2 + 0, t1);
+        ticket_store(part + ((size_t)c * S + s) * 2 + 1, t2);
+    }
+    if (tick && threadIdx.x < WAVE && ticket_last_wave(tick + c, S)) {
+        const float* p = part + ((size_t)c * S + min((int)threadIdx.x, S - 1)) * 2;
+        const float2 mine = make_float2(ticket_load(p), ticket_load(p + 1));
+        bn_bwd_finish(c, S, mean, fin, threadIdx.x == 0,
+                      [&](int s) { return make_float2(__shfl(mine.x, s, WAVE), __shfl(mine.y, s, WAVE)); });
+        if (threadIdx.x == 0) ticket_reset(tick + c);
     }
 }
 
@@ -394,20 +462,9 @@
                                                              float* __restrict__ g_weight, float* __restrict__ g_bias) {
     const int c = blockIdx.x * NT + threadIdx.x;
     if (c >= C) return;
-    double s1 = 0.0, s2 = 0.0;
-    for (int s = 0; s < S; ++s) {
-        s1 += (double)part[((size_t)c * S + s) * 2 + 0];
-        s2 += (double)part[((size_t)c * S + s) * 2 + 1];
-    }
-    const double is = (double)invstd[c], w = weight ? (double)weight[c] : 1.0;
-    if (g_bias) g_bias[c] = (float)s1;
-    if (g_weight) g_weight[c] = (float)(s2 * is);
-    float4 k;
-    k.x = (float)(w * is);
-    k.y = (float)(s1 * inv_n);
-    k.z = (float)(s2 * is * is * inv_n);
-    k.w = mean[c];
-    reinterpret_cast<float4*>(coef)[c] = k;
+    bn_bwd_finish(c, S, mean, BnBwdFin{inv_n, weight, invstd, coef, g_weight, g_bias}, true, [&](int s) {
+        return make_float2(ticket_load(part + ((size_t)c * S + s) * 2 + 0), ticket_load(part + ((size_t)c * S + s) * 2 + 1));
+    });
 }
 
 template <bool RELU, bool RES>
@@ -457,8 +514,15 @@
                            reinterpret_cast<const float4*>(coef), (unsigned)C, (unsigned)HW, (unsigned)total, g_x, g_res);
 }
 
+template <typename Get>
+__device__ __forceinline__ float channel_sum_finish(int S, Get get) {
+    double t = 0.0;
+    for (int s = 0; s < S; ++s) t += (double)get(s);
+    return (float)t;
+}
+
 __global__ __launch_bounds__(NT) void channel_sum_partial_kernel(const float* __restrict__ g, int B, int C, int HW, int S,
-                                                                 float* __restrict__ part) {
+                                                                 float* part, int* tick, float* out) {
     const int c = blockIdx.y, s = blockIdx.x;
     float a[4] = {0.f, 0.f, 0.f, 0.f};
     if ((HW & 3) == 0) {
@@ -490,7 +554,15 @@
         float u = red[0];
 #pragma unroll
         for (int i = 1; i < NT / WAVE; ++i) u += red[i];
-        part[(size_t)c * S + s] = u;
+        ticket_store(part + (size_t)c * S + s, u);
+    }
+    if (tick && threadIdx.x < WAVE && ticket_last_wave(tick + c, S)) {
+        const float mine = ticket_load(part + (size_t)c * S + min((int)threadIdx.x, S - 1));
+        const float r = channel_sum_finish(S, [&](int s) { return __shfl(mine, s, WAVE); });
+        if (threadIdx.x == 0) {
+            out[c] = r;
+            ticket_reset(tick + c);
+        }
     }
 }
 
@@ -498,9 +570,7 @@
                                                                   float* __restrict__ out) {
     const int c = blockIdx.x * NT + threadIdx.x;
     if (c >= C) return;
-    double t = 0.0;
-    for (int s = 0; s < S; ++s) t += (double)part[(size_t)c * S + s];
-    out[c] = (float)t;
+    out[c] = channel_sum_finish(S, [&](int s) { return ticket_load(part + (size_t)c * S + s); });
 }
 
 template <bool RELU, bool RES>
@@ -580,20 +650,40 @@
                                       scale, shift, save_mean, save_invstd, stream);
 }
 
-int dmh_bn_train_stats_tracked(const float* x, int B, int C, int HW, const float* weight, const float* bias, float momentum,
-                               float eps, float* running_mean, float* running_var, long long* num_batches_tracked,
-                               float* partials, float* scale, float* shift, float* save_mean, float* save_invstd,
-                               void* stream) {
+static int bn_train_stats_common(const float* x, int B, int C, int HW, const float* weight, const float* bias, float momentum,
+                                 float eps, float* running_mean, float* running_var, long long* num_batches_tracked,
+                                 float* partials, float* scale, float* shift, float* save_mean, float* save_invstd,
+                                 int* tickets, void* stream) {
     DMH_REQUIRE(x && partials && scale && shift && save_mean && save_invstd, "null pointer");
     DMH_REQUIRE((reinterpret_cast<uintptr_t>(num_batches_tracked) & 7) == 0, "num_batches_tracked must be an aligned int64");
     DMH_REQUIRE(B > 0 && C > 0 && HW > 0 && C <= 65535, "bad sizes");
     int64_t S = ((int64_t)HW + 4 * NT - 1) / (4 * NT);
     if (S > 64) S = 64;
     hipStream_t st = (hipStream_t)stream;
-    hipLaunchKernelGGL(bn_stats_partial_kernel, dim3((unsigned)S, C), dim3(NT), 0, st, x, B, C, HW, (int)S, partials);
-    hipLaunchKernelGGL(bn_stats_finalize_kernel, dim3(blocks_for(C)), dim3(NT), 0, st, partials, C, (int)S, weight, bias,
-                       momentum, eps, running_mean, running_var, scale, shift, save_mean, save_invstd, num_batches_tracked);
+    const BnStatsFin fin{weight, bias, momentum, eps, running_mean, running_var, scale, shift, save_mean, save_invstd,
+                         num_batches_tracked};
+    hipLaunchKernelGGL(bn_stats_partial_kernel, dim3((unsigned)S, C), dim3(NT), 0, st, x, B, C, HW, (int)S, partials, tickets, fin);
+    if (!tickets)
+        hipLaunchKernelGGL(bn_stats_finalize_kernel, dim3(blocks_for(C)), dim3(NT), 0, st, partials, C, (int)S, weight, bias,
+                           momentum, eps, running_mean, running_var, scale, shift, save_mean, save_invstd, num_batches_tracked);
     return check_launch("dmh_bn_train_stats");
+}
+
+int dmh_bn_train_stats_tracked(const float* x, int B, int C, int HW, const float* weight, const float* bias, float momentum,
+                               float eps, float* running_mean, float* running_var, long long* num_batches_tracked,
+                               float* partials, float* scale, float* shift, float* save_mean, float* save_invstd,
+                               void* stream) {
+    return bn_train_stats_common(x, B, C, HW, weight, bias, momentum, eps, running_mean, running_var, num_batches_tracked,
+                                 partials, scale, shift, save_mean, save_invstd, nullptr, stream);
+}
+
+int dmh_bn_train_stats_tracked_tk(const float* x, int B, int C, int HW, const float* weight, const float* bias, float momentum,
+                                  float eps, float* running_mean, float* running_var, long long* num_batches_tracked,
+                                  float* partials, float* scale, float* shift, float* save_mean, float* save_invstd,
+                                  int* tickets, int n_tickets, void* stream) {
+    DMH_REQUIRE(tickets && n_tickets >= C, "one ticket counter per channel is required");
+    return bn_train_stats_common(x, B, C, HW, weight, bias, momentum, eps, running_mean, running_var, num_batches_tracked,
+                                 partials, scale, shift, save_mean, save_invstd, tickets, stream);
 }
 
 int64_t dmh_channel_sum_partials_size(int B, int C, int HW) {
@@ -601,15 +691,25 @@
     return S < 0 ? -1 : S / 3;
 }
 
-int dmh_channel_sum(const float* g, int B, int C, int HW, float* partials, float* out, void* stream) {
+static int channel_sum_common(const float* g, int B, int C, int HW, float* partials, float* out, int* tickets, void* stream) {
     DMH_REQUIRE(g && partials && out, "null pointer");
     DMH_REQUIRE(B > 0 && C > 0 && HW > 0 && C <= 65535, "bad sizes");
     int64_t S = ((int64_t)HW + 4 * NT - 1) / (4 * NT);
     if (S > 64) S = 64;
     hipStream_t st = (hipStream_t)stream;
-    hipLaunchKernelGGL(channel_sum_partial_kernel, dim3((unsigned)S, C), dim3(NT), 0, st, g, B, C, HW, (int)S, partials);
-    hipLaunchKernelGGL(channel_sum_finalize_kernel, dim3(blocks_for(C)), dim3(NT), 0, st, partials, C, (int)S, out);
+    hipLaunchKernelGGL(channel_sum_partial_kernel, dim3((unsigned)S, C), dim3(NT), 0, st, g, B, C, HW, (int)S, partials, tickets, out);
+    if (!tickets) hipLaunchKernelGGL(channel_sum_finalize_kernel, dim3(blocks_for(C)), dim3(NT), 0, st, partials, C, (int)S, out);
     return check_launch("dmh_channel_sum");
+}
+
+int dmh_channel_sum(const float* g, int B, int C, int HW, float* partials, float* out, void* stream) {
+    return channel_sum_common(g, B, C, HW, partials, out, nullptr, stream);
+}
+
+int dmh_channel_sum_tk(const float* g, int B, int C, int HW, float* partials, float* out, int* tickets, int n_tickets,
+                       void* stream) {
+    DMH_REQUIRE(tickets && n_tickets >= C, "one ticket counter per channel is required");
+    return channel_sum_common(g, B, C, HW, partials, out, tickets, stream);
 }
 
 int64_t dmh_bn_train_bwd_workspace_size(int B, int C, int HW) {
@@ -618,9 +718,9 @@
     return S / 3 * 2 + (int64_t)C * 4;
 }
 
-int dmh_bn_train_bwd(const float* x, const float* g_out, const float* out, const float* weight, const float* save_mean,
-                     const float* save_invstd, int B, int C, int HW, float* workspace, float* g_x, float* g_weight,
-                     float* g_bias, float* g_pre, void* stream) {
+static int bn_train_bwd_common(const float* x, const float* g_out, const float* out, const float* weight, const float* save_mean,
+                               const float* save_invstd, int B, int C, int HW, float* workspace, float* g_x, float* g_weight,
+                               float* g_bias, float* g_pre, int* tickets, void* stream) {
     DMH_REQUIRE(x && g_out && save_mean && save_invstd && workspace && g_x, "null pointer");
     DMH_REQUIRE(B > 0 && C > 0 && HW > 0 && C <= 65535, "bad sizes");
     const int64_t total = (int64_t)B * C * HW;
@@ -633,15 +733,17 @@
     float* part = workspace + (size_t)C * 4;
     const dim3 pg((unsigned)S, C);
     const bool vec = (HW & 3) == 0;
+    const BnBwdFin fin{1.0 / ((double)B * (double)HW), weight, save_invstd, coef, g_weight, g_bias};
     if (out) {
-        if (vec) hipLaunchKernelGGL((bn_bwd_partial_kernel<true, true>), pg, dim3(NT), 0, st, x, g_out, out, save_mean, B, C, HW, (int)S, part);
-        else hipLaunchKernelGGL((bn_bwd_partial_kernel<true, false>), pg, dim3(NT), 0, st, x, g_out, out, save_mean, B, C, HW, (int)S, part);
+        if (vec) hipLaunchKernelGGL((bn_bwd_partial_kernel<true, true>), pg, dim3(NT), 0, st, x, g_out, out, save_mean, B, C, HW, (int)S, part, tickets, fin);
+        else hipLaunchKernelGGL((bn_bwd_partial_kernel<true, false>), pg, dim3(NT), 0, st, x, g_out, out, save_mean, B, C, HW, (int)S, part, tickets, fin);
     } else {
-        if (vec) hipLaunchKernelGGL((bn_bwd_partial_kernel<false, true>), pg, dim3(NT), 0, st, x, g_out, out, save_mean, B, C, HW, (int)S, part);
-        else hipLaunchKernelGGL((bn_bwd_partial_kernel<false, false>), pg, dim3(NT), 0, st, x, g_out, out, save_mean, B, C, HW, (int)S, part);
-    }
-    hipLaunchKernelGGL(bn_bwd_finalize_kernel, dim3(blocks_for(C)), dim3(NT), 0, st, part, C, (int)S,
-                       1.0 / ((double)B * (double)HW), weight, save_mean, save_invstd, coef, g_weight, g_bias);
+        if (vec) hipLaunchKernelGGL((bn_bwd_partial_kernel<false, true>), pg, dim3(NT), 0, st, x, g_out, out, save_mean, B, C, HW, (int)S, part, tickets, fin);
+        else hipLaunchKernelGGL((bn_bwd_partial_kernel<false, false>), pg, dim3(NT), 0, st, x, g_out, out, save_mean, B, C, HW, (int)S, part, tickets, fin);
+    }
+    if (!tickets)
+        hipLaunchKernelGGL(bn_bwd_finalize_kernel, dim3(blocks_for(C)), dim3(NT), 0, st, part, C, (int)S, fin.inv_n, weight,
+                           save_mean, save_invstd, coef, g_weight, g_bias);
     if (out) {
         if (g_pre) launch_bn_bwd_apply<true, true>(x, g_out, out, coef, C, HW, total, g_x, g_pre, st);
         else launch_bn_bwd_apply<true, false>(x, g_out, out, coef, C, HW, total, g_x, nullptr, st);
@@ -650,6 +752,21 @@
         else launch_bn_bwd_apply<false, false>(x, g_out, out, coef, C, HW, total, g_x, nullptr, st);
     }
     return check_launch("dmh_bn_train_bwd");
+}
+
+int dmh_bn_train_bwd(const float* x, const float* g_out, const float* out, const float* weight, const float* save_mean,
+                     const float* save_invstd, int B, int C, int HW, float* workspace, float* g_x, float* g_weight,
+                     float* g_bias, float* g_pre, void* stream) {
+    return bn_train_bwd_common(x, g_out, out, weight, save_mean, save_invstd, B, C, HW, workspace, g_x, g_weight, g_bias, g_pre,
+                               nullptr, stream);
+}
+
+int dmh_bn_train_bwd_tk(const float* x, const float* g_out, const float* out, const float* weight, const float* save_mean,
+                        const float* save_invstd, int B, int C, int HW, float* workspace, float* g_x, float* g_weight,
+                        float* g_bias, float* g_pre, int* tickets, int n_tickets, void* stream) {
+    DMH_REQUIRE(tickets && n_tickets >= C, "one ticket counter per channel is required");
+    return bn_train_bwd_common(x, g_out, out, weight, save_mean, save_invstd, B, C, HW, workspace, g_x, g_weight, g_bias, g_pre,
+                               tickets, stream);
 }
 
 int dmh_stem_bn_relu_pool_fwd(const float* x, const float* scale, const float* shift, int B, int C, int H, int W,
diff --git a/depthmodelhardening_amd/csrc/roi_glue.hip b/depthmodelhardening_amd/csrc/roi_glue.hip
--- a/depthmodelhardening_amd/csrc/roi_glue.hip
+++ b/depthmodelhardening_amd/csrc/roi_glue.hip
@@ -300,10 +300,24 @@
     }
 }
 
+__device__ __forceinline__ void roi_cost_finish(const float* partials, int nblk, double n, float* cost, double* s_red) {
+    double acc = 0.0;
+    for (int i = threadIdx.x; i < nblk; i += NT) acc += (double)ticket_load(partials + i);
+    s_red[threadIdx.x] = acc;
+    __syncthreads();
+    for (int o = NT / 2; o > 0; o >>= 1) {
+        if ((int)threadIdx.x < o) s_red[threadIdx.x] += s_red[threadIdx.x + o];
+        __syncthreads();
+    }
+    if (threadIdx.x == 0) cost[0] = (float)(s_red[0] / n);
+}
+
 __global__ __launch_bounds__(NT) void roi_cost_fwd_kernel(const float* __restrict__ d_pre, const float* __restrict__ mask,
                                                           const int* __restrict__ org, int hd, int wd, int H, int W,
-                                                          float* __restrict__ sig, float* __restrict__ partials) {
-    __shared__ float s_red[NT / WAVE];
+                                                          float* __restrict__ sig, float* partials, int* tick, double n_div,
+                                                          float* cost) {
+    __shared__ double s_fin[NT];
+    float* s_red = reinterpret_cast<float*>(s_fin);
     const int b = blockIdx.y, n = hd * wd;
     const int oy = org[2 * b], ox = org[2 * b + 1];
     float acc = 0.f;
@@ -315,21 +329,20 @@
         acc += v * v;
     }
     const float r = block_sum<NT>(acc, s_red);
-    if (threadIdx.x == 0) partials[blockIdx.y * gridDim.x + blockIdx.x] = r;
+    if (threadIdx.x == 0) ticket_store(partials + blockIdx.y * gridDim.x + blockIdx.x, r);
+    if (tick == nullptr) return;
+    const int nblk = (int)(gridDim.x * gridDim.y);
+    if (ticket_last_block(tick, nblk, reinterpret_cast<int*>(s_fin))) {
+        __syncthreads();
+        roi_cost_finish(partials, nblk, n_div, cost, s_fin);
+        if (threadIdx.x == 0) ticket_reset(tick);
+    }
 }
 
 __global__ __launch_bounds__(NT) void roi_cost_finalize_kernel(const float* __restrict__ partials, int nblk, double n,
                                                                float* __restrict__ cost) {
     __shared__ double s_red[NT];
-    double acc = 0.0;
-    for (int i = threadIdx.x; i < nblk; i += NT) acc += (double)partials[i];
-    s_red[threadIdx.x] = acc;
-    __syncthreads();
-    for (int o = NT / 2; o > 0; o >>= 1) {
-        if ((int)threadIdx.x < o) s_red[threadIdx.x] += s_red[threadIdx.x + o];
-        __syncthreads();
-    }
-    if (threadIdx.x == 0) cost[0] = (float)(s_red[0] / n);
+    roi_cost_finish(partials, nblk, n, cost, s_red);
 }
 
 __global__ __launch_bounds__(NT) void roi_cost_bwd_kernel(const float* __restrict__ sig, const float* __restrict__ mask,
@@ -430,17 +443,30 @@
     return dmh_roi_cost_fwd_scaled(d_pre, mask, org, B, hd, wd, H, W, 1.f, sig, partials, cost, stream);
 }
 
-int dmh_roi_cost_fwd_scaled(const float* d_pre, const float* mask, const int* org, int B, int hd, int wd, int H, int W,
-                            float scale, float* sig, float* partials, float* cost, void* stream) {
+static int roi_cost_fwd_common(const float* d_pre, const float* mask, const int* org, int B, int hd, int wd, int H, int W,
+                               float scale, float* sig, float* partials, float* cost, int* tickets, void* stream) {
     DMH_REQUIRE(d_pre && mask && org && sig && partials && cost, "null pointer");
     DMH_REQUIRE(scale == 1.f || scale == -1.f, "scale must be +1 or -1 (a sign: the result stays bit-identical to -cost)");
     DMH_REQUIRE(B > 0 && B <= 65535 && hd >= 1 && wd >= 1 && hd <= H && wd <= W && (int64_t)hd * wd < (1 << 30), "bad sizes");
     const int nb = cost_blocks(hd * wd);
+    const double n_div = (double)scale * (double)B * (double)H * (double)W;
     hipLaunchKernelGGL(roi_cost_fwd_kernel, dim3(nb, B), dim3(NT), 0, (hipStream_t)stream, d_pre, mask, org, hd, wd, H, W, sig,
-                       partials);
-    hipLaunchKernelGGL(roi_cost_finalize_kernel, dim3(1), dim3(NT), 0, (hipStream_t)stream, partials, nb * B,
-                       (double)scale * (double)B * (double)H * (double)W, cost);
+                       partials, tickets, n_div, cost);
+    if (!tickets)
+        hipLaunchKernelGGL(roi_cost_finalize_kernel, dim3(1), dim3(NT), 0, (hipStream_t)stream, partials, nb * B, n_div, cost);
     return check_launch("dmh_roi_cost_fwd");
+}
+
+int dmh_roi_cost_fwd_scaled(const float* d_pre, const float* mask, const int* org, int B, int hd, int wd, int H, int W,
+                            float scale, float* sig, float* partials, float* cost, void* stream) {
+    return roi_cost_fwd_common(d_pre, mask, org, B, hd, wd, H, W, scale, sig, partials, cost, nullptr, stream);
+}
+
+int dmh_roi_cost_fwd_scaled_tk(const float* d_pre, const float* mask, const int* org, int B, int hd, int wd, int H, int W,
+                               float scale, float* sig, float* partials, float* cost, int* tickets, int n_tickets,
+                               void* stream) {
+    DMH_REQUIRE(tickets && n_tickets >= 1, "a ticket counter is required");
+    return roi_cost_fwd_common(d_pre, mask, org, B, hd, wd, H, W, scale, sig, partials, cost, tickets, stream);
 }
 
 int dmh_roi_cost_bwd(const float* sig, const float* mask, const int* org, int B, int hd, int wd, int H, int W,
diff --git a/depthmodelhardening_amd/ops.py b/depthmodelhardening_amd/ops.py
--- a/depthmodelhardening_amd/ops.py
+++ b/depthmodelhardening_amd/ops.py
@@ -1027,12 +1027,17 @@
     nbt = bn.num_batches_tracked if (track and bn.num_batches_tracked is not None) else None
     if nbt is not None and not (nbt.is_cuda and nbt.dtype == torch.int64 and nbt.numel() == 1):
         raise RuntimeError("bn_act_train: num_batches_tracked must be a CUDA int64 scalar")
-    N.check(_timed("bn_train_stats", lambda: lib.dmh_bn_train_stats_tracked(
-        N.ptr(x), B, Cc, HW, N.ptr(None if bn.weight is None else _c(bn.weight.detach())),
-        N.ptr(None if bn.bias is None else _c(bn.bias.detach())), float(bn.momentum), float(bn.eps),
-        N.ptr(bn.running_mean if track else None), N.ptr(bn.running_var if track else None),
-        None if nbt is None else C.c_void_p(nbt.data_ptr()), N.ptr(part), N.ptr(scale),
-        N.ptr(shift), N.ptr(mean), N.ptr(invstd), N.stream()), 4 * x.numel()))
+    tk = _tickets(dev, Cc)
+    args = (N.ptr(x), B, Cc, HW, N.ptr(None if bn.weight is None else _c(bn.weight.detach())),
+            N.ptr(None if bn.bias is None else _c(bn.bias.detach())), float(bn.momentum), float(bn.eps),
+            N.ptr(bn.running_mean if track else None), N.ptr(bn.running_var if track else None),
+            None if nbt is None else C.c_void_p(nbt.data_ptr()), N.ptr(part), N.ptr(scale),
+            N.ptr(shift), N.ptr(mean), N.ptr(invstd))
+    if tk is None:
+        N.check(_timed("bn_train_stats", lambda: lib.dmh_bn_train_stats_tracked(*args, N.stream()), 4 * x.numel()))
+    else:
+        N.check(_timed("bn_train_stats", lambda: lib.dmh_bn_train_stats_tracked_tk(*args, N.ptr(tk), tk.numel(), N.stream()),
+                       4 * x.numel()))
     return scale, shift, mean, invstd
 
 
@@ -1049,8 +1054,13 @@
     HW = g.numel() // (B * Cc)
     part = torch.empty(lib.dmh_channel_sum_partials_size(B, Cc, HW), device=g.device, dtype=torch.float32)
     out = torch.empty(Cc, device=g.device, dtype=torch.float32)
-    N.check(_timed("channel_sum", lambda: lib.dmh_channel_sum(N.ptr(g), B, Cc, HW, N.ptr(part), N.ptr(out), N.stream()),
-                   4 * g.numel()))
+    tk = _tickets(g.device, Cc)
+    if tk is None:
+        N.check(_timed("channel_sum", lambda: lib.dmh_channel_sum(N.ptr(g), B, Cc, HW, N.ptr(part), N.ptr(out), N.stream()),
+                       4 * g.numel()))
+    else:
+        N.check(_timed("channel_sum", lambda: lib.dmh_channel_sum_tk(N.ptr(g), B, Cc, HW, N.ptr(part), N.ptr(out), N.ptr(tk),
+                                                                     tk.numel(), N.stream()), 4 * g.numel()))
     return out
 
 
@@ -1067,9 +1077,13 @@
     gb = torch.empty(Cc, device=g.device, dtype=torch.float32)
     g_pre = torch.empty_like(g) if want_pre else None
     nb = 4 * g.numel() * ((6 if out is not None else 4) + 1 + (1 if want_pre else 0))
-    N.check(_timed("bn_train_bwd", lambda: lib.dmh_bn_train_bwd(
-        N.ptr(x), N.ptr(g), N.ptr(out), N.ptr(weight), N.ptr(mean), N.ptr(invstd), B, Cc, HW, N.ptr(ws), N.ptr(gx), N.ptr(gw),
-        N.ptr(gb), N.ptr(g_pre), N.stream()), nb))
+    tk = _tickets(g.device, Cc)
+    args = (N.ptr(x), N.ptr(g), N.ptr(out), N.ptr(weight), N.ptr(mean), N.ptr(invstd), B, Cc, HW, N.ptr(ws), N.ptr(gx), N.ptr(gw),
+            N.ptr(gb), N.ptr(g_pre))
+    if tk is None:
+        N.check(_timed("bn_train_bwd", lambda: lib.dmh_bn_train_bwd(*args, N.stream()), nb))
+    else:
+        N.check(_timed("bn_train_bwd", lambda: lib.dmh_bn_train_bwd_tk(*args, N.ptr(tk), tk.numel(), N.stream()), nb))
     return gx, gw, gb, g_pre
 
 
@@ -1393,6 +1407,8 @@
 
 
 _sk_ws = {}
+_sk_tk = {}
+_TICKET_CHANNELS = 512
 _SK_SLOT_FLOATS = 16384
 
 
@@ -1405,7 +1421,16 @@
     ws = _sk_ws.get(key)
     if ws is None:
         ws = _sk_ws[key] = torch.empty(_sk_ws_floats(device), device=device, dtype=torch.float32)
+        _tickets(device)
     return ws
+
+
+def _tickets(device, need=0):
+    key = (device.index if device.index is not None else torch.cuda.current_device(), torch.cuda.current_stream(device).cuda_stream)
+    tk = _sk_tk.get(key)
+    if tk is None:
+        tk = _sk_tk[key] = torch.zeros(_TICKET_CHANNELS, device=device, dtype=torch.int32)
+    return tk if need <= tk.numel() else None
 
 
 def _k10_act(lib, x, U, bias, res, relu, B, Cc, K, H, W, pad, y, stream):
@@ -2054,8 +2079,9 @@
         sig = torch.empty_like(d_pre)
         part = torch.empty(lib.dmh_roi_cost_partials_size(B, hd, wd_), device=dev, dtype=torch.float32)
         cost = torch.empty((), device=dev, dtype=torch.float32)
-        N.check(lib.dmh_roi_cost_fwd_scaled(N.ptr(d_pre), N.ptr(mask), N.ptr(org["d"]), B, hd, wd_, H0, W0, sign, N.ptr(sig),
-                                            N.ptr(part), N.ptr(cost), N.stream()))
+        tk = _tickets(dev)
+        N.check(lib.dmh_roi_cost_fwd_scaled_tk(N.ptr(d_pre), N.ptr(mask), N.ptr(org["d"]), B, hd, wd_, H0, W0, sign, N.ptr(sig),
+                                               N.ptr(part), N.ptr(cost), N.ptr(tk), tk.numel(), N.stream()))
         ctx.save_for_backward(x_top, mask, tab, sig, *feats, *outs, *wb[0::2])
         ctx.plan, ctx.depth, ctx.f0c, ctx.sign = plan, depth, f0c, sign
         return cost
diff --git a/include/dmh_hip.h b/include/dmh_hip.h
--- a/include/dmh_hip.h
+++ b/include/dmh_hip.h
@@ -242,6 +242,9 @@
                      const float* gscale, float* g_pre, void* stream);
 int dmh_roi_cost_fwd_scaled(const float* d_pre, const float* mask, const int* org, int B, int hd, int wd, int H, int W,
                             float scale, float* sig, float* partials, float* cost, void* stream);
+int dmh_roi_cost_fwd_scaled_tk(const float* d_pre, const float* mask, const int* org, int B, int hd, int wd, int H, int W,
+                               float scale, float* sig, float* partials, float* cost, int* tickets, int n_tickets,
+                               void* stream);
 int dmh_roi_cost_bwd_scaled(const float* sig, const float* mask, const int* org, int B, int hd, int wd, int H, int W,
                             float scale, const float* gscale, float* g_pre, void* stream);
 
@@ -265,12 +268,21 @@
                                float eps, float* running_mean, float* running_var, long long* num_batches_tracked,
                                float* partials, float* scale, float* shift, float* save_mean, float* save_invstd,
                                void* stream);
+int dmh_bn_train_stats_tracked_tk(const float* x, int B, int C, int HW, const float* weight, const float* bias, float momentum,
+                                  float eps, float* running_mean, float* running_var, long long* num_batches_tracked,
+                                  float* partials, float* scale, float* shift, float* save_mean, float* save_invstd,
+                                  int* tickets, int n_tickets, void* stream);
 int64_t dmh_channel_sum_partials_size(int B, int C, int HW);
 int dmh_channel_sum(const float* g, int B, int C, int HW, float* partials, float* out, void* stream);
+int dmh_channel_sum_tk(const float* g, int B, int C, int HW, float* partials, float* out, int* tickets, int n_tickets,
+                       void* stream);
 int64_t dmh_bn_train_bwd_workspace_size(int B, int C, int HW);
 int dmh_bn_train_bwd(const float* x, const float* g_out, const float* out, const float* weight, const float* save_mean,
                      const float* save_invstd, int B, int C, int HW, float* workspace, float* g_x, float* g_weight,
                      float* g_bias, float* g_pre, void* stream);
+int dmh_bn_train_bwd_tk(const float* x, const float* g_out, const float* out, const float* weight, const float* save_mean,
+                        const float* save_invstd, int B, int C, int HW, float* workspace, float* g_x, float* g_weight,
+                        float* g_bias, float* g_pre, int* tickets, int n_tickets, void* stream);
 int dmh_stem_bn_relu_pool_fwd(const float* x, const float* scale, const float* shift, int B, int C, int H, int W,
                               float* feat, float* pooled, unsigned char* argmax, void* stream);
 int dmh_stem_bn_relu_pool_bwd(const float* feat, const unsigned char* argmax, const float* g_feat, const float* g_pooled,
```
